# skamann/mcmc-dynamics

Hardware: AMD Instinct MI355X
Metric: star-walker log-L terms/sec (higher is better)
Workload: dtype f64; 1 GPU; C3: 1e6 synthetic stars x 256 walkers, rotation+dispersion + fixed single-Gaussian background mixture (ConstantFit + background.Gaussian), fixed centre; stars_per_gpu=1000000, stars_total=1000000, walkers=256, likelihood=bgfixed, parallelism=1 GPU

## Files before the change

include/mcd.h:

```cpp
#ifndef MCD_H
#define MCD_H

#include <stdint.h>

#ifdef __cplusplus
extern "C" {
#endif

#define MCD_ABI_VERSION 1
#define MCD_UNIQUE_ID_BYTES 128

typedef struct mcd_ctx mcd_ctx;
typedef struct mcd_catalog mcd_catalog;

typedef enum {
    MCD_OK = 0,
    MCD_ERR_INVALID = -1,
    MCD_ERR_HIP = -2,
    MCD_ERR_RCCL = -3,
    MCD_ERR_NO_DEVICE = -4,
    MCD_ERR_NONFINITE = -5,
    MCD_ERR_NOMEM = -6
} mcd_status;

typedef enum {
    MCD_MODEL_CONST = 0,
    MCD_MODEL_CONST_BGFIXED = 1,
    MCD_MODEL_CONST_BGGAUSS = 2,
    MCD_MODEL_PROFILE = 3,
    MCD_MODEL_PROFILE_BGGAUSS = 4,
    MCD_MODEL_PROFILE_BGDENS = 5,
    MCD_MODEL_PROFILE_BGFIXED = 6
} mcd_model;

typedef enum {
    MCD_CENTRE_FIXED = 0,
    MCD_CENTRE_FREE = 1
} mcd_centre;

typedef enum {
    MCD_F64 = 0,
    MCD_F32 = 1,
    MCD_F32_ACC64 = 2
} mcd_precision;

typedef struct {
    int64_t n_stars;
    const double* ra;
    const double* dec;
    const double* v;
    const double* verr;
    const double* lnlike_bg;
    const double* pmember;
    const double* density;
    int32_t model;
    int32_t centre;
    int32_t precision;
    int32_t reserved;
    double ra_center;
    double dec_center;
    int64_t n_bins;
    const int64_t* bin_offsets;
} mcd_catalog_desc;


int mcd_ctx_create(int n_dev, const int* dev_ids, mcd_ctx** out);

int mcd_get_unique_id(void* out_id);
int mcd_ctx_create_rank(int device, int rank, int n_ranks, const void* unique_id, mcd_ctx** out);

int mcd_ctx_set_option(mcd_ctx* ctx, const char* key, int64_t value);
int mcd_ctx_abort(mcd_ctx* ctx, const char* reason);
int mcd_ctx_failed(const mcd_ctx* ctx);

int mcd_ctx_destroy(mcd_ctx* ctx);
int mcd_ctx_n_devices(const mcd_ctx* ctx);
int mcd_ctx_comm_info(const mcd_ctx* ctx, int* comm_size, int* comm_rank, int* rccl_version);


int mcd_catalog_create(mcd_ctx* ctx, const mcd_catalog_desc* desc, mcd_catalog** out);
int mcd_catalog_destroy(mcd_catalog* cat);

int mcd_catalog_param_count(const mcd_catalog* cat);
int64_t mcd_catalog_n_stars(const mcd_catalog* cat);
int64_t mcd_catalog_n_outputs(const mcd_catalog* cat, int64_t n_walkers);


int mcd_loglike_batch(mcd_catalog* cat, int64_t n_walkers, int32_t k, const double* params, double* out);

int mcd_params_upload(mcd_catalog* cat, int64_t n_walkers, int32_t k, const double* params);
int mcd_loglike_enqueue(mcd_catalog* cat);
int mcd_loglike_fetch(mcd_catalog* cat, double* out);
int mcd_sync(mcd_catalog* cat);

int mcd_membership(mcd_catalog* cat, int32_t k, const double* params, double* out);
int mcd_loglike_per_star(mcd_catalog* cat, int32_t k, const double* params, double* out);
int mcd_pointwise_posterior(mcd_catalog* cat, int64_t n_samples, int32_t k, const double* params,
                            double* lppd, double* lnl_var, double* pmem_mean, double* pmem_std);
int mcd_psis_loo(mcd_catalog* cat, int64_t n_samples, int32_t k, const double* params, double r_eff,
                 double* elpd_loo, double* pareto_k, double* lppd, double* n_eff);

int mcd_kde_background(mcd_ctx* ctx, int64_t n_comp, const double* comp, int64_t n, const double* v,
                       const double* verr, double sigma_int, double* out, double* kernel_ms);


typedef struct {
    int64_t n_walkers;
    int32_t n_dim;
    int32_t k;
    const int32_t* col_source;
    const double* col_const;
    const double* col_factor;
    const double* lo;
    const double* hi;
    int32_t fixed_ok;
    int32_t n_bins;
} mcd_stretch_desc;

int mcd_stretch_move(mcd_catalog* cat, const mcd_stretch_desc* desc, int64_t n_steps, double* pos, double* lnp,
                     const int32_t* order, const double* zz, const double* thr, const int32_t* pick, double* chain,
                     double* lnprob_chain, int64_t* accepted);
int mcd_stretch_move_seeded(mcd_catalog* cat, const mcd_stretch_desc* desc, int64_t n_steps, double* pos, double* lnp,
                            uint64_t seed, int64_t step0, double* chain, double* lnprob_chain, int64_t* accepted);
int mcd_chain_numbers(uint64_t seed, int64_t step0, int64_t n_steps, int64_t n_bins, int64_t n_walkers, int32_t n_dim,
                      int32_t* order, double* zz, double* thr, int32_t* pick);

int mcd_stretch_info(const mcd_catalog* cat, int64_t* device_blocks, int64_t* host_blocks, int64_t* discarded_blocks,
                     int32_t* last_discard_status);


const char* mcd_last_error(void);
int mcd_abi_version(void);
double mcd_last_kernel_ms(const mcd_catalog* cat);
double mcd_last_device_ms(const mcd_catalog* cat);
int mcd_set_option(mcd_catalog* cat, const char* key, int64_t value);
int mcd_timing_collect(mcd_catalog* cat, double* total_kernel_ms, int64_t* n_launches);
int64_t mcd_rerun_count(const mcd_catalog* cat);
int mcd_last_prefetch(const mcd_catalog* cat);
int mcd_last_narrow_bounded(const mcd_catalog* cat);
int mcd_last_fast_level(const mcd_catalog* cat);

int mcd_last_f32_domain(const mcd_catalog* cat, double* kappa_v, double* kappa_theta);
int mcd_last_launch_info(const mcd_catalog* cat, int64_t* n_workgroups, int32_t* walker_tile,
                         int64_t* n_chunks, int32_t* record_bytes);

#ifdef __cplusplus
}
#endif
#endif
```

mcmc_dynamics_amd/_native.py:

```python
import atexit
import ctypes
import os
import weakref

import numpy as np

_HERE = os.path.dirname(os.path.abspath(__file__))
LIB_PATH = os.environ.get("MCD_LIB_PATH") or os.path.join(_HERE, "libmcd_hip.so")

MODEL_CONST, MODEL_CONST_BGFIXED, MODEL_CONST_BGGAUSS = 0, 1, 2
MODEL_PROFILE, MODEL_PROFILE_BGGAUSS, MODEL_PROFILE_BGDENS, MODEL_PROFILE_BGFIXED = 3, 4, 5, 6
CENTRE_FIXED, CENTRE_FREE = 0, 1
F64, F32, F32_ACC64 = 0, 1, 2
PRECISIONS = {"f64": F64, "f32": F32, "f32acc64": F32_ACC64}
UNIQUE_ID_BYTES = 128

_c_double_p = ctypes.POINTER(ctypes.c_double)
_c_int64_p = ctypes.POINTER(ctypes.c_int64)

SYMBOLS = {
    "mcd_ctx_create": (ctypes.c_int, [ctypes.c_int, ctypes.POINTER(ctypes.c_int), ctypes.POINTER(ctypes.c_void_p)]),
    "mcd_get_unique_id": (ctypes.c_int, [ctypes.c_void_p]),
    "mcd_ctx_create_rank": (ctypes.c_int, [ctypes.c_int, ctypes.c_int, ctypes.c_int, ctypes.c_void_p,
                                           ctypes.POINTER(ctypes.c_void_p)]),
    "mcd_ctx_destroy": (ctypes.c_int, [ctypes.c_void_p]),
    "mcd_ctx_set_option": (ctypes.c_int, [ctypes.c_void_p, ctypes.c_char_p, ctypes.c_int64]),
    "mcd_ctx_abort": (ctypes.c_int, [ctypes.c_void_p, ctypes.c_char_p]),
    "mcd_ctx_failed": (ctypes.c_int, [ctypes.c_void_p]),
    "mcd_ctx_n_devices": (ctypes.c_int, [ctypes.c_void_p]),
    "mcd_ctx_comm_info": (ctypes.c_int, [ctypes.c_void_p, ctypes.POINTER(ctypes.c_int), ctypes.POINTER(ctypes.c_int),
                                         ctypes.POINTER(ctypes.c_int)]),
    "mcd_catalog_create": (ctypes.c_int, [ctypes.c_void_p, ctypes.c_void_p, ctypes.POINTER(ctypes.c_void_p)]),
    "mcd_catalog_destroy": (ctypes.c_int, [ctypes.c_void_p]),
    "mcd_catalog_param_count": (ctypes.c_int, [ctypes.c_void_p]),
    "mcd_catalog_n_stars": (ctypes.c_int64, [ctypes.c_void_p]),
    "mcd_catalog_n_outputs": (ctypes.c_int64, [ctypes.c_void_p, ctypes.c_int64]),
    "mcd_loglike_batch": (ctypes.c_int, [ctypes.c_void_p, ctypes.c_int64, ctypes.c_int32, _c_double_p, _c_double_p]),
    "mcd_params_upload": (ctypes.c_int, [ctypes.c_void_p, ctypes.c_int64, ctypes.c_int32, _c_double_p]),
    "mcd_loglike_enqueue": (ctypes.c_int, [ctypes.c_void_p]),
    "mcd_loglike_fetch": (ctypes.c_int, [ctypes.c_void_p, _c_double_p]),
    "mcd_sync": (ctypes.c_int, [ctypes.c_void_p]),
    "mcd_membership": (ctypes.c_int, [ctypes.c_void_p, ctypes.c_int32, _c_double_p, _c_double_p]),
    "mcd_loglike_per_star": (ctypes.c_int, [ctypes.c_void_p, ctypes.c_int32, _c_double_p, _c_double_p]),
    "mcd_pointwise_posterior": (ctypes.c_int, [ctypes.c_void_p, ctypes.c_int64, ctypes.c_int32, _c_double_p, _c_double_p,
                                               _c_double_p, _c_double_p, _c_double_p]),
    "mcd_psis_loo": (ctypes.c_int, [ctypes.c_void_p, ctypes.c_int64, ctypes.c_int32, _c_double_p, ctypes.c_double,
                                    _c_double_p, _c_double_p, _c_double_p, _c_double_p]),
    "mcd_kde_background": (ctypes.c_int, [ctypes.c_void_p, ctypes.c_int64, _c_double_p, ctypes.c_int64, _c_double_p,
                                          _c_double_p, ctypes.c_double, _c_double_p, _c_double_p]),
    "mcd_stretch_move": (ctypes.c_int, [ctypes.c_void_p, ctypes.c_void_p, ctypes.c_int64, _c_double_p, _c_double_p,
                                        ctypes.POINTER(ctypes.c_int32), _c_double_p, _c_double_p,
                                        ctypes.POINTER(ctypes.c_int32), _c_double_p, _c_double_p, _c_int64_p]),
    "mcd_stretch_move_seeded": (ctypes.c_int, [ctypes.c_void_p, ctypes.c_void_p, ctypes.c_int64, _c_double_p, _c_double_p,
                                               ctypes.c_uint64, ctypes.c_int64, _c_double_p, _c_double_p, _c_int64_p]),
    "mcd_chain_numbers": (ctypes.c_int, [ctypes.c_uint64, ctypes.c_int64, ctypes.c_int64, ctypes.c_int64, ctypes.c_int64,
                                         ctypes.c_int32, ctypes.POINTER(ctypes.c_int32), _c_double_p, _c_double_p,
                                         ctypes.POINTER(ctypes.c_int32)]),
    "mcd_stretch_info": (ctypes.c_int, [ctypes.c_void_p, _c_int64_p, _c_int64_p, _c_int64_p, ctypes.POINTER(ctypes.c_int32)]),
    "mcd_last_error": (ctypes.c_char_p, []),
    "mcd_abi_version": (ctypes.c_int, []),
    "mcd_last_kernel_ms": (ctypes.c_double, [ctypes.c_void_p]),
    "mcd_last_device_ms": (ctypes.c_double, [ctypes.c_void_p]),
    "mcd_timing_collect": (ctypes.c_int, [ctypes.c_void_p, _c_double_p, _c_int64_p]),
    "mcd_rerun_count": (ctypes.c_int64, [ctypes.c_void_p]),
    "mcd_last_prefetch": (ctypes.c_int, [ctypes.c_void_p]),
    "mcd_last_narrow_bounded": (ctypes.c_int, [ctypes.c_void_p]),
    "mcd_last_fast_level": (ctypes.c_int, [ctypes.c_void_p]),
    "mcd_last_f32_domain": (ctypes.c_int, [ctypes.c_void_p, _c_double_p, _c_double_p]),
    "mcd_set_option": (ctypes.c_int, [ctypes.c_void_p, ctypes.c_char_p, ctypes.c_int64]),
    "mcd_last_launch_info": (ctypes.c_int, [ctypes.c_void_p, _c_int64_p, ctypes.POINTER(ctypes.c_int32), _c_int64_p,
                                            ctypes.POINTER(ctypes.c_int32)]),
}


class NativeError(RuntimeError):
    """Raised when the HIP library is missing, fails to load, or a call returns an error status."""


class CatalogDesc(ctypes.Structure):
    _fields_ = [
        ("n_stars", ctypes.c_int64),
        ("ra", _c_double_p), ("dec", _c_double_p), ("v", _c_double_p), ("verr", _c_double_p),
        ("lnlike_bg", _c_double_p), ("pmember", _c_double_p), ("density", _c_double_p),
        ("model", ctypes.c_int32), ("centre", ctypes.c_int32), ("precision", ctypes.c_int32),
        ("reserved", ctypes.c_int32),
        ("ra_center", ctypes.c_double), ("dec_center", ctypes.c_double),
        ("n_bins", ctypes.c_int64), ("bin_offsets", _c_int64_p),
    ]


class StretchDesc(ctypes.Structure):
    _fields_ = [
        ("n_walkers", ctypes.c_int64), ("n_dim", ctypes.c_int32), ("k", ctypes.c_int32),
        ("col_source", ctypes.POINTER(ctypes.c_int32)), ("col_const", _c_double_p), ("col_factor", _c_double_p),
        ("lo", _c_double_p), ("hi", _c_double_p), ("fixed_ok", ctypes.c_int32), ("n_bins", ctypes.c_int32),
    ]


TEST_SWITCHES = ("MCD_LIB_PATH", "MCD_RCCL_LIBRARY", "MCD_ALLOW_SHARED_DEVICE", "MCD_FORCE_RCCL", "MCD_TARGET_WAVES",
                 "MCD_CHAIN_PART_BYTES", "MCD_CHAIN_PARTS", "MCD_COLLECTIVE_TIMEOUT_MS")

_lib = None
_live_catalogs = weakref.WeakSet()
_live_contexts = weakref.WeakSet()


@atexit.register
def _shutdown():
    for cat in list(_live_catalogs):
        try:
            cat.close()
        except Exception:
            pass
    for ctx in list(_live_contexts):
        try:
            ctx.close()
        except Exception:
            pass


def load_library(path=None):
    global _lib
    if _lib is not None and path is None:
        return _lib
    p = path or LIB_PATH
    if not os.path.exists(p):
        raise NativeError(
            "HIP library not found at {0}: build it with `make -C mcmc_dynamics_amd/csrc` "
            "(or __graft_entry__.build()); there is no CPU fallback.".format(p))
    try:
        lib = ctypes.CDLL(p)
    except OSError as exc:
        raise NativeError("could not load {0}: {1}".format(p, exc))
    for name, (restype, argtypes) in SYMBOLS.items():
        try:
            fn = getattr(lib, name)
        except AttributeError:
            raise NativeError("{0} does not export {1}".format(p, name))
        fn.restype = restype
        fn.argtypes = argtypes
    if path is None:
        _lib = lib
        active = ["{0}={1}".format(k, os.environ[k]) for k in TEST_SWITCHES if os.environ.get(k)]
        if active:
            import logging
            logging.getLogger("mcmc_dynamics_amd").warning(
                "test / tuning switches active (none is needed in production, see INTEGRATION.md): %s", ", ".join(active))
    return lib


def _check(lib, rc, what):
    if rc != 0:
        msg = lib.mcd_last_error()
        raise NativeError("{0} failed (status {1}): {2}".format(what, rc, msg.decode() if msg else ""))


def _f64(a):
    return np.ascontiguousarray(a, dtype=np.float64)


def _ptr(a):
    return a.ctypes.data_as(_c_double_p) if a is not None else None


class Context(object):

    def __init__(self, n_devices=1, device_ids=None, rank=None, n_ranks=None, unique_id=None, device=None):
        self.lib = load_library()
        handle = ctypes.c_void_p()
        if rank is not None:
            uid = ctypes.create_string_buffer(bytes(unique_id), UNIQUE_ID_BYTES) if unique_id is not None else None
            rc = self.lib.mcd_ctx_create_rank(int(device or 0), int(rank), int(n_ranks), uid, ctypes.byref(handle))
            _check(self.lib, rc, "mcd_ctx_create_rank")
            self.rank, self.n_ranks = int(rank), int(n_ranks)
        else:
            ids = None
            if device_ids is not None:
                ids = (ctypes.c_int * len(device_ids))(*[int(d) for d in device_ids])
                n_devices = len(device_ids)
            rc = self.lib.mcd_ctx_create(int(n_devices), ids, ctypes.byref(handle))
            _check(self.lib, rc, "mcd_ctx_create")
            self.rank, self.n_ranks = 0, 1
        self.handle = handle
        self.host_group = None
        self._catalogs = weakref.WeakSet()
        _live_contexts.add(self)

    @staticmethod
    def unique_id():
        lib = load_library()
        buf = ctypes.create_string_buffer(UNIQUE_ID_BYTES)
        _check(lib, lib.mcd_get_unique_id(buf), "mcd_get_unique_id")
        return buf.raw

    @property
    def n_devices(self):
        return self.lib.mcd_ctx_n_devices(self.handle)

    def set_option(self, key, value):
        _check(self.lib, self.lib.mcd_ctx_set_option(self.handle, key.encode(), int(value)), "mcd_ctx_set_option")

    def abort(self, reason=""):
        if getattr(self, "handle", None):
            self.lib.mcd_ctx_abort(self.handle, str(reason).encode()[:400])

    @property
    def failed(self):
        return bool(getattr(self, "handle", None)) and bool(self.lib.mcd_ctx_failed(self.handle))

    def comm_info(self):
        n, r, v = ctypes.c_int(), ctypes.c_int(), ctypes.c_int()
        _check(self.lib, self.lib.mcd_ctx_comm_info(self.handle, ctypes.byref(n), ctypes.byref(r), ctypes.byref(v)),
               "mcd_ctx_comm_info")
        return {"size": n.value, "rank": r.value, "rccl_version": v.value}

    def kde_background(self, comp, v, verr, sigma_int=0.0, return_kernel_ms=False):
        if not getattr(self, "handle", None):
            raise NativeError("context is closed")
        comp, v, verr = _f64(comp).ravel(), _f64(v).ravel(), _f64(verr).ravel()
# ... 86 lines not shown
        self.k = self.lib.mcd_catalog_param_count(handle)
        self._walkers = 0
        _live_catalogs.add(self)
        ctx._catalogs.add(self)

    def _params(self, params):
        p = _f64(params)
        if p.ndim == 1:
            p = p[None, :]
        if self.n_sets > 1:
            if p.ndim != 3 or p.shape[0] != self.n_sets:
                raise ValueError("binned catalogue expects params of shape (n_bins, W, K)")
            w = p.shape[1]
        else:
            if p.ndim == 3 and p.shape[0] == 1:
                p = p[0]
            if p.ndim != 2:
                raise ValueError("params must have shape (W, K)")
            w = p.shape[0]
        if p.shape[-1] != self.k:
            raise ValueError("params have {0} columns, catalogue expects {1}".format(p.shape[-1], self.k))
        return np.ascontiguousarray(p), w

    def _alive(self):
        if not getattr(self, "handle", None):
            raise NativeError("catalogue is closed")

    def loglike(self, params):
        self._alive()
        p, w = self._params(params)
        out = np.empty((self.n_sets, w) if self.n_sets > 1 else (w,), dtype=np.float64)
        rc = self.lib.mcd_loglike_batch(self.handle, w, self.k, _ptr(p), _ptr(out))
        _check(self.lib, rc, "mcd_loglike_batch")
        self._walkers = w
        return out

    def upload_params(self, params):
        p, w = self._params(params)
        _check(self.lib, self.lib.mcd_params_upload(self.handle, w, self.k, _ptr(p)), "mcd_params_upload")
        self._walkers = w

    def enqueue(self):
        _check(self.lib, self.lib.mcd_loglike_enqueue(self.handle), "mcd_loglike_enqueue")

    def sync(self):
        _check(self.lib, self.lib.mcd_sync(self.handle), "mcd_sync")

    def fetch(self):
        w = self._walkers
        out = np.empty((self.n_sets, w) if self.n_sets > 1 else (w,), dtype=np.float64)
        _check(self.lib, self.lib.mcd_loglike_fetch(self.handle, _ptr(out)), "mcd_loglike_fetch")
        return out

    def membership(self, params_row):
        p = _f64(params_row).reshape(-1)
        out = np.empty(self.n_stars, dtype=np.float64)
        _check(self.lib, self.lib.mcd_membership(self.handle, p.size, _ptr(p), _ptr(out)), "mcd_membership")
        return out

    def loglike_per_star(self, params_row):
        p = _f64(params_row).reshape(-1)
        out = np.empty(self.n_stars, dtype=np.float64)
        _check(self.lib, self.lib.mcd_loglike_per_star(self.handle, p.size, _ptr(p), _ptr(out)), "mcd_loglike_per_star")
        return out

    def pointwise_posterior(self, table, membership=False):
        self._alive()
        if self.n_sets > 1:
            raise ValueError("pointwise_posterior is defined for un-binned catalogues only")
        p = _f64(table)
        if p.ndim == 1:
            p = p[None, :]
        if p.ndim != 2 or p.shape[1] != self.k:
            raise ValueError("table must have shape (S, {0})".format(self.k))
        p = np.ascontiguousarray(p)
        names = ("lppd", "lnl_var") + (("pmem_mean", "pmem_std") if membership else ())
        out = {k: np.empty(self.n_stars, dtype=np.float64) for k in names}
        ptrs = [_ptr(out[k]) if k in out else None for k in ("lppd", "lnl_var", "pmem_mean", "pmem_std")]
        rc = self.lib.mcd_pointwise_posterior(self.handle, p.shape[0], self.k, _ptr(p), *ptrs)
        _check(self.lib, rc, "mcd_pointwise_posterior")
        return out

    def psis_loo(self, table, r_eff=1.0):
        self._alive()
        if self.n_sets > 1:
            raise ValueError("psis_loo is defined for un-binned catalogues only")
        p = _f64(table)
        if p.ndim == 1:
            p = p[None, :]
        if p.ndim != 2 or p.shape[1] != self.k:
            raise ValueError("table must have shape (S, {0})".format(self.k))
        p = np.ascontiguousarray(p)
        names = ("elpd_loo", "pareto_k", "lppd", "n_eff")
        out = {k: np.empty(self.n_stars, dtype=np.float64) for k in names}
        rc = self.lib.mcd_psis_loo(self.handle, p.shape[0], self.k, _ptr(p), float(r_eff), *[_ptr(out[k]) for k in names])
        _check(self.lib, rc, "mcd_psis_loo")
        return out

    def _stretch_args(self, name, plan, pos, lnp, n_steps, chain, lnprob_chain, accepted):
        self._alive()
        for a in (pos, lnp):
            if a.dtype != np.float64 or not a.flags.c_contiguous:
                raise ValueError(name + " needs C-contiguous arrays of the documented dtypes")
        if pos.ndim not in (2, 3) or lnp.shape != pos.shape[:-1]:
            raise ValueError(name + ": inconsistent array shapes")
        lead, (w, p) = pos.shape[:-2], pos.shape[-2:]
        cols = [np.ascontiguousarray(plan["col_source"], dtype=np.int32), _f64(plan["col_const"]), _f64(plan["col_factor"]),
                _f64(plan["lo"]), _f64(plan["hi"])]
        if cols[0].size != self.k or cols[1].size != self.k or cols[2].size != self.k or cols[3].size != p or cols[4].size != p:
            raise ValueError("stretch_move: plan does not match the catalogue / the number of free parameters")
        d = StretchDesc()
        d.n_walkers, d.n_dim, d.k, d.n_bins = w, p, self.k, lead[0] if lead else 1
        d.col_source = cols[0].ctypes.data_as(ctypes.POINTER(ctypes.c_int32))
        d.col_const, d.col_factor, d.lo, d.hi = (_ptr(c) for c in cols[1:])
        d.fixed_ok = 1 if plan.get("fixed_ok", True) else 0
        for a, shape in ((chain, (n_steps,) + lead + (w, p)), (lnprob_chain, (n_steps,) + lead + (w,))):
            if a is not None and (a.dtype != np.float64 or not a.flags.c_contiguous or a.shape != shape):
                raise ValueError("stretch_move: chain buffers must be C-contiguous float64 of shape (steps, [B,] W, P) / (steps, [B,] W)")
        if accepted is not None and (accepted.dtype != np.int64 or accepted.shape != lead + (w,) or not accepted.flags.c_contiguous):
            raise ValueError("stretch_move: accepted must be a C-contiguous int64 array of shape ([B,] W)")
        return ((self.handle, ctypes.byref(d), n_steps, _ptr(pos), _ptr(lnp)),
                (_ptr(chain), _ptr(lnprob_chain), accepted.ctypes.data_as(_c_int64_p) if accepted is not None else None), cols)

    def stretch_move(self, plan, pos, lnp, order, zz, thr, pick, chain=None, lnprob_chain=None, accepted=None):
        head, tail, _keep = self._stretch_args("stretch_move", plan, pos, lnp, order.shape[0], chain, lnprob_chain, accepted)
        for a, dt in ((zz, np.float64), (thr, np.float64), (order, np.int32), (pick, np.int32)):
            if a.dtype != dt or not a.flags.c_contiguous:
                raise ValueError("stretch_move needs C-contiguous arrays of the documented dtypes")
        half_shape = (order.shape[0], 2) + pos.shape[:-2] + (pos.shape[-2] // 2,)
        if order.shape != order.shape[:1] + lnp.shape or zz.shape != half_shape or thr.shape != half_shape or \
                pick.shape != half_shape:
            raise ValueError("stretch_move: inconsistent array shapes")
        rc = self.lib.mcd_stretch_move(*head, order.ctypes.data_as(ctypes.POINTER(ctypes.c_int32)), _ptr(zz), _ptr(thr),
                                       pick.ctypes.data_as(ctypes.POINTER(ctypes.c_int32)), *tail)
        _check(self.lib, rc, "mcd_stretch_move")
        self._walkers = pos.shape[-2] // 2

    def stretch_move_seeded(self, plan, pos, lnp, seed, step0, n_steps, chain=None, lnprob_chain=None, accepted=None):
        if n_steps < 0 or step0 < 0:
            raise ValueError("stretch_move_seeded: inconsistent array shapes")
        head, tail, _keep = self._stretch_args("stretch_move_seeded", plan, pos, lnp, n_steps, chain, lnprob_chain, accepted)
        rc = self.lib.mcd_stretch_move_seeded(*head, int(seed) & 0xFFFFFFFFFFFFFFFF, int(step0), *tail)
        _check(self.lib, rc, "mcd_stretch_move_seeded")
        self._walkers = pos.shape[-2] // 2

    @property
    def last_prefetch(self):
        return self.lib.mcd_last_prefetch(self.handle)

    @property
    def last_narrow_bounded(self):
        return self.lib.mcd_last_narrow_bounded(self.handle)

    def stretch_info(self):
        a, b, c, st = ctypes.c_int64(), ctypes.c_int64(), ctypes.c_int64(), ctypes.c_int32()
        _check(self.lib, self.lib.mcd_stretch_info(self.handle, ctypes.byref(a), ctypes.byref(b), ctypes.byref(c), ctypes.byref(st)),
               "mcd_stretch_info")
        return {"device_blocks": a.value, "host_blocks": b.value, "discarded_blocks": c.value, "last_discard_status": st.value}

    def set_option(self, key, value):
        _check(self.lib, self.lib.mcd_set_option(self.handle, key.encode(), int(value)), "mcd_set_option")

    @property
    def last_kernel_ms(self):
        return self.lib.mcd_last_kernel_ms(self.handle)

    @property
    def last_device_ms(self):
        return self.lib.mcd_last_device_ms(self.handle)

    def timing_collect(self):
        total, n = ctypes.c_double(), ctypes.c_int64()
        _check(self.lib, self.lib.mcd_timing_collect(self.handle, ctypes.byref(total), ctypes.byref(n)),
               "mcd_timing_collect")
        return total.value, n.value

    @property
    def rerun_count(self):
        return self.lib.mcd_rerun_count(self.handle)

    @property
    def fast_level(self):
        return self.lib.mcd_last_fast_level(self.handle)

    @property
    def f32_in_domain(self):
        return bool(self.lib.mcd_last_f32_domain(self.handle, None, None))

    @property
    def f32_condition(self):
        kv, kt = ctypes.c_double(), ctypes.c_double()
        self.lib.mcd_last_f32_domain(self.handle, ctypes.byref(kv), ctypes.byref(kt))
        return kv.value, kt.value

    def launch_info(self):
        wg, ch = ctypes.c_int64(), ctypes.c_int64()
        tile, rb = ctypes.c_int32(), ctypes.c_int32()
        _check(self.lib, self.lib.mcd_last_launch_info(self.handle, ctypes.byref(wg), ctypes.byref(tile),
                                                       ctypes.byref(ch), ctypes.byref(rb)), "mcd_last_launch_info")
        return {"workgroups": wg.value, "walker_tile": tile.value, "chunks": ch.value, "record_bytes": rb.value}

    def close(self):
        if getattr(self, "handle", None):
            self.lib.mcd_catalog_destroy(self.handle)
            self.handle = None

    def __del__(self):
        try:
            self.close()
        except Exception:
            pass
```

mcmc_dynamics_amd/csrc/mcd_api_catalog.hip:

```cpp
#include "mcd_host.h"

using namespace mcd::host;

namespace {

int param_count(int model, bool free_centre) {
    int k = (mcd::is_profile(model) ? 6 : 4) + (free_centre ? 2 : 0);
    const int bg = mcd::bg_kind(model);
    if (bg == mcd::BG_GAUSS) k += 3;
    if (bg == mcd::BG_FIXED_DENSITY) k += 1;
    return k;
}

void free_workset(WorkSet& w) {
    if (w.d_chunks) (void)hipFree(w.d_chunks);
    if (w.d_offsets) (void)hipFree(w.d_offsets);
    if (w.d_chunk_general) (void)hipFree(w.d_chunk_general);
    if (w.d_params) (void)hipFree(w.d_params);
    if (w.d_wpar) (void)hipFree(w.d_wpar);
    if (w.d_partials) (void)hipFree(w.d_partials);
    if (w.d_out) (void)hipFree(w.d_out);
    if (w.d_out2) (void)hipFree(w.d_out2);
    if (w.d_partials2) (void)hipFree(w.d_partials2);
    if (w.ev_staged) (void)hipEventDestroy(w.ev_staged);
    for (int b = 0; b < 2; ++b) {
        if (w.ev_reduced[b]) (void)hipEventDestroy(w.ev_reduced[b]);
        if (w.ev_comm[b]) (void)hipEventDestroy(w.ev_comm[b]);
    }
    if (w.h_params) (void)hipHostFree(w.h_params);
    if (w.h_out) (void)hipHostFree(w.h_out);
    w = WorkSet();
}

double model_cost(int model, bool free_centre) {
    static const double kCost[mcd::kNumModels] = {8.5, 24.0, 45.0, 25.0, 60.0, 40.0, 42.0};
    return (kCost[model] + (free_centre ? 7.0 : 0.0)) / 8.5;
}
int balance_auto_m(const mcd_catalog* cat, int64_t n, int64_t n_walkers) {
    const int64_t n_wtiles = (n_walkers + 63) / 64;
    const double tiles = n_wtiles <= 4 ? (double)n_wtiles : 4.0 * (double)((n_wtiles + 3) / 4);
    const double work = (double)n * tiles / 4.0 * model_cost(cat->model, cat->free_centre);
    const double limit = mcd::bg_kind(cat->model) == mcd::BG_NONE ? 9.0e5 : 1.3e6;
    if (cat->n_psets != 1 || work > limit) return 0;
    return work < 6.0e4 ? 2 : (work <= 3.4e5 ? 4 : 8);
}

bool wants_prefetch(const mcd_catalog* cat, const Shard& sh) {
    if (cat->prefetch >= 0) return cat->prefetch != 0;
    const size_t bytes = (size_t)sh.n * (size_t)mcd::record_bytes(cat->model, cat->free_centre, cat->precision);
    if (mcd::bg_kind(cat->model) == mcd::BG_NONE) return cat->n_psets == 1 && bytes >= ((size_t)128 << 20);
    return bytes >= ((size_t)8 << 20);
}

struct Option {
    const char* key;
    int64_t min, max;
    const char* message;
    bool sync, replan;
    void (*set)(mcd_catalog* c, int64_t v);
    bool (*accepts)(int64_t v) = nullptr;
};
constexpr int64_t kMin = std::numeric_limits<int64_t>::min(), kMax = std::numeric_limits<int64_t>::max();
#define MCD_SET(statement) [](mcd_catalog* c, int64_t v) { statement; }
const Option kOptions[] = {
    {"fast_path", 0, 2, "fast_path: 0 (plain), 1 (guarded, default) or 2 (guarded, no narrow variant)", false, false, MCD_SET(c->allow_fast = (int)v)},
    {"zero_copy", kMin, kMax, nullptr, false, false, MCD_SET(c->zero_copy = v != 0)},
    {"device_chain", 0, 2, "device_chain: 0 (host-driven blocks), 1 (default) or 2 (as 1 with the general step kernel, testing aid)", false, false,
     MCD_SET(c->device_chain = (int)v; c->chain_backoff = 0; c->chain_consecutive = 0; c->chain_hint = -1)},
    {"fused_reduce", kMin, kMax, nullptr, false, false, MCD_SET(c->fused_reduce = v != 0)},
    {"defer_guard", kMin, kMax, nullptr, false, false, MCD_SET(c->defer_guard = v != 0)},
    {"f32_domain", kMin, kMax, nullptr, false, false, MCD_SET(c->f32_domain = v != 0)},
    {"loo_scratch_mb", 1, kMax, "loo_scratch_mb must be >= 1", false, false, MCD_SET(c->loo_scratch_mb = v)},
    {"posterior_pass", 1, kMax, "posterior_pass must be >= 1", false, false, MCD_SET(c->posterior_pass = v)},
    {"two_lanes", kMin, kMax, nullptr, true, false, MCD_SET(c->two_lanes = v != 0)},
    {"narrow_bounded", 0, 1, "narrow_bounded: 1 (where the guard admits it, default) or 0 (never)", false, false, MCD_SET(c->narrow_bounded = (int)v)},
    {"prefetch", -1, 1, "prefetch: -1 (by record volume, default), 0 (off) or 1 (on)", false, false, MCD_SET(c->prefetch = (int)v)},
    {"spin_us", 0, kMax, "spin_us must be >= 0", false, false, MCD_SET(c->spin_us = v)},
    {"tail_split", kMin, kMax, nullptr, true, true, MCD_SET(c->tail_split = (int)v)},
    {"target_waves", 1, kMax, "target_waves must be positive", true, true, MCD_SET(c->target_waves = v)},
    {"chunk_len", 0, kMax, "chunk_len must be >= 0", true, true, MCD_SET(c->chunk_len = v)},
    {"balance", -1, 8, "balance: -1 (auto), 0 (off) or 1 .. 8 workgroups per CU", true, true, MCD_SET(c->balance = (int)v)},
    {"combine", 0, 16, "combine: 0 (never), 1 (largest workgroup the plan allows), 8 or 16 (waves per workgroup at most)", true, true,
     MCD_SET(c->combine = (int)v), [](int64_t v) { return v <= 1 || v == 8 || v == 16; }},
};
#undef MCD_SET
}

MCD_HOST_BEGIN

LaunchShape main_launch_shape(mcd_catalog* cat, const Shard& sh, const WorkSet& w, int level, bool coll, double* out_buf,
                              int64_t n_out) {
    LaunchShape shape{cat->model, cat->free_centre, cat->precision, level, w.uniform_len, sh.n};
    shape.uniform_extra = w.uniform_extra;
    shape.waves = w.waves;
    shape.chunk_general = w.d_chunk_general;
    shape.prefetch = wants_prefetch(cat, sh);
    cat->last_prefetch = shape.prefetch && shape.fast != 0;
    shape.rerun_flag = coll ? nullptr : out_buf + n_out;
    return shape;
}

const double* fast_pset_const(const mcd_catalog* cat, const Shard& sh, int level) {
    const int bgk = mcd::bg_kind(cat->model);
    return (level && (bgk == mcd::BG_FIXED || bgk == mcd::BG_FIXED_DENSITY)) ? sh.d_pset_const : nullptr;
}

int build_workset(mcd_catalog* cat, Shard& sh, int64_t n_walkers, WorkSet** out) {
    auto it = sh.work.find(n_walkers);
    if (it != sh.work.end()) { *out = &it->second; return MCD_OK; }
    if (sh.work.size() >= 8) {
        for (auto& kv : sh.work) free_workset(kv.second);
        sh.work.clear();
        cat->cur_walkers = 0;
    }
    const DeviceSlot& slot = cat->ctx->slots[sh.slot];
    MCD_HIP(hipSetDevice(slot.device));

    mcd::ChunkPlan plan;
    for (int m = cat->balance < 0 ? balance_auto_m(cat, sh.n, n_walkers) : cat->balance;; m /= 2) {
        plan = mcd::plan_chunks(cat->bin_offsets, sh.star_begin, sh.n, n_walkers, cat->target_waves, cat->tail_split,
                                cat->stats.narrow_exceptions, cat->chunk_len, m);
        if (m == 0 || plan.balanced_m > 0) break;
    }
    const std::vector<mcd::Chunk>& chunks = plan.chunks;
    const std::vector<int64_t>& offs = plan.offsets;
    const std::vector<uint8_t>& general = plan.general;

    WorkSet w;
    w.n_walkers = n_walkers;
    w.n_chunks = (int64_t)chunks.size();
    w.max_chunks_per_pset = plan.max_chunks_per_pset;
    w.uniform_len = plan.uniform_len;
    w.uniform_extra = plan.uniform_extra;
    {
        const int64_t n_wtiles = (n_walkers + 63) / 64;
        const bool shape_ok = plan.balanced_m > 0 && plan.balanced_m % 2 == 0 && (n_wtiles == 1 || n_wtiles == 2 || n_wtiles == 4) &&
                              cat->precision == MCD_F64;
        w.waves = 4;
        if (cat->combine != 0 && shape_ok) {
            const bool can16 = mcd::bg_kind(cat->model) != mcd::BG_GAUSS;
            w.waves = 8;
            if (cat->combine == 16 && plan.balanced_m % 4 == 0 && can16) w.waves = 16;
            if (cat->combine == 1 && plan.balanced_m == 4 && can16) w.waves = 16;
        }
    }
    const int64_t padded_walkers = (n_walkers + 63) / 64 * 64;
    const int64_t n_out = cat->n_psets * n_walkers;
    const size_t term_bytes = cat->precision == MCD_F64 ? 8 : 4;
    auto allocate = [&]() -> hipError_t {
        hipError_t e;
        if (!general.empty()) {
            if ((e = hipMalloc(&w.d_chunk_general, general.size())) != hipSuccess) return e;
            if ((e = hipMemcpy(w.d_chunk_general, general.data(), general.size(), hipMemcpyHostToDevice)) != hipSuccess) return e;
        }
        if ((e = hipMalloc(&w.d_chunks, std::max<size_t>(1, chunks.size()) * sizeof(mcd::Chunk))) != hipSuccess) return e;
        if ((e = hipMalloc(&w.d_offsets, offs.size() * sizeof(int64_t))) != hipSuccess) return e;
        if ((e = hipMalloc(&w.d_params, (size_t)n_out * cat->k * sizeof(double))) != hipSuccess) return e;
        if ((e = hipMalloc(&w.d_wpar, (size_t)n_out * mcd::KD * term_bytes)) != hipSuccess) return e;
        if ((e = hipMalloc(&w.d_partials, std::max<size_t>(1, (size_t)padded_walkers * w.n_chunks) * sizeof(double))) != hipSuccess) return e;
        if ((e = hipMalloc(&w.d_out, (size_t)(n_out + 1) * sizeof(double))) != hipSuccess) return e;
        if ((e = hipMemset(w.d_out, 0, (size_t)(n_out + 1) * sizeof(double))) != hipSuccess) return e;
        if ((e = hipMalloc(&w.d_out2, (size_t)(n_out + 1) * sizeof(double))) != hipSuccess) return e;
        if ((e = hipMemset(w.d_out2, 0, (size_t)(n_out + 1) * sizeof(double))) != hipSuccess) return e;
        if ((e = hipEventCreateWithFlags(&w.ev_staged, hipEventDisableTiming)) != hipSuccess) return e;
        for (int b = 0; b < 2; ++b) {
            if ((e = hipEventCreateWithFlags(&w.ev_reduced[b], hipEventDisableTiming)) != hipSuccess) return e;
            if ((e = hipEventCreateWithFlags(&w.ev_comm[b], hipEventDisableTiming)) != hipSuccess) return e;
        }
        if ((e = hipHostMalloc(&w.h_params, (size_t)n_out * cat->k * sizeof(double), hipHostMallocMapped)) != hipSuccess) return e;
        if ((e = hipHostMalloc(&w.h_out, (size_t)(n_out + 1) * sizeof(double), hipHostMallocMapped)) != hipSuccess) return e;
        std::memset(w.h_out, 0, (size_t)(n_out + 1) * sizeof(double));
        if ((e = hipHostGetDevicePointer((void**)&w.m_params, w.h_params, 0)) != hipSuccess) return e;
        if ((e = hipHostGetDevicePointer((void**)&w.m_out, w.h_out, 0)) != hipSuccess) return e;
        if (!chunks.empty() &&
            (e = hipMemcpy(w.d_chunks, chunks.data(), chunks.size() * sizeof(mcd::Chunk), hipMemcpyHostToDevice)) != hipSuccess)
            return e;
        return hipMemcpy(w.d_offsets, offs.data(), offs.size() * sizeof(int64_t), hipMemcpyHostToDevice);
    };
    const hipError_t err = allocate();
    if (err != hipSuccess) {
        free_workset(w);
        return fail(MCD_ERR_HIP, std::string("work buffers for this walker count: ") + hipGetErrorString(err));
    }
    auto ins = sh.work.emplace(n_walkers, w);
    *out = &ins.first->second;
    return MCD_OK;
}

MCD_HOST_END

extern "C" {

static int catalog_create_impl(mcd_ctx* ctx, const mcd_catalog_desc* d, std::unique_ptr<mcd_catalog>& cat);

int mcd_catalog_create(mcd_ctx* ctx, const mcd_catalog_desc* d, mcd_catalog** out) {
    try {
    if (!ctx || !d || !out) return fail(MCD_ERR_INVALID, "mcd_catalog_create: null argument");
    std::unique_ptr<mcd_catalog> cat;
    const int rc = catalog_create_impl(ctx, d, cat);
    if (rc != MCD_OK) {
        if (cat) {
            const std::string msg = g_last_error;
            mcd_catalog_destroy(cat.release());
            g_last_error = msg;
        }
        return rc;
    }
    *out = cat.release();
    return MCD_OK;
    } catch (...) { return on_exception("mcd_catalog_create"); }
}

static int catalog_create_impl(mcd_ctx* ctx, const mcd_catalog_desc* d, std::unique_ptr<mcd_catalog>& cat) {
    if (int urc = ctx_usable(ctx)) return urc;
    if (d->n_stars < 0) return fail(MCD_ERR_INVALID, "negative n_stars");
    if (d->model < 0 || d->model >= mcd::kNumModels) return fail(MCD_ERR_INVALID, "unknown model");
    const int bgk = mcd::bg_kind(d->model);
    if (d->centre != MCD_CENTRE_FIXED && d->centre != MCD_CENTRE_FREE) return fail(MCD_ERR_INVALID, "unknown centre mode");
    if (d->precision < MCD_F64 || d->precision > MCD_F32_ACC64) return fail(MCD_ERR_INVALID, "unknown precision");
    if (d->n_stars > 0 && (!d->ra || !d->dec || !d->v || !d->verr)) return fail(MCD_ERR_INVALID, "missing ra/dec/v/verr column");
    if (bgk == mcd::BG_FIXED && d->n_stars > 0 && (!d->lnlike_bg || !d->pmember))
        return fail(MCD_ERR_INVALID, "background model needs lnlike_bg and pmember columns");
    if (bgk == mcd::BG_GAUSS && d->n_stars > 0 && !d->density)
        return fail(MCD_ERR_INVALID, "Gaussian-background model needs the density column");
    if (bgk == mcd::BG_FIXED_DENSITY && d->n_stars > 0 && (!d->lnlike_bg || !d->density))
        return fail(MCD_ERR_INVALID, "constant-background model needs lnlike_bg and density columns");

    cat.reset(new (std::nothrow) mcd_catalog());
    if (!cat) return fail(MCD_ERR_INVALID, "out of memory");
    cat->ctx = ctx;
    cat->model = d->model;
    cat->free_centre = d->centre == MCD_CENTRE_FREE;
    cat->precision = d->precision;
    cat->k = param_count(d->model, cat->free_centre);
    cat->n_stars = d->n_stars;
    if (const char* tw = std::getenv("MCD_TARGET_WAVES")) {
        long v = std::atol(tw);
        if (v > 0) cat->target_waves = v;
    }
    if (d->n_bins > 1) {
        if (!d->bin_offsets) return fail(MCD_ERR_INVALID, "bin_offsets required when n_bins > 1");
        cat->n_psets = d->n_bins;
        cat->bin_offsets.assign(d->bin_offsets, d->bin_offsets + d->n_bins + 1);
        if (cat->bin_offsets.front() != 0 || cat->bin_offsets.back() != d->n_stars)
            return fail(MCD_ERR_INVALID, "bin_offsets must start at 0 and end at n_stars");
        for (int64_t b = 0; b < d->n_bins; ++b)
            if (cat->bin_offsets[b + 1] < cat->bin_offsets[b]) return fail(MCD_ERR_INVALID, "bin_offsets must be non-decreasing");
    } else {
        cat->n_psets = 1;
        cat->bin_offsets = {0, d->n_stars};
    }

    cat->stats = mcd::compute_stats(d->n_stars, d->v, d->verr, d->lnlike_bg, d->pmember, d->density, bgk,
                                    cat->precision != MCD_F64 || mcd::is_profile(cat->model) ? d->ra : nullptr, d->dec,
                                    !cat->free_centre, d->ra_center, d->dec_center);

    const int n_dev = (int)ctx->slots.size();
    cat->shards.resize(n_dev);
    const int rec_bytes = mcd::record_bytes(cat->model, cat->free_centre, cat->precision);
    for (int i = 0; i < n_dev; ++i) {
        Shard& sh = cat->shards[i];
        sh.slot = i;
        const mcd::ShardRange range = mcd::shard_range(d->n_stars, i, n_dev);
        sh.star_begin = range.begin;
        sh.n = range.n;
        const DeviceSlot& slot = ctx->slots[i];
        MCD_HIP(hipSetDevice(slot.device));
        MCD_HIP(hipEventCreate(&sh.ev_begin));
        MCD_HIP(hipEventCreate(&sh.ev_k0));
        MCD_HIP(hipEventCreate(&sh.ev_k1));
        MCD_HIP(hipEventCreate(&sh.ev_end));
        MCD_HIP(hipMalloc(&sh.records, (size_t)sh.n * rec_bytes + 2048));
        MCD_HIP(hipMemsetAsync(sh.records, 0, (size_t)sh.n * rec_bytes + 2048, slot.stream));
        if (bgk == mcd::BG_FIXED || bgk == mcd::BG_FIXED_DENSITY) {
            const std::vector<double> sums = mcd::pset_background_sums(d->lnlike_bg, cat->bin_offsets, sh.star_begin, sh.n);
            MCD_HIP(hipMalloc(&sh.d_pset_const, sums.size() * sizeof(double)));
            MCD_HIP(hipMemcpy(sh.d_pset_const, sums.data(), sums.size() * sizeof(double), hipMemcpyHostToDevice));
        }
        if (sh.n == 0) continue;
        const double* host_cols[7] = {d->ra, d->dec, d->v, d->verr, d->lnlike_bg, d->pmember, d->density};
        struct Scratch {
            double* p[7] = {nullptr, nullptr, nullptr, nullptr, nullptr, nullptr, nullptr};
            ~Scratch() { for (double* q : p) if (q) (void)hipFree(q); }
        } dev;
        for (int c = 0; c < 7; ++c) {
            if (!host_cols[c]) continue;
            MCD_HIP(hipMalloc(&dev.p[c], (size_t)sh.n * sizeof(double)));
            MCD_HIP(hipMemcpyAsync(dev.p[c], host_cols[c] + sh.star_begin, (size_t)sh.n * sizeof(double),
                                   hipMemcpyHostToDevice, slot.stream));
        }
        mcd::RawColumns raw{dev.p[0], dev.p[1], dev.p[2], dev.p[3], dev.p[4], dev.p[5], dev.p[6]};
        MCD_HIP(mcd::launch_prepare_records(slot.stream, raw, sh.n, cat->model, cat->free_centre, cat->precision,
                                            d->ra_center, d->dec_center, sh.records));
        MCD_HIP(hipStreamSynchronize(slot.stream));
    }
    return MCD_OK;
}

int mcd_catalog_destroy(mcd_catalog* cat) {
    if (!cat) return MCD_OK;
    if (cat->ctx && cat->ctx->failed.load()) { delete cat; return MCD_OK; }
    for (Shard& sh : cat->shards) {
        (void)hipSetDevice(cat->ctx->slots[sh.slot].device);
        (void)hipStreamSynchronize(cat->ctx->slots[sh.slot].stream);
        (void)hipStreamSynchronize(cat->ctx->slots[sh.slot].comm_stream);
        (void)hipStreamSynchronize(cat->ctx->slots[sh.slot].stream2);
        for (auto& kv : sh.work) free_workset(kv.second);
        if (sh.records) (void)hipFree(sh.records);
        if (sh.d_pset_const) (void)hipFree(sh.d_pset_const);
        if (sh.ev_begin) (void)hipEventDestroy(sh.ev_begin);
        if (sh.ev_k0) (void)hipEventDestroy(sh.ev_k0);
        if (sh.ev_k1) (void)hipEventDestroy(sh.ev_k1);
        if (sh.ev_end) (void)hipEventDestroy(sh.ev_end);
        for (auto& pr : sh.ring) { (void)hipEventDestroy(pr.first); (void)hipEventDestroy(pr.second); }
    }
    for (hipEvent_t e : cat->chain_events) (void)hipEventDestroy(e);
    if (cat->chain.d) (void)hipFree(cat->chain.d);
    if (cat->chain.h) (void)hipHostFree(cat->chain.h);
    delete cat;
    return MCD_OK;
}

int mcd_catalog_param_count(const mcd_catalog* cat) { return cat ? cat->k : MCD_ERR_INVALID; }
int64_t mcd_catalog_n_stars(const mcd_catalog* cat) { return cat ? cat->n_stars : MCD_ERR_INVALID; }
int64_t mcd_catalog_n_outputs(const mcd_catalog* cat, int64_t n_walkers) {
    return cat ? cat->n_psets * n_walkers : MCD_ERR_INVALID;
}

int mcd_set_option(mcd_catalog* cat, const char* key, int64_t value) {
    try {
    if (!cat || !key) return fail(MCD_ERR_INVALID, "mcd_set_option: null argument");
    if (!std::strcmp(key, "timing")) {
        int rc = sync_all(cat);
        if (rc != MCD_OK) return rc;
        cat->timing = value != 0;
        cat->timing_all = value == 2;
        for (Shard& sh : cat->shards) sh.ring_used = 0;
        return MCD_OK;
    }
    if (!std::strcmp(key, "timing_discard")) {
        int rc = sync_all(cat);
        if (rc != MCD_OK) return rc;
        for (Shard& sh : cat->shards) sh.ring_used = 0;
        cat->timing_launches = 0;
        return MCD_OK;
    }
    if (!std::strcmp(key, "timing_stride")) {
        if (value < 1) return fail(MCD_ERR_INVALID, "timing_stride must be >= 1");
        int rc = sync_all(cat);
        if (rc != MCD_OK) return rc;
        cat->timing_stride = value;
        cat->timing_launches = 0;
        return MCD_OK;
    }
    if (!std::strcmp(key, "timing_reserve")) {
        if (value < 0 || value > ((int64_t)1 << 16)) return fail(MCD_ERR_INVALID, "timing_reserve: 0 .. 65536 launches");
        for (Shard& sh : cat->shards) {
            MCD_HIP(hipSetDevice(cat->ctx->slots[sh.slot].device));
            while ((int64_t)sh.ring.size() < value) {
                hipEvent_t a, b;
                MCD_HIP(hipEventCreate(&a));
                if (hipEventCreate(&b) != hipSuccess) { (void)hipEventDestroy(a); return fail(MCD_ERR_HIP, "hipEventCreate"); }
                sh.ring.emplace_back(a, b);
            }
        }
        return MCD_OK;
    }
    for (const Option& o : kOptions) {
        if (std::strcmp(key, o.key)) continue;
        if (value < o.min || value > o.max || (o.accepts && !o.accepts(value))) return fail(MCD_ERR_INVALID, o.message);
        if (o.sync)
            if (int rc = sync_all(cat)) return rc;
        o.set(cat, value);
        if (o.replan) {
            for (Shard& sh : cat->shards) {
                (void)hipSetDevice(cat->ctx->slots[sh.slot].device);
                for (auto& kv : sh.work) free_workset(kv.second);
                sh.work.clear();
            }
            cat->cur_walkers = 0;
        }
        return MCD_OK;
    }
    return fail(MCD_ERR_INVALID, std::string("unknown option: ") + key);
    } catch (...) { return on_exception("mcd_set_option"); }
}

int mcd_timing_collect(mcd_catalog* cat, double* total_kernel_ms, int64_t* n_launches) {
    try {
    if (!cat) return fail(MCD_ERR_INVALID, "null catalogue");
    int rc = sync_all(cat);
    if (rc != MCD_OK) return rc;
    Shard& sh = cat->shards[0];
    double total = 0.0;
    for (size_t i = 0; i < sh.ring_used; ++i) {
        float ms = 0.f;
        MCD_HIP(hipEventElapsedTime(&ms, sh.ring[i].first, sh.ring[i].second));
        total += ms;
    }
    if (total_kernel_ms) *total_kernel_ms = total;
    if (n_launches) *n_launches = (int64_t)sh.ring_used;
    for (Shard& s2 : cat->shards) s2.ring_used = 0;
    cat->timing_launches = 0;
    return MCD_OK;
    } catch (...) { return on_exception("mcd_timing_collect"); }
}

int64_t mcd_rerun_count(const mcd_catalog* cat) { return cat ? cat->n_reruns : MCD_ERR_INVALID; }

int mcd_stretch_info(const mcd_catalog* cat, int64_t* device_blocks, int64_t* host_blocks, int64_t* discarded_blocks,
                     int32_t* last_discard_status) {
    if (!cat) return fail(MCD_ERR_INVALID, "null catalogue");
    if (device_blocks) *device_blocks = cat->chain_device_blocks;
    if (host_blocks) *host_blocks = cat->chain_host_blocks;
    if (discarded_blocks) *discarded_blocks = cat->chain_discarded;
    if (last_discard_status) *last_discard_status = cat->chain_last_status;
    return MCD_OK;
}

int mcd_last_prefetch(const mcd_catalog* cat) { return cat ? cat->last_prefetch : -1; }

int mcd_last_narrow_bounded(const mcd_catalog* cat) { return cat ? cat->last_narrow_bounded : -1; }

int mcd_last_f32_domain(const mcd_catalog* cat, double* kappa_v, double* kappa_theta) {
    if (!cat) return -1;
    if (kappa_v) *kappa_v = cat->last_f32.kappa_v;
    if (kappa_theta) *kappa_theta = cat->last_f32.kappa_theta;
    if (cat->precision == MCD_F64) return 1;
    return cat->last_f32.inside ? 1 : 0;
}

int mcd_last_fast_level(const mcd_catalog* cat) {
    if (!cat || cat->cur_walkers <= 0 || cat->shards.empty()) return -1;
    const auto it = cat->shards.front().work.find(cat->cur_walkers);
    return it == cat->shards.front().work.end() ? -1 : it->second.fast;
}

double mcd_last_kernel_ms(const mcd_catalog* cat) { return cat ? cat->last_kernel_ms : -1.0; }
double mcd_last_device_ms(const mcd_catalog* cat) { return cat ? cat->last_device_ms : -1.0; }

int mcd_last_launch_info(const mcd_catalog* cat, int64_t* n_workgroups, int32_t* walker_tile, int64_t* n_chunks,
                         int32_t* record_bytes) {
    if (!cat) return fail(MCD_ERR_INVALID, "null catalogue");
    if (n_workgroups) *n_workgroups = cat->last_grid;
    if (walker_tile) *walker_tile = 64;
    if (n_chunks) *n_chunks = cat->last_chunks;
    if (record_bytes) *record_bytes = mcd::record_bytes(cat->model, cat->free_centre, cat->precision);
    return MCD_OK;
}

}
```

mcmc_dynamics_amd/csrc/mcd_api_chain.hip:

```cpp
#include "mcd_host.h"
#include "mcd_rng.h"
#include "mcd_stretch.h"

using namespace mcd::host;

namespace {

void big_copy(void* dst, const void* src, size_t bytes) {
    constexpr size_t kSerial = (size_t)4 << 20;
    if (bytes < kSerial) { std::memcpy(dst, src, bytes); return; }
    constexpr int kMaxThreads = 16;
    static const int kThreads = [] {
        const char* e = std::getenv("MCD_COPY_THREADS");
        const int n = e ? std::atoi(e) : 4;
        return n < 1 ? 1 : (n > kMaxThreads ? kMaxThreads : n);
    }();
    std::thread workers[kMaxThreads - 1];
    const size_t part = (bytes / kThreads + 63) / 64 * 64;
    int started = 0;
    for (int t = 1; t < kThreads; ++t) {
        const size_t at = std::min(bytes, part * t), len = std::min(bytes, part * (t + 1)) - at;
        try {
            workers[t - 1] = std::thread([=] { if (len) std::memcpy((char*)dst + at, (const char*)src + at, len); });
            ++started;
// ... 10 lines not shown
int stretch_block_device(mcd_catalog* cat, const mcd_stretch_desc* d, int64_t n_steps, double* pos, double* lnp,
                         const int32_t* order, const double* zz, const double* thr, const int32_t* pick, double* chain,
                         double* lnprob_chain, int64_t* accepted, bool* done, const uint64_t* seed = nullptr,
                         int64_t step0 = 0) {
    *done = false;
    mcd_ctx* ctx = cat->ctx;
    if (int urc = ctx_usable(ctx)) return urc;
    const int64_t B = cat->n_psets;
    if (!cat->device_chain || cat->shards.size() != 1 || cat->precision != MCD_F64 || n_steps < 1 || cat->timing || !d->fixed_ok)
        return MCD_OK;
    if (B > 1 && cat->device_chain != 1) return MCD_OK;
    if (cat->chain_backoff > 0) { --cat->chain_backoff; return MCD_OK; }
    const int64_t W = d->n_walkers, half = W / 2;
    const int P = d->n_dim, K = d->k;
    bool small_ensemble = false;
    {
        mcd::StretchDevice probe;
        probe.n_bins = B; probe.n_walkers = W; probe.n_dim = P; probe.k = K;
        probe.force_general = cat->device_chain == 2;
        if (!mcd::stretch_step_handles(probe)) return MCD_OK;
        small_ensemble = mcd::stretch_step_fuses(probe);
    }
    Shard& sh = cat->shards[0];
    const DeviceSlot& slot = ctx->slots[sh.slot];
    MCD_HIP(hipSetDevice(slot.device));
    WorkSet* wp = nullptr;
    int rc = build_workset(cat, sh, half, &wp);
    if (rc != MCD_OK) return rc;
    WorkSet& w = *wp;
    MCD_WAIT(cat->ctx, slot.stream, cat->spin_us, "mcd_stretch_move (previous evaluation)");
    MCD_WAIT(cat->ctx, slot.stream2, cat->spin_us, "mcd_stretch_move (previous evaluation, second lane)");
    MCD_WAIT(cat->ctx, slot.comm_stream, cat->spin_us, "mcd_stretch_move (previous collective)");
    w.comm_pending[0] = w.comm_pending[1] = false;
    w.staged = false;

    size_t off = 0;
    auto take = [&](size_t bytes) { const size_t at = off; off += (bytes + 63) / 64 * 64; return at; };
    const size_t BW = (size_t)B * W, Bh = (size_t)B * half;
    const size_t o_pos = take(BW * P * 8), o_lnp = take(BW * 8), o_acc = take(BW * 8);
    const size_t o_meta = take(mcd::META_WORDS * 4), o_status = take(8);
    const size_t n_launches = (size_t)2 * n_steps;
    const bool defer = cat->defer_guard != 0 && B == 1 && small_ensemble && n_launches * half * K * 8 <= ((size_t)64 << 20);
    const size_t o_levels = take(defer ? n_launches * 4 : 0);
    const size_t state_end = off;
    const size_t o_src = take((size_t)K * 4), o_const = take((size_t)K * 8), o_fac = take((size_t)K * 8);
    const size_t o_lo = take((size_t)P * 8), o_hi = take((size_t)P * 8);
    const bool seeded = seed != nullptr;
    const bool gen_device = seeded && mcd::chain_numbers_on_device(W);
    const size_t n_in = (size_t)n_steps;
    const size_t o_order = take(n_in * BW * 4), o_zz = take(n_in * BW * 8);
    const size_t o_thr = take(n_in * BW * 8), o_pick = take(n_in * BW * 4);
    const size_t input_end = off;
    const size_t o_prop = take(Bh * P * 8), o_ok = take(Bh), o_nok = take((size_t)2 * B * 4), o_ranges = take((size_t)2 * B * 10 * 8);
    const size_t o_nok_log = take(defer ? n_launches * 4 : 0), o_table_log = take(defer ? n_launches * half * K * 8 : 0);
    const size_t o_chain = take(chain ? (size_t)n_steps * BW * P * 8 : 0);
    const size_t o_lnpc = take(lnprob_chain ? (size_t)n_steps * BW * 8 : 0);
    const size_t total = off;
    ChainArena& a = cat->chain;
    if (a.bytes < total) {
        if (a.d) (void)hipFree(a.d);
        if (a.h) (void)hipHostFree(a.h);
        a = ChainArena();
        const size_t want = total + total / 2;
        const bool must_agree = ctx->n_ranks > 1 || ctx->force_collective;
        if (hipMalloc((void**)&a.d, want) != hipSuccess) {
            (void)hipGetLastError();
            a = ChainArena();
            if (must_agree) return fail(MCD_ERR_NOMEM, "mcd_stretch_move: no device memory for the resident block of this rank (use shorter blocks)");
            return MCD_OK;
        }
        if (hipHostMalloc((void**)&a.h, want, hipHostMallocDefault) != hipSuccess) {
            (void)hipGetLastError();
            (void)hipFree(a.d);
            a = ChainArena();
            if (must_agree) return fail(MCD_ERR_NOMEM, "mcd_stretch_move: no pinned host memory for the resident block of this rank (use shorter blocks)");
            return MCD_OK;
        }
        a.bytes = want;
    }
    std::memcpy(a.h + o_pos, pos, BW * P * 8);
    std::memcpy(a.h + o_lnp, lnp, BW * 8);
    if (accepted) std::memcpy(a.h + o_acc, accepted, BW * 8);
    else std::memset(a.h + o_acc, 0, BW * 8);
    std::memset(a.h + o_meta, 0, mcd::META_WORDS * 4);
    std::memset(a.h + o_status, 0, 8);
    std::memcpy(a.h + o_src, d->col_source, (size_t)K * 4);
    std::memcpy(a.h + o_const, d->col_const, (size_t)K * 8);
    std::memcpy(a.h + o_fac, d->col_factor, (size_t)K * 8);
    std::memcpy(a.h + o_lo, d->lo, (size_t)P * 8);
    std::memcpy(a.h + o_hi, d->hi, (size_t)P * 8);
    const size_t moved = (size_t)n_steps * BW * ((gen_device ? 0 : 24) + (chain ? (size_t)P * 8 : 0) + (lnprob_chain ? 8 : 0));
    size_t part_threshold = (size_t)16 << 20;
    if (const char* e = std::getenv("MCD_CHAIN_PART_BYTES")) part_threshold = (size_t)std::strtoull(e, nullptr, 10);
    int64_t max_parts = 16;
    if (const char* e = std::getenv("MCD_CHAIN_PARTS")) max_parts = std::max<long long>(1, std::atoll(e));
    const int64_t n_parts = moved >= part_threshold ? std::min<int64_t>(max_parts, n_steps) : 1;
    auto part_begin = [&](int64_t k) { return n_steps * k / n_parts; };
    auto copy_in = [&](int64_t i0, int64_t i1) {
        if (gen_device) return;
        const size_t at = (size_t)i0 * BW, n = (size_t)(i1 - i0) * BW;
        if (seeded) {
            std::vector<uint64_t> sorter;
            for (int64_t i = i0; i < i1; ++i)
                mcd::chain_numbers_of_step(*seed, step0 + i, B, W, P, (int32_t*)(a.h + o_order) + (size_t)i * BW,
                                           (double*)(a.h + o_zz) + (size_t)i * BW, (double*)(a.h + o_thr) + (size_t)i * BW,
                                           (int32_t*)(a.h + o_pick) + (size_t)i * BW, sorter);
            return;
        }
        big_copy(a.h + o_order + at * 4, order + at, n * 4);
        big_copy(a.h + o_zz + at * 8, zz + at, n * 8);
        big_copy(a.h + o_thr + at * 8, thr + at, n * 8);
        big_copy(a.h + o_pick + at * 4, pick + at, n * 4);
    };
    if (n_parts == 1) copy_in(0, n_steps);

    int level = cat->chain_hint;
    if (level < 0) {
        std::vector<double> table(BW * K);
        for (size_t j = 0; j < BW; ++j)
            for (int c = 0; c < K; ++c) {
                const int src = d->col_source[c];
                table[j * K + c] = src < 0 ? d->col_const[c]
                                           : (d->col_factor[c] == 1.0 ? pos[j * P + src] : pos[j * P + src] * d->col_factor[c]);
            }
        level = fast_level(cat, table.data(), (int64_t)BW);
    }

    mcd::StretchDevice sd;
    sd.n_bins = B;
    sd.n_walkers = W; sd.n_dim = P; sd.k = K; sd.fixed_ok = d->fixed_ok;
    sd.model = cat->model; sd.free_centre = cat->free_centre ? 1 : 0; sd.allow_fast = cat->allow_fast;
    sd.expected_level = level;
    sd.force_general = cat->device_chain == 2;
    sd.stats = cat->stats;
    sd.col_source = (const int32_t*)(a.d + o_src); sd.col_const = (const double*)(a.d + o_const);
    sd.col_factor = (const double*)(a.d + o_fac); sd.lo = (const double*)(a.d + o_lo); sd.hi = (const double*)(a.d + o_hi);
    sd.pos = (double*)(a.d + o_pos); sd.lnp = (double*)(a.d + o_lnp); sd.accepted = (long long*)(a.d + o_acc);
    sd.order = (const int32_t*)(a.d + o_order); sd.zz = (const double*)(a.d + o_zz); sd.thr = (const double*)(a.d + o_thr);
    sd.pick = (const int32_t*)(a.d + o_pick);
    sd.chain = chain ? (double*)(a.d + o_chain) : nullptr;
    sd.lnprob_chain = lnprob_chain ? (double*)(a.d + o_lnpc) : nullptr;
    sd.proposal = (double*)(a.d + o_prop); sd.ok = (uint8_t*)(a.d + o_ok); sd.meta = (int32_t*)(a.d + o_meta);
    sd.n_ok = (int32_t*)(a.d + o_nok); sd.ranges = (double*)(a.d + o_ranges);
    sd.table = w.d_params; sd.wpar = (double*)w.d_wpar;
    if (defer) {
        sd.defer_guard = 1;
        sd.table_log = (double*)(a.d + o_table_log); sd.n_ok_log = (int32_t*)(a.d + o_nok_log); sd.level_log = (int32_t*)(a.d + o_levels);
    }

    const bool coll = ctx->n_ranks > 1 || ctx->force_collective;
    double* const out_buf = w.d_out;
    mcd::LaunchShape shape = main_launch_shape(cat, sh, w, level, coll, out_buf, (int64_t)Bh);
    cat->last_narrow_bounded = 0;
    const double* pset_const = fast_pset_const(cat, sh, level);
    const int64_t n_slots = mcd::partial_slots(shape, w.n_chunks, half);
    const int64_t max_slots = B == 1 ? n_slots : w.max_chunks_per_pset;
    const bool fused = cat->fused_reduce != 0 && !coll && max_slots <= mcd::kFusedReduceSlots && mcd::stretch_step_fuses(sd);
    sd.fused = fused ? 1 : 0;
    sd.partials = w.d_partials;
    sd.n_slots = n_slots;
    sd.slot_offsets = B == 1 ? nullptr : w.d_offsets;
    sd.pset_const = pset_const;
    cat->chain_last_fused = fused;
    double prev_tag = 0.0;
    int64_t acc_step = -1;
    int acc_h = 0;
#ifdef MCD_CHAIN_STAMPS
    static unsigned long long* d_stamps = nullptr;
    if (!d_stamps) MCD_HIP(hipMalloc((void**)&d_stamps, 8 * 8 * 4096));
    MCD_HIP(hipMemsetAsync(d_stamps, 0, 8 * 8 * 4096, slot.stream));
    sd.stamps = d_stamps;
#endif
    auto enqueue_steps = [&](int64_t i0, int64_t i1, hipEvent_t mark) -> int {
        for (int64_t i = i0; i < i1; ++i)
            for (int h = 0; h < 2; ++h) {
#ifdef MCD_CHAIN_STAMPS
                sd.launch_index = i * 2 + h;
#endif
                MCD_HIP(mcd::launch_stretch_step(slot.stream, sd, acc_step, acc_h, i, h, out_buf, prev_tag));
                if (mark && i == i0 && h == 0) MCD_HIP(hipEventRecord(mark, slot.stream));
                prev_tag = coll ? 0.0 : (double)(++cat->launch_seq);
                shape.launch_tag = prev_tag;
                MCD_HIP(mcd::launch_loglike(slot.stream, shape, sh.records, w.d_chunks, w.n_chunks, w.d_wpar, w.d_partials, half));
                if (!fused)
                    MCD_HIP(mcd::launch_reduce(slot.stream, w.d_partials, w.d_offsets, B, n_slots, max_slots, half, pset_const,
                                               out_buf));
                if (coll) {
                    if (!ctx->multi_process) MCD_NCCL(g_rccl.GroupStart());
                    MCD_NCCL(g_rccl.AllReduce(out_buf, out_buf, Bh, ncclDouble, ncclSum, slot.comm, slot.stream));
                    if (!ctx->multi_process) MCD_NCCL(g_rccl.GroupEnd());
                }
                acc_step = i;
                acc_h = h;
            }
        return MCD_OK;
    };
    auto finish = [&]() -> int {
        MCD_HIP(mcd::launch_stretch_step(slot.stream, sd, acc_step, acc_h, -1, 0, out_buf, prev_tag));
        if (defer) MCD_HIP(mcd::launch_stretch_judge(slot.stream, sd, (int64_t)n_launches));
        if (coll) {
            double* status = (double*)(a.d + o_status);
            MCD_HIP(mcd::launch_stretch_status(slot.stream, sd.meta, status));
            if (!ctx->multi_process) MCD_NCCL(g_rccl.GroupStart());
            MCD_NCCL(g_rccl.AllReduce(status, status, 1, ncclDouble, ncclSum, slot.comm, slot.stream));
            if (!ctx->multi_process) MCD_NCCL(g_rccl.GroupEnd());
        }
        return MCD_OK;
    };
    struct MidBlockGuard {
        mcd_ctx* ctx; bool armed; bool ok;
        ~MidBlockGuard() {
            if (armed && !ok && !ctx->failed.load()) {
                const std::string cause = g_last_error;
                (void)ctx_fail(ctx, "mcd_stretch_move: this rank failed in the middle of a resident block (" + cause + ")");
            }
        }
    } mid_block{ctx, coll, false};
    bool rows_delivered = false;
    auto generate = [&](hipStream_t s, int64_t i0, int64_t i1) {
        return mcd::launch_chain_numbers(s, *seed, step0, i0, i1, B, W, P, (int32_t*)(a.d + o_order), (double*)(a.d + o_zz),
                                         (double*)(a.d + o_thr), (int32_t*)(a.d + o_pick));
    };
    if (n_parts == 1) {
        MCD_HIP(hipMemcpyAsync(a.d, a.h, gen_device ? o_order : input_end, hipMemcpyHostToDevice, slot.stream));
        if (gen_device) MCD_HIP(generate(slot.stream, 0, n_steps));
        rc = enqueue_steps(0, n_steps, nullptr);
        if (rc != MCD_OK) return rc;
        rc = finish();
        if (rc != MCD_OK) return rc;
        MCD_HIP(hipMemcpyAsync(a.h, a.d, state_end, hipMemcpyDeviceToHost, slot.stream));
        if (total > o_chain)
            MCD_HIP(hipMemcpyAsync(a.h + o_chain, a.d + o_chain, total - o_chain, hipMemcpyDeviceToHost, slot.stream));
        MCD_WAIT(cat->ctx, slot.stream, cat->spin_us, "mcd_stretch_move (resident block)");
    } else {
        while ((int64_t)cat->chain_events.size() < 3 * n_parts) {
            hipEvent_t e;
            MCD_HIP(hipEventCreateWithFlags(&e, hipEventDisableTiming));
            cat->chain_events.push_back(e);
        }
        hipEvent_t* ev_in = cat->chain_events.data();
        hipEvent_t* ev_rows = ev_in + n_parts;
        hipEvent_t* ev_out = ev_rows + n_parts;
        auto rows_to_host = [&](int64_t k) -> int {
            const size_t at = (size_t)part_begin(k) * BW, n = (size_t)(part_begin(k + 1) - part_begin(k)) * BW;
            MCD_HIP(hipStreamWaitEvent(slot.comm_stream, ev_rows[k], 0));
            if (chain) MCD_HIP(hipMemcpyAsync(a.h + o_chain + at * P * 8, a.d + o_chain + at * P * 8, n * P * 8, hipMemcpyDeviceToHost, slot.comm_stream));
            if (lnprob_chain) MCD_HIP(hipMemcpyAsync(a.h + o_lnpc + at * 8, a.d + o_lnpc + at * 8, n * 8, hipMemcpyDeviceToHost, slot.comm_stream));
            MCD_HIP(hipEventRecord(ev_out[k], slot.comm_stream));
            return MCD_OK;
        };
        auto rows_to_caller = [&](int64_t k) -> int {
            const size_t at = (size_t)part_begin(k) * BW, n = (size_t)(part_begin(k + 1) - part_begin(k)) * BW;
            MCD_WAIT(cat->ctx, slot.comm_stream, cat->spin_us, "mcd_stretch_move (chain rows of a part)");
            if (chain) big_copy(chain + at * P, a.h + o_chain + at * P * 8, n * P * 8);
            if (lnprob_chain) big_copy(lnprob_chain + at, a.h + o_lnpc + at * 8, n * 8);
            return MCD_OK;
        };
        MCD_HIP(hipMemcpyAsync(a.d, a.h, o_order, hipMemcpyHostToDevice, slot.stream));
        for (int64_t k = 0; k < n_parts; ++k) {
            const int64_t i0 = part_begin(k), i1 = part_begin(k + 1);
            const size_t at = (size_t)i0 * BW, n = (size_t)(i1 - i0) * BW;
            if (gen_device) {
                MCD_HIP(generate(slot.comm_stream, i0, i1));
                MCD_HIP(hipEventRecord(ev_in[k], slot.comm_stream));
                MCD_HIP(hipStreamWaitEvent(slot.stream, ev_in[k], 0));
            } else {
                copy_in(i0, i1);
                MCD_HIP(hipMemcpyAsync(a.d + o_order + at * 4, a.h + o_order + at * 4, n * 4, hipMemcpyHostToDevice, slot.comm_stream));
                MCD_HIP(hipMemcpyAsync(a.d + o_zz + at * 8, a.h + o_zz + at * 8, n * 8, hipMemcpyHostToDevice, slot.comm_stream));
                MCD_HIP(hipMemcpyAsync(a.d + o_thr + at * 8, a.h + o_thr + at * 8, n * 8, hipMemcpyHostToDevice, slot.comm_stream));
                MCD_HIP(hipMemcpyAsync(a.d + o_pick + at * 4, a.h + o_pick + at * 4, n * 4, hipMemcpyHostToDevice, slot.comm_stream));
                MCD_HIP(hipEventRecord(ev_in[k], slot.comm_stream));
                MCD_HIP(hipStreamWaitEvent(slot.stream, ev_in[k], 0));
            }
            rc = enqueue_steps(i0, i1, k > 0 ? ev_rows[k - 1] : nullptr);
            if (rc != MCD_OK) return rc;
            if (k > 0) {
                rc = rows_to_host(k - 1);
                if (rc != MCD_OK) return rc;
                rc = rows_to_caller(k - 1);
                if (rc != MCD_OK) return rc;
            }
        }
        rc = finish();
        if (rc != MCD_OK) return rc;
        MCD_HIP(hipEventRecord(ev_rows[n_parts - 1], slot.stream));
        MCD_HIP(hipMemcpyAsync(a.h, a.d, state_end, hipMemcpyDeviceToHost, slot.stream));
        rc = rows_to_host(n_parts - 1);
        if (rc != MCD_OK) return rc;
        rc = rows_to_caller(n_parts - 1);
        if (rc != MCD_OK) return rc;
        MCD_WAIT(cat->ctx, slot.stream, cat->spin_us, "mcd_stretch_move (resident block, last part)");
        MCD_WAIT(cat->ctx, slot.comm_stream, cat->spin_us, "mcd_stretch_move (resident block, chain rows)");
        rows_delivered = true;
    }
#ifdef MCD_CHAIN_STAMPS
    {
        const int64_t n = std::min<int64_t>(n_steps * 2, 4096);
        std::vector<unsigned long long> st((size_t)n * 8);
        MCD_HIP(hipMemcpy(st.data(), d_stamps, st.size() * 8, hipMemcpyDeviceToHost));
        double sum[8] = {0}, period = 0;
        int64_t cnt = 0;
        for (int64_t i = 2; i + 1 < n; ++i) {
            for (int k = 1; k < 8; ++k) sum[k] += (double)(st[i * 8 + k] - st[i * 8 + k - 1]);
            period += (double)(st[(i + 1) * 8] - st[i * 8]);
            ++cnt;
        }
        if (cnt > 0) {
            fprintf(stderr, "[chain stamps] period %.2f us; phases (us):", period / cnt / 100.0);
            for (int k = 1; k < 8; ++k) fprintf(stderr, " %d:%.2f", k, sum[k] / cnt / 100.0);
            fprintf(stderr, "\n");
        }
    }
#endif

    mid_block.ok = true;
    w.fast = level;
    cat->cur_walkers = half;
    cat->last_chunks = w.n_chunks;
    {
        const int64_t slots = mcd::partial_slots(shape, w.n_chunks, half);
        cat->last_grid = slots != w.n_chunks ? slots : mcd::main_grid(w.n_chunks, half);
    }
    const int32_t* meta = (const int32_t*)(a.h + o_meta);
    const bool discard = meta[mcd::META_STATUS] != 0 || (coll && *(const double*)(a.h + o_status) != 0.0);
    if (discard) {
        ++cat->chain_discarded;
        cat->chain_last_status = meta[mcd::META_STATUS];
        cat->chain_hint = (meta[mcd::META_STATUS] & mcd::CHAIN_LEVEL) ? meta[mcd::META_LEVEL] : -1;
        if (defer && (meta[mcd::META_STATUS] & mcd::CHAIN_LEVEL)) {
            const int32_t* levels = (const int32_t*)(a.h + o_levels);
            cat->chain_hint = -1;
            for (size_t l = 0; l < n_launches; ++l)
                if (levels[l] >= 0 && levels[l] != level) { cat->chain_hint = levels[l]; break; }
        }
        cat->chain_consecutive = std::min(cat->chain_consecutive + 1, 7);
// ... 114 lines not shown
```

mcmc_dynamics_amd/csrc/mcd_api_eval.hip:

```cpp
#include "mcd_host.h"

using namespace mcd::host;

MCD_HOST_BEGIN

int fast_level(const mcd_catalog* cat, const double* params, int64_t n_rows) {
    if (!cat->allow_fast) return 0;
    const int level = mcd::fast_level(cat->stats, cat->model, cat->free_centre, cat->precision != MCD_F64, cat->k, params, n_rows);
    return cat->allow_fast == 2 && level > 1 ? 1 : level;
}

int sync_all(mcd_catalog* cat) {
    if (!cat) return fail(MCD_ERR_INVALID, "null catalogue");
    if (int rc = ctx_usable(cat->ctx)) return rc;
    for (Shard& sh : cat->shards) {
        const DeviceSlot& slot = cat->ctx->slots[sh.slot];
        MCD_HIP(hipSetDevice(slot.device));
        MCD_WAIT(cat->ctx, slot.stream, cat->spin_us, "mcd_sync / mcd_loglike_fetch (compute stream)");
        MCD_WAIT(cat->ctx, slot.stream2, cat->spin_us, "mcd_sync / mcd_loglike_fetch (second compute lane)");
        MCD_WAIT(cat->ctx, slot.comm_stream, cat->spin_us, "mcd_sync / mcd_loglike_fetch (communication stream)");
    }
    if (cat->timing && cat->timing_pending) {
        Shard& sh = cat->shards[0];
        float k_ms = 0.f, d_ms = 0.f;
        if (cat->timing_all) {
            if (sh.ring_used > 0)
                MCD_HIP(hipEventElapsedTime(&k_ms, sh.ring[sh.ring_used - 1].first, sh.ring[sh.ring_used - 1].second));
        } else {
            MCD_HIP(hipEventElapsedTime(&k_ms, sh.ev_k0, sh.ev_k1));
        }
        if (!cat->timing_all) MCD_HIP(hipEventElapsedTime(&d_ms, sh.ev_begin, sh.ev_end));
        cat->last_kernel_ms = k_ms;
        cat->last_device_ms = cat->timing_all ? -1.0 : d_ms;
        cat->timing_pending = false;
    }
    return MCD_OK;
}

MCD_HOST_END

namespace {

WorkSet* find_work(Shard& sh, int64_t W) {
    const auto it = sh.work.find(W);
    return it == sh.work.end() ? nullptr : &it->second;
}

bool all_staged(mcd_catalog* cat) {
    if (cat->cur_walkers <= 0) return false;
    for (Shard& sh : cat->shards) {
        const WorkSet* w = find_work(sh, cat->cur_walkers);
        if (!w || !w->staged) return false;
    }
    return true;
}

int stage_params_impl(mcd_catalog* cat, int64_t n_walkers, int32_t k, const double* params, bool zero_copy) {
    if (!cat || !params) return fail(MCD_ERR_INVALID, "null catalogue or params");
    if (int rc = ctx_usable(cat->ctx)) return rc;
    if (n_walkers <= 0) return fail(MCD_ERR_INVALID, "n_walkers must be positive");
    if (k != cat->k) {
        char buf[128];
        snprintf(buf, sizeof buf, "parameter table has %d columns, catalogue expects %d", (int)k, cat->k);
        return fail(MCD_ERR_INVALID, buf);
    }
    const int64_t n_rows = cat->n_psets * n_walkers;
    if (cat->precision != MCD_F64) {
        cat->last_f32 = mcd::f32_domain(cat->stats, cat->model, cat->free_centre, cat->k, params, n_rows);
        if (!cat->last_f32.inside && cat->f32_domain)
            return fail(MCD_ERR_INVALID, std::string("outside the float32 accuracy domain (use an MCD_F64 catalogue, or option "
                                                     "f32_domain = 0 to evaluate regardless): ") + cat->last_f32.reason);
    }
    const int fast = fast_level(cat, params, n_rows);
    const int narrow_rescale = fast == 2 && cat->precision == MCD_F64
                                   ? mcd::bounded_rescale(cat->stats, cat->model, cat->free_centre, cat->k, params, n_rows) : 0;
    for (Shard& sh : cat->shards) {
        WorkSet* w = nullptr;
        int rc = build_workset(cat, sh, n_walkers, &w);
        if (rc != MCD_OK) return rc;
        const DeviceSlot& slot = cat->ctx->slots[sh.slot];
        MCD_HIP(hipSetDevice(slot.device));
        MCD_WAIT(cat->ctx, slot.stream, cat->spin_us, "mcd_params_upload (previous evaluation)");
        if (w->lane1_used) {
            MCD_WAIT(cat->ctx, slot.stream2, cat->spin_us, "mcd_params_upload (previous evaluation, second lane)");
            w->lane1_used = false;
        }
        std::memcpy(w->h_params, params, (size_t)n_rows * k * sizeof(double));
        w->mapped = zero_copy;
        const double* src = w->m_params;
        if (!zero_copy) {
            MCD_HIP(hipMemcpyAsync(w->d_params, w->h_params, (size_t)n_rows * k * sizeof(double), hipMemcpyHostToDevice,
                                   slot.stream));
            src = w->d_params;
        }
        MCD_HIP(mcd::launch_prepare_walkers(slot.stream, src, n_rows, k, cat->model, cat->free_centre,
                                            cat->precision, w->d_wpar));
        MCD_HIP(hipEventRecord(w->ev_staged, slot.stream));
        w->lane1_knows_staging = false;
        w->fast = fast;
        w->narrow_rescale = narrow_rescale;
        w->staged = true;
    }
    cat->cur_walkers = n_walkers;
    return MCD_OK;
}

int stage_params(mcd_catalog* cat, int64_t n_walkers, int32_t k, const double* params, bool zero_copy) {
    const int rc = stage_params_impl(cat, n_walkers, k, params, zero_copy);
    if (rc != MCD_OK && cat) cat->cur_walkers = 0;
    return rc;
}

int enqueue(mcd_catalog* cat, bool pipelined) {
    if (!cat) return fail(MCD_ERR_INVALID, "null catalogue");
    if (int rc = ctx_usable(cat->ctx)) return rc;
    if (cat->cur_walkers <= 0) return fail(MCD_ERR_INVALID, "no parameters staged (call mcd_params_upload first)");
    if (!all_staged(cat)) return fail(MCD_ERR_INVALID, "no parameters staged for this walker count (the last upload failed?)");
    const int64_t W = cat->cur_walkers;
    const int64_t n_out = cat->n_psets * W;
    mcd_ctx* ctx = cat->ctx;
    for (Shard& sh : cat->shards) {
        WorkSet& w = (*find_work(sh, W));
        const DeviceSlot& slot = ctx->slots[sh.slot];
        MCD_HIP(hipSetDevice(slot.device));
        const bool coll = ctx->n_ranks > 1 || ctx->slots.size() > 1 || ctx->force_collective;
        double* out_buf = w.mapped ? w.m_out : w.d_out;
        const bool two_lanes = pipelined && cat->two_lanes && !(cat->timing && !cat->timing_all);
        hipStream_t lane_stream = slot.stream;
        double* lane_partials = w.d_partials;
        if (coll || two_lanes) {
            w.buf ^= 1;
            out_buf = w.buf ? w.d_out2 : w.d_out;
            if (two_lanes && w.buf) {
                if (!w.d_partials2) {
                    const int64_t padded_walkers = (W + 63) / 64 * 64;
                    MCD_HIP(hipMalloc(&w.d_partials2, std::max<size_t>(1, (size_t)padded_walkers * w.n_chunks) * sizeof(double)));
                }
                if (!w.lane1_knows_staging) {
                    MCD_HIP(hipStreamWaitEvent(slot.stream2, w.ev_staged, 0));
                    w.lane1_knows_staging = true;
                }
                lane_stream = slot.stream2;
                lane_partials = w.d_partials2;
                w.lane1_used = true;
            }
        } else {
            w.buf = 0;
        }
        mcd::LaunchShape shape = main_launch_shape(cat, sh, w, w.fast, coll, out_buf, n_out);
        shape.narrow_rescale = cat->narrow_bounded ? w.narrow_rescale : 0;
        cat->last_narrow_bounded = mcd::narrow_bounded_launch(shape) ? shape.narrow_rescale : 0;
        w.launch_tag = coll ? 0.0 : (double)(++cat->launch_seq);
        shape.launch_tag = w.launch_tag;
        hipEvent_t k0 = sh.ev_k0, k1 = sh.ev_k1;
        const bool sampled = !cat->timing_all || (cat->timing_launches % cat->timing_stride) == 0;
        if (cat->timing_all && sampled) {
            if (sh.ring_used >= (size_t)1 << 16) sh.ring_used = 0;
            if (sh.ring_used == sh.ring.size()) {
                hipEvent_t a, b;
                MCD_HIP(hipEventCreate(&a));
                MCD_HIP(hipEventCreate(&b));
                sh.ring.emplace_back(a, b);
            }
            k0 = sh.ring[sh.ring_used].first;
            k1 = sh.ring[sh.ring_used].second;
            ++sh.ring_used;
        }
        if (cat->timing && !cat->timing_all) MCD_HIP(hipEventRecord(sh.ev_begin, slot.stream));
        if (cat->timing && sampled) MCD_HIP(hipEventRecord(k0, lane_stream));
        MCD_HIP(mcd::launch_loglike(lane_stream, shape, sh.records, w.d_chunks, w.n_chunks, w.d_wpar, lane_partials, W));
        if (cat->timing && sampled) MCD_HIP(hipEventRecord(k1, lane_stream));
        const double* pset_const = fast_pset_const(cat, sh, w.fast);
        if (coll && w.comm_pending[w.buf]) {
            MCD_HIP(hipStreamWaitEvent(lane_stream, w.ev_comm[w.buf], 0));
            w.comm_pending[w.buf] = false;
        }
        {
            const int64_t n_slots = mcd::partial_slots(shape, w.n_chunks, W);
            MCD_HIP(mcd::launch_reduce(lane_stream, lane_partials, w.d_offsets, cat->n_psets, n_slots,
                                       cat->n_psets == 1 ? n_slots : w.max_chunks_per_pset, W, pset_const, out_buf));
        }
        if (coll && pipelined) MCD_HIP(hipEventRecord(w.ev_reduced[w.buf], lane_stream));
    }
    const bool collective = ctx->n_ranks > 1 || ctx->slots.size() > 1 || ctx->force_collective;
    if (collective) {
        if (!ctx->multi_process) MCD_NCCL(g_rccl.GroupStart());
        for (Shard& sh : cat->shards) {
            WorkSet& w = (*find_work(sh, W));
            const DeviceSlot& slot = ctx->slots[sh.slot];
            MCD_HIP(hipSetDevice(slot.device));
            double* buf = w.buf ? w.d_out2 : w.d_out;
            if (pipelined) {
                MCD_HIP(hipStreamWaitEvent(slot.comm_stream, w.ev_reduced[w.buf], 0));
                MCD_NCCL(g_rccl.AllReduce(buf, buf, (size_t)n_out, ncclDouble, ncclSum, slot.comm, slot.comm_stream));
            } else {
                if (w.comm_pending[w.buf ^ 1]) {
                    MCD_HIP(hipStreamWaitEvent(slot.stream, w.ev_comm[w.buf ^ 1], 0));
                    w.comm_pending[w.buf ^ 1] = false;
                }
                MCD_NCCL(g_rccl.AllReduce(buf, buf, (size_t)n_out, ncclDouble, ncclSum, slot.comm, slot.stream));
            }
        }
        if (!ctx->multi_process) MCD_NCCL(g_rccl.GroupEnd());
        if (pipelined) {
            for (Shard& sh : cat->shards) {
                WorkSet& w = (*find_work(sh, W));
                const DeviceSlot& slot = ctx->slots[sh.slot];
                MCD_HIP(hipSetDevice(slot.device));
                MCD_HIP(hipEventRecord(w.ev_comm[w.buf], slot.comm_stream));
                w.comm_pending[w.buf] = true;
            }
        }
    }
    if (cat->timing_all) ++cat->timing_launches;
    if (cat->timing) {
        if (!cat->timing_all) {
            for (Shard& sh : cat->shards) {
                const DeviceSlot& slot = ctx->slots[sh.slot];
                MCD_HIP(hipSetDevice(slot.device));
                MCD_HIP(hipEventRecord(sh.ev_end, slot.stream));
            }
        }
        cat->timing_pending = true;
    }
    {
        WorkSet& w0 = (*find_work(cat->shards[0], W));
        cat->last_chunks = w0.n_chunks;
        mcd::LaunchShape sh0{cat->model, cat->free_centre, cat->precision, w0.fast};
        sh0.waves = w0.waves;
        const int64_t slots = mcd::partial_slots(sh0, w0.n_chunks, W);
        cat->last_grid = slots != w0.n_chunks ? slots : mcd::main_grid(w0.n_chunks, W);
    }
    return MCD_OK;
}

int fetch_once(mcd_catalog* cat, bool* rerun) {
    const int64_t W = cat->cur_walkers;
    const int64_t n_out = cat->n_psets * W;
    *rerun = false;
    const bool coll = cat->ctx->n_ranks > 1 || cat->ctx->slots.size() > 1 || cat->ctx->force_collective;
    bool any_fast = false;
    for (Shard& sh : cat->shards) {
        WorkSet& w = (*find_work(sh, W));
        any_fast = any_fast || w.fast != 0;
        const DeviceSlot& slot = cat->ctx->slots[sh.slot];
        MCD_HIP(hipSetDevice(slot.device));
        if (!w.mapped && &sh == &cat->shards[0]) {
            const double* res = w.buf ? w.d_out2 : w.d_out;
            if (w.comm_pending[w.buf]) MCD_HIP(hipStreamWaitEvent(slot.stream, w.ev_comm[w.buf], 0));
            hipStream_t copy_stream = (!coll && w.buf && w.lane1_used) ? slot.stream2 : slot.stream;
            MCD_HIP(hipMemcpyAsync(w.h_out, res, (size_t)(n_out + 1) * sizeof(double), hipMemcpyDeviceToHost, copy_stream));
        }
    }
    int rc = sync_all(cat);
    if (rc != MCD_OK) return rc;
    const WorkSet& w0 = (*find_work(cat->shards[0], W));
    if (coll) {
        for (int64_t i = 0; i < n_out && !*rerun; ++i) *rerun = w0.h_out[i] != w0.h_out[i];
    } else if (any_fast) {
        *rerun = w0.h_out[n_out] == w0.launch_tag;
    }
    return MCD_OK;
}

int fetch(mcd_catalog* cat, double* out) {
    if (!cat || !out) return fail(MCD_ERR_INVALID, "null catalogue or output");
    if (cat->cur_walkers <= 0 || !all_staged(cat)) return fail(MCD_ERR_INVALID, "nothing evaluated yet");
    const int64_t W = cat->cur_walkers;
    const int64_t n_out = cat->n_psets * W;
    bool rerun = false;
    int rc = fetch_once(cat, &rerun);
    if (rc != MCD_OK) return rc;
    if (rerun) {
        ++cat->n_reruns;
        for (Shard& sh : cat->shards) (*find_work(sh, W)).fast = 0;
        rc = enqueue(cat, false);
        if (rc != MCD_OK) return rc;
        rc = fetch_once(cat, &rerun);
        if (rc != MCD_OK) return rc;
    }
    std::memcpy(out, (*find_work(cat->shards[0], W)).h_out, (size_t)n_out * sizeof(double));
    return MCD_OK;
}

int per_star(mcd_catalog* cat, int32_t k, const double* params, int mode, double* out) {
    if (!cat || !params || !out) return fail(MCD_ERR_INVALID, "per-star output: null argument");
    if (mcd::bg_kind(cat->model) == mcd::BG_NONE) return fail(MCD_ERR_INVALID, "per-star outputs need a background model");
    if (cat->n_psets != 1) return fail(MCD_ERR_INVALID, "per-star outputs are defined for un-binned catalogues");
    if (k != cat->k) return fail(MCD_ERR_INVALID, "parameter row has the wrong number of columns");
    const size_t term_bytes = cat->precision == MCD_F64 ? 8 : 4;
    for (Shard& sh : cat->shards) {
        if (sh.n == 0) continue;
        const DeviceSlot& slot = cat->ctx->slots[sh.slot];
        MCD_HIP(hipSetDevice(slot.device));
        double* d_p = nullptr; void* d_w = nullptr; double* d_o = nullptr;
        MCD_HIP(hipMalloc(&d_p, k * sizeof(double)));
        MCD_HIP(hipMalloc(&d_w, mcd::KD * term_bytes));
        MCD_HIP(hipMalloc(&d_o, (size_t)sh.n * sizeof(double)));
        MCD_HIP(hipMemcpyAsync(d_p, params, k * sizeof(double), hipMemcpyHostToDevice, slot.stream));
        MCD_HIP(mcd::launch_prepare_walkers(slot.stream, d_p, 1, k, cat->model, cat->free_centre, cat->precision, d_w));
        mcd::LaunchShape shape{cat->model, cat->free_centre, cat->precision, 0};
        MCD_HIP(mcd::launch_per_star(slot.stream, shape, sh.records, sh.n, d_w, mode, d_o));
        MCD_HIP(hipMemcpyAsync(out + sh.star_begin, d_o, (size_t)sh.n * sizeof(double), hipMemcpyDeviceToHost, slot.stream));
        MCD_HIP(hipStreamSynchronize(slot.stream));
        MCD_HIP(hipFree(d_p)); MCD_HIP(hipFree(d_w)); MCD_HIP(hipFree(d_o));
    }
    return MCD_OK;
}

}

extern "C" {

int mcd_params_upload(mcd_catalog* cat, int64_t n_walkers, int32_t k, const double* params) {
    try { return stage_params(cat, n_walkers, k, params, false); } catch (...) { return on_exception("mcd_params_upload"); }
}

int mcd_loglike_enqueue(mcd_catalog* cat) {
    try { return enqueue(cat, true); } catch (...) { return on_exception("mcd_loglike_enqueue"); }
}
int mcd_loglike_fetch(mcd_catalog* cat, double* out) {
    try { return fetch(cat, out); } catch (...) { return on_exception("mcd_loglike_fetch"); }
}
// ... 30 lines not shown
```

mcmc_dynamics_amd/csrc/mcd_chunks.h:

```cpp
#pragma once

#include <algorithm>
#include <cmath>
#include <cstdint>
#include <vector>

namespace mcd {

struct Chunk {
    int64_t begin;
    int32_t count;
    int32_t pset;
};

struct ShardRange { int64_t begin, n; };
inline ShardRange shard_range(int64_t n_stars, int i, int n_shards) {
    const int64_t b = n_stars * i / n_shards;
    return ShardRange{b, n_stars * (i + 1) / n_shards - b};
}

constexpr int64_t kMaxChunkLen = (int64_t)1 << 20;

struct ChunkPlan {
    std::vector<Chunk> chunks;
    std::vector<int64_t> offsets;
    std::vector<uint8_t> general;
    int64_t max_chunks_per_pset = 0;
    int64_t len = 0;
    int uniform_len = 0;
    int uniform_extra = 0;
    int balanced_m = 0;
};

inline Chunk uniform_chunk(int64_t c, int64_t len, int64_t extra, int64_t n, int64_t n_chunks) {
    Chunk ch;
    ch.begin = c * len + 8 * std::min(c, extra);
    ch.count = (int32_t)(c == n_chunks - 1 ? n - ch.begin : len + (c < extra ? 8 : 0));
    ch.pset = 0;
    return ch;
}

constexpr int64_t kNumCUs = 256;

inline int64_t balanced_chunk_count(int64_t n_wtiles, int64_t m) {
    if (n_wtiles <= 0 || m <= 0) return 0;
    if (n_wtiles == 3) return (4 * kNumCUs * m + 2) / 3;
    if (n_wtiles <= 4) return kNumCUs * m * (4 / n_wtiles);
    const int64_t mb = (n_wtiles + 3) / 4;
    return std::max<int64_t>(8, kNumCUs * m / mb / 8 * 8);
}

inline ChunkPlan plan_chunks(const std::vector<int64_t>& bin_offsets, int64_t star_begin, int64_t n, int64_t n_walkers,
                             int64_t target_waves, int tail_split, const std::vector<int64_t>& narrow_exceptions,
                             int64_t chunk_len = 0, int balance = 0) {
    ChunkPlan plan;
    const int64_t n_psets = (int64_t)bin_offsets.size() - 1;
    const int64_t n_wtiles = (n_walkers + 63) / 64;
    if (balance > 0 && n_psets == 1 && chunk_len == 0 && n > 0 && bin_offsets[0] <= star_begin &&
        bin_offsets[1] >= star_begin + n) {
        const int64_t m = std::min<int64_t>(balance, 8);
        const int64_t G = balanced_chunk_count(n_wtiles, m);
        const int64_t q = G > 0 ? n / G / 8 * 8 : 0;
        if (q >= 16 && q + 8 < kMaxChunkLen) {
            const int64_t extra = (n - G * q) / 8;
            plan.len = q;
            plan.uniform_len = (int)q;
            plan.uniform_extra = (int)extra;
            plan.balanced_m = (int)m;
            plan.chunks.reserve((size_t)G);
            for (int64_t c = 0; c < G; ++c) plan.chunks.push_back(uniform_chunk(c, q, extra, n, G));
            plan.offsets = {0, G};
            plan.max_chunks_per_pset = G;
        }
    }
    if (!plan.chunks.empty()) {
    } else {
    plan = ChunkPlan();
    int64_t len;
    if (n_wtiles > 4) len = (5 * n * n_wtiles + 6 * target_waves - 1) / std::max<int64_t>(1, 6 * target_waves);
    else if (n_wtiles == 4) len = (n * n_wtiles + target_waves - 1) / std::max<int64_t>(1, target_waves);
    else len = (5 * n * n_wtiles / 4 + (target_waves * 3 / 5 - 136) - 1) / std::max<int64_t>(1, target_waves * 3 / 5 - 136);
    if (n_psets > 1) len = std::max<int64_t>(1, len * 4 / 5);
    if (chunk_len > 0) {
        len = std::max<int64_t>(64, (chunk_len + 31) / 32 * 32);
    } else {
        const int64_t k = std::max<int64_t>(1, len / 64);
        len = 32 * (2 * k + 1);
    }
    len = std::min(len, kMaxChunkLen - 32);
    plan.len = len;
    plan.offsets.assign(n_psets + 1, 0);
    for (int64_t p = 0; p < n_psets; ++p) {
        plan.offsets[p] = (int64_t)plan.chunks.size();
        const int64_t b0 = std::max(bin_offsets[p], star_begin);
        const int64_t b1 = std::min(bin_offsets[p + 1], star_begin + n);
        const int64_t total = b1 - b0;
        const int mode = (total >= 16 * len && len >= 128 && p == n_psets - 1) ? tail_split : 0;
        const int64_t resident_chunks = std::max<int64_t>(1, 8192 / n_wtiles);
        for (int64_t s = b0; s < b1;) {
            const int64_t done = s - b0, rem = b1 - s;
            int64_t step = len;
            if (mode == 1) step = done * 100 < total * 85 ? len : (done * 100 < total * 95 ? len / 2 : len / 4);
            else if (mode == 2) step = done * 100 < total * 70 ? len : (done * 100 < total * 85 ? len / 2 : (done * 100 < total * 95 ? len / 4 : len / 8));
            else if (mode == 3) step = std::min(len, std::max<int64_t>(64, rem / (2 * resident_chunks) / 8 * 8));
            else if (mode == 4) step = std::min(len, std::max<int64_t>(128, rem / resident_chunks / 8 * 8));
            step = std::max<int64_t>(8, step / 8 * 8);
            Chunk c;
            c.begin = s - star_begin;
            c.count = (int32_t)std::min(step, rem);
            c.pset = (int32_t)p;
            plan.chunks.push_back(c);
            s += step;
        }
        plan.max_chunks_per_pset = std::max<int64_t>(plan.max_chunks_per_pset, (int64_t)plan.chunks.size() - plan.offsets[p]);
    }
    plan.offsets[n_psets] = (int64_t)plan.chunks.size();
    if (n_psets == 1 && !plan.chunks.empty() && len < (int64_t)1 << 30) {
        bool uniform = true;
        for (size_t i = 0; i < plan.chunks.size() && uniform; ++i) {
            const Chunk u = uniform_chunk((int64_t)i, len, 0, n, (int64_t)plan.chunks.size());
            uniform = plan.chunks[i].begin == u.begin && plan.chunks[i].count == u.count;
        }
        if (uniform) plan.uniform_len = (int)len;
    }
    }
    if (!narrow_exceptions.empty()) {
        plan.general.assign(plan.chunks.size(), 0);
        bool any = false;
        for (size_t i = 0; i < plan.chunks.size(); ++i) {
            const int64_t lo = star_begin + plan.chunks[i].begin, hi = lo + plan.chunks[i].count;
            const auto it = std::lower_bound(narrow_exceptions.begin(), narrow_exceptions.end(), lo);
            if (it != narrow_exceptions.end() && *it < hi) { plan.general[i] = 1; any = true; }
        }
        if (!any) plan.general.clear();
    }
    return plan;
}

inline std::vector<double> pset_background_sums(const double* lnlike_bg, const std::vector<int64_t>& bin_offsets,
                                                int64_t star_begin, int64_t n) {
    const int64_t n_psets = (int64_t)bin_offsets.size() - 1;
    std::vector<double> sums(n_psets, 0.0);
    for (int64_t p = 0; p < n_psets; ++p) {
        const int64_t b0 = std::max(bin_offsets[p], star_begin);
        const int64_t b1 = std::min(bin_offsets[p + 1], star_begin + n);
        double sum = 0.0, comp = 0.0;
        for (int64_t i = b0; i < b1; ++i) {
            const double x = lnlike_bg[i], t = sum + x;
            comp += (std::fabs(sum) >= std::fabs(x)) ? (sum - t) + x : (x - t) + sum;
            sum = t;
        }
        sums[p] = sum + comp;
    }
    return sums;
}

inline int64_t main_grid(int64_t n_chunks, int64_t n_walkers) {
    const int64_t n_wtiles = (n_walkers + 63) / 64;
    if (n_wtiles <= 4) return (n_chunks * n_wtiles + 3) / 4;
    return (n_chunks + 7) / 8 * 8 * ((n_wtiles + 3) / 4);
}

}
```

mcmc_dynamics_amd/csrc/mcd_host.h:

```cpp
#pragma once

#include <hip/hip_runtime.h>
#include <rccl/rccl.h>

#include <algorithm>
#include <atomic>
#include <chrono>
#include <cmath>
#include <cstdio>
#include <cstdlib>
#include <cstring>
#include <limits>
#include <map>
#include <memory>
#include <mutex>
#include <string>
#include <thread>
#include <vector>

#include "../../include/mcd.h"
#include "mcd_internal.h"
#include "mcd_guard.h"
#include "mcd_math.h"

struct mcd_ctx;
struct mcd_catalog;

#define MCD_HOST_BEGIN namespace mcd { namespace host __attribute__((visibility("hidden"))) {
#define MCD_HOST_END }}
MCD_HOST_BEGIN

extern thread_local std::string g_last_error;
int fail(int code, const std::string& msg);
int on_exception(const char* where) noexcept;

#define MCD_HIP(call)                                                                                   \
    do {                                                                                                \
        hipError_t e_ = (call);                                                                         \
        if (e_ != hipSuccess)                                                                           \
            return ::mcd::host::fail(MCD_ERR_HIP, std::string(#call) + ": " + hipGetErrorString(e_));   \
    } while (0)

struct Rccl {
    void* handle = nullptr;
    decltype(&ncclGetUniqueId) GetUniqueId = nullptr;
    decltype(&ncclCommInitRank) CommInitRank = nullptr;
    decltype(&ncclCommInitAll) CommInitAll = nullptr;
    decltype(&ncclCommDestroy) CommDestroy = nullptr;
    decltype(&ncclAllReduce) AllReduce = nullptr;
    decltype(&ncclGroupStart) GroupStart = nullptr;
    decltype(&ncclGroupEnd) GroupEnd = nullptr;
    decltype(&ncclGetErrorString) GetErrorString = nullptr;
    decltype(&ncclCommCount) CommCount = nullptr;
    decltype(&ncclCommUserRank) CommUserRank = nullptr;
    decltype(&ncclGetVersion) GetVersion = nullptr;
};
extern Rccl g_rccl;
int load_rccl();

#define MCD_NCCL(call)                                                                                  \
    do {                                                                                                \
        ncclResult_t r_ = (call);                                                                       \
        if (r_ != ncclSuccess)                                                                          \
            return ::mcd::host::fail(MCD_ERR_RCCL,                                                      \
                                   std::string(#call) + ": " + ::mcd::host::g_rccl.GetErrorString(r_)); \
    } while (0)

struct DeviceSlot {
    int device = 0;
    hipStream_t stream = nullptr;
    hipStream_t stream2 = nullptr;
    hipStream_t comm_stream = nullptr;
    ncclComm_t comm = nullptr;
};

struct WorkSet {
    int64_t n_walkers = 0;
    int64_t n_chunks = 0;
    int64_t max_chunks_per_pset = 0;
    int uniform_len = 0;
    int uniform_extra = 0;
    int waves = 4;
    mcd::Chunk* d_chunks = nullptr;
    int64_t* d_offsets = nullptr;
    uint8_t* d_chunk_general = nullptr;
    double* d_params = nullptr;
    void* d_wpar = nullptr;
    double* d_partials = nullptr;
    double* d_out = nullptr;
    double* d_out2 = nullptr;
    int buf = 0;
    double* d_partials2 = nullptr;
    hipEvent_t ev_staged = nullptr;
    bool lane1_knows_staging = false;
    bool lane1_used = false;
    hipEvent_t ev_reduced[2] = {nullptr, nullptr};
    hipEvent_t ev_comm[2] = {nullptr, nullptr};
    bool comm_pending[2] = {false, false};
    double* h_params = nullptr;
    double* h_out = nullptr;
    double* m_params = nullptr;
    double* m_out = nullptr;
    bool mapped = false;
    double launch_tag = 0.0;
    int fast = 0;
    int narrow_rescale = 0;
    bool staged = false;
};

struct ChainArena {
    char* d = nullptr;
    char* h = nullptr;
    size_t bytes = 0;
};

struct Shard {
    int slot = 0;
    int64_t star_begin = 0;
    int64_t n = 0;
    void* records = nullptr;
    double* d_pset_const = nullptr;
    std::map<int64_t, WorkSet> work;
    hipEvent_t ev_begin = nullptr, ev_k0 = nullptr, ev_k1 = nullptr, ev_end = nullptr;
    std::vector<std::pair<hipEvent_t, hipEvent_t>> ring;
    size_t ring_used = 0;
};

struct DeviceScratch {
    std::vector<void*> blocks;
    hipEvent_t e0 = nullptr, e1 = nullptr;
    DeviceScratch() = default;
    DeviceScratch(const DeviceScratch&) = delete;
    template <class T>
    hipError_t malloc(T** p, size_t bytes) {
        blocks.push_back(nullptr);
        const hipError_t e = hipMalloc(&blocks.back(), bytes);
        *p = static_cast<T*>(blocks.back());
        return e;
    }
    hipError_t create_events() {
        const hipError_t e = hipEventCreate(&e0);
        return e != hipSuccess ? e : hipEventCreate(&e1);
    }
    ~DeviceScratch() {
        for (void* p : blocks) (void)hipFree(p);
        if (e0) (void)hipEventDestroy(e0);
        if (e1) (void)hipEventDestroy(e1);
    }
};

int ctx_fail(mcd_ctx* ctx, const std::string& what);
int ctx_usable(mcd_ctx* ctx);
int wait_ctx_stream(mcd_ctx* ctx, hipStream_t s, int64_t spin_us, const char* stage);
int build_workset(mcd_catalog* cat, Shard& sh, int64_t n_walkers, WorkSet** out);
LaunchShape main_launch_shape(mcd_catalog* cat, const Shard& sh, const WorkSet& w, int level, bool coll, double* out_buf,
                              int64_t n_out);
const double* fast_pset_const(const mcd_catalog* cat, const Shard& sh, int level);
int fast_level(const mcd_catalog* cat, const double* params, int64_t n_rows);
int sync_all(mcd_catalog* cat);

MCD_HOST_END

struct mcd_ctx {
    std::vector<mcd::host::DeviceSlot> slots;
    int rank = 0;
    int n_ranks = 1;
    bool multi_process = false;
    bool force_collective = false;
    int64_t collective_timeout_ms = 120000;
    std::atomic<int> abort_flag{0};
    std::atomic<int> failed{0};
    std::mutex note_mutex;
    std::string abort_reason;
    std::string failure;
    bool has_comm() const { return n_ranks > 1 || slots.size() > 1 || force_collective; }
};

struct mcd_catalog {
    mcd_ctx* ctx = nullptr;
    int model = 0;
    bool free_centre = false;
    int precision = 0;
    int k = 4;
    int64_t n_stars = 0;
    int64_t n_psets = 1;
    std::vector<int64_t> bin_offsets;
    std::vector<mcd::host::Shard> shards;
    mcd::CatalogStats stats;
    bool timing = false;
    bool timing_all = false;
    int allow_fast = 1;
    bool zero_copy = true;
    int64_t timing_stride = 1;
    int64_t timing_launches = 0;
    int64_t spin_us = 20000;
    int tail_split = 1;
    int64_t target_waves = 10240;
    int64_t chunk_len = 0;
    int prefetch = -1;
    int narrow_bounded = 1;
    int balance = -1;
    int two_lanes = 1;
    int f32_domain = 1;
    mcd::F32Domain last_f32;
    int64_t posterior_pass = 65536;
    int64_t loo_scratch_mb = 2048;
    int combine = 1;
    int64_t cur_walkers = 0;
    double last_kernel_ms = -1.0, last_device_ms = -1.0;
    bool timing_pending = false;
    int64_t last_grid = 0, last_chunks = 0;
    uint64_t launch_seq = 0;
    int64_t n_reruns = 0;
    int device_chain = 1;
    int fused_reduce = 1;
    int defer_guard = 1;
    bool chain_last_fused = false;
    mcd::host::ChainArena chain;
    int chain_hint = -1;
    int64_t chain_backoff = 0;
    int chain_consecutive = 0;
    int64_t chain_device_blocks = 0, chain_host_blocks = 0, chain_discarded = 0;
    int chain_last_status = 0;
    std::vector<hipEvent_t> chain_events;
    int last_prefetch = -1;
    int last_narrow_bounded = -1;
};

#define MCD_WAIT(ctx, stream, spin, stage)                                                              \
    do {                                                                                                \
        const int w_rc_ = ::mcd::host::wait_ctx_stream((ctx), (stream), (spin), (stage));               \
        if (w_rc_ != MCD_OK) return w_rc_;                                                              \
    } while (0)
```

mcmc_dynamics_amd/csrc/mcd_internal.h:

```cpp
#pragma once

#include <hip/hip_runtime.h>
#include <cstdint>

#include "mcd_chunks.h"
#include "mcd_guard.h"

namespace mcd {

struct LaunchShape {
    int model;
    bool free_centre;
    int precision;
    int fast;
    int uniform_len = 0;
    int64_t n_records = 0;
    int uniform_extra = 0;
    int waves = 4;
    const uint8_t* chunk_general = nullptr;
    bool prefetch = false;
    int narrow_rescale = 0;
    double* rerun_flag = nullptr;
    double launch_tag = 0.0;
};

struct RawColumns {
    const double* ra;
    const double* dec;
    const double* v;
    const double* verr;
    const double* lnbg;
    const double* pmember;
    const double* density;
};

hipError_t launch_prepare_records(hipStream_t s, const RawColumns& raw, int64_t n, int model, bool free_centre,
                                  int precision, double ra_c_deg, double dec_c_deg, void* records);

hipError_t launch_prepare_walkers(hipStream_t s, const double* params, int64_t n_rows, int k, int model,
                                  bool free_centre, int precision, void* wpar);

inline bool narrow_bounded_launch(const LaunchShape& sh) {
    return sh.fast == 2 && sh.model == MODEL_BGFIXED && !sh.free_centre && sh.precision == 0 && sh.prefetch &&
           (sh.narrow_rescale == 16 || sh.narrow_rescale == 32);
}

hipError_t launch_loglike(hipStream_t s, const LaunchShape& shape, const void* records, const Chunk* chunks,
                          int64_t n_chunks, const void* wpar, double* partials, int64_t n_walkers);

hipError_t launch_reduce(hipStream_t s, const double* partials, const int64_t* pset_slot_offsets,
                         int64_t n_psets, int64_t n_slots, int64_t max_slots_per_pset, int64_t n_walkers,
                         const double* pset_const, double* out);
int64_t partial_slots(const LaunchShape& shape, int64_t n_chunks, int64_t n_walkers);
constexpr int64_t kFusedReduceSlots = 256;

hipError_t launch_per_star(hipStream_t s, const LaunchShape& shape, const void* records, int64_t n,
                           const void* wpar_row, int mode, double* out);

int record_bytes(int model, bool free_centre, int precision);

enum ChainMeta : int { META_N_OK = 0, META_STATUS = 1, META_LEVEL = 2, META_WORDS = 4 };
enum ChainStatus : int {
    CHAIN_NAN = 1,
    CHAIN_RERUN = 2,
    CHAIN_LEVEL = 4,
    CHAIN_NO_PROPOSAL = 8
};
struct StretchDevice {
    int64_t n_bins = 1;
    int64_t n_walkers = 0;
    int32_t n_dim = 0, k = 0;
    int32_t fixed_ok = 1;
    int32_t model = 0, free_centre = 0;
    int32_t allow_fast = 1;
    int32_t expected_level = 0;
#ifdef MCD_CHAIN_STAMPS
    unsigned long long* stamps = nullptr;
    long long launch_index = 0;
#endif
    int32_t force_general = 0;
    int32_t fused = 0;
    const double* partials = nullptr;
    int64_t n_slots = 0;
    const int64_t* slot_offsets = nullptr;
    const double* pset_const = nullptr;
    StatsScalars stats;
    const int32_t* col_source = nullptr;
    const double* col_const = nullptr;
    const double* col_factor = nullptr;
    const double* lo = nullptr;
    const double* hi = nullptr;
    double* pos = nullptr;
    double* lnp = nullptr;
    long long* accepted = nullptr;
    const int32_t* order = nullptr;
    const double* zz = nullptr;
    const double* thr = nullptr;
    const int32_t* pick = nullptr;
    double* chain = nullptr;
    double* lnprob_chain = nullptr;
    double* proposal = nullptr;
    uint8_t* ok = nullptr;
    int32_t* meta = nullptr;
    int32_t* n_ok = nullptr;
    double* ranges = nullptr;
    double* table = nullptr;
    int32_t defer_guard = 0;
    double* table_log = nullptr;
    int32_t* n_ok_log = nullptr;
    int32_t* level_log = nullptr;
    double* wpar = nullptr;
};

hipError_t launch_stretch_step(hipStream_t s, const StretchDevice& d, int64_t acc_step, int acc_h, int64_t prop_step,
                               int prop_h, const double* ll, double rerun_tag);
hipError_t launch_stretch_status(hipStream_t s, const int32_t* meta, double* out);
hipError_t launch_stretch_judge(hipStream_t s, const StretchDevice& d, int64_t n_launches);
bool chain_numbers_on_device(int64_t n_walkers);
hipError_t launch_chain_numbers(hipStream_t s, uint64_t seed, int64_t step0, int64_t i0, int64_t i1, int64_t n_bins,
                                int64_t n_walkers, int n_dim, int32_t* order, double* zz, double* thr, int32_t* pick);
bool stretch_step_handles(const StretchDevice& d);
bool stretch_step_fuses(const StretchDevice& d);

int kde_slices(int64_t n, int64_t m, int* slice_len);
hipError_t launch_kde(hipStream_t s, const double* comp, int64_t m, const double* v, const double* verr, int64_t n,
                      double sigma_int, int slice_len, int n_slices, double* part_dmin, double* part_sum,
                      double* out);

}
```

mcmc_dynamics_amd/csrc/mcd_kernels.hip:

```cpp
#include "mcd_internal.h"
#include "mcd_math.h"
#include "mcd_prep.h"
#include "mcd_reduce.h"

namespace mcd {

namespace {

constexpr int kWave = 64;
constexpr int kBlock = 256;
constexpr int kWavesPerBlock = kBlock / kWave;

constexpr double kR0Arcmin = 3437.7467707849392526;

template <class T>
__global__ __launch_bounds__(kBlock) void prepare_records_kernel(RawColumns raw, int64_t n, int model,
                                                                  int free_centre, double ra_c, double dec_c,
                                                                  T* __restrict__ rec) {
    int64_t i = (int64_t)blockIdx.x * kBlock + threadIdx.x;
    if (i >= n) return;
    const int nd = record_doubles(model, free_centre != 0);
    T* r = rec + i * nd;
    const double verr = raw.verr[i];
    r[0] = (T)raw.v[i];
    r[1] = (T)(verr * verr);
    const double ra = raw.ra[i], dec = raw.dec[i];
    const int k = geometry_doubles(model, free_centre != 0);
    if (free_centre) {
        double sa, ca, sd, cd;
        sincos(ra * kDeg2Rad, &sa, &ca);
        sincos(dec * kDeg2Rad, &sd, &cd);
        r[2] = (T)(cd * sa); r[3] = (T)(cd * ca); r[4] = (T)sd; r[5] = (T)0;
    } else {
        const double dra = (ra - ra_c) * kDeg2Rad;
        const double dec_r = dec * kDeg2Rad, dec_cr = dec_c * kDeg2Rad;
        const double dx = -kR0Arcmin * cos(dec_r) * sin(dra);
        const double dy = kR0Arcmin * (sin(dec_r) * cos(dec_cr) - cos(dec_r) * sin(dec_cr) * cos(dra));
        if (is_profile(model)) {
            const double xs = 60.0 * dx, ys = 60.0 * dy;
            r[2] = (T)xs; r[3] = (T)ys; r[4] = (T)(xs * xs + ys * ys); r[5] = (T)0;
        } else {
            const double rr = hypot(dx, dy);
            double s, c;
            if (rr > 0.0) { s = dy / rr; c = dx / rr; }
            else { s = 0.0; c = signbit(dx) ? -1.0 : 1.0; }
            r[2] = (T)s; r[3] = (T)c;
        }
    }
    const int bg = bg_kind(model);
    if (bg == BG_FIXED) {
        const double b = raw.lnbg[i], pm = raw.pmember[i];
        r[k] = (T)b; r[k + 1] = (T)pm; r[k + 2] = (T)(1.0 - pm); r[k + 3] = (T)fmax(log(pm) - (b + kHalfLn2Pi), -2000.0);
    } else if (bg == BG_GAUSS) {
        r[k] = (T)raw.density[i]; r[k + 1] = (T)0;
    } else if (bg == BG_FIXED_DENSITY) {
        const double b = raw.lnbg[i];
        r[k] = (T)b; r[k + 1] = (T)fmax(log(raw.density[i]) - (b + kHalfLn2Pi), -2000.0); r[k + 2] = (T)raw.density[i];
        r[k + 3] = (T)0;
    }
}

template <class T>
__global__ __launch_bounds__(kBlock) void prepare_walkers_kernel(const double* __restrict__ params, int64_t n_rows,
                                                                  int k, int model, int free_centre,
                                                                  T* __restrict__ wpar) {
    int64_t i = (int64_t)blockIdx.x * kBlock + threadIdx.x;
    if (i >= n_rows) return;
    walker_constants<T>(params + i * k, model, free_centre != 0, wpar + i * KD);
}

#ifdef MCD_MAIN_STAMPS
constexpr int kStampBlocks = 1 << 16;
__device__ unsigned long long g_main_stamps[kStampBlocks][4];
#endif

__device__ const double kExpTabDevice[kExpTabSize] = {MCD_EXP_TABLE_VALUES};
__device__ const double kExpTabSqrt2Device[kExpTabSize] = {MCD_EXP_TABLE_SQRT2_VALUES};

template <int MODEL, bool FREE, class T, class A, int FAST, bool PF, int WAVES, bool BOUNDED = false>
__global__ __launch_bounds__(WAVES * kWave, WAVES > 4 ? 4 : 1) void loglike_kernel(const T* __restrict__ recs,
                                                                 const Chunk* __restrict__ chunks,
                                                                 const T* __restrict__ wpar,
                                                                 double* __restrict__ partials, int64_t n_tasks,
                                                                 int n_wtiles, int64_t n_walkers, int64_t n_chunks,
                                                                 int uniform_len, int uniform_extra, int64_t n_records,
                                                                 double* __restrict__ rerun_flag, double launch_tag,
                                                                 const uint8_t* __restrict__ chunk_general,
                                                                 int64_t n_slots, int narrow_iters) {
    constexpr int ND = record_doubles(MODEL, FREE);
    constexpr int kThreads = WAVES * kWave;
    constexpr bool kCombine = WAVES > kWavesPerBlock;
#ifdef MCD_MAIN_STAMPS
    const unsigned long long stamp_entry = __builtin_amdgcn_s_memrealtime();
#endif
    constexpr bool kUsesExpTab = FAST && bg_kind(MODEL) != BG_NONE && sizeof(T) == 8;
    __shared__ double exptab_lds[kUsesExpTab ? kExpTabSize : 1];
    constexpr bool kTabBiased = kUsesExpTab && FAST == 2 && MODEL == MODEL_BGFIXED;
    __shared__ double combine_lds[kCombine ? WAVES : 1][kCombine ? kWave : 1];
    if constexpr (kUsesExpTab) {
        static_assert(kExpTabSize % kThreads == 0, "whole table entries per thread");
        const double* __restrict__ src = exp_table_is_sqrt2_scaled(MODEL) ? kExpTabSqrt2Device : kExpTabDevice;
#pragma unroll
        for (int i = 0; i < kExpTabSize / kThreads; ++i) {
            const int j = i * kThreads + threadIdx.x;
            exptab_lds[j] = kTabBiased ? exp_tab_bias(src[j], j) : src[j];
        }
        __syncthreads();
    }
    const int wave = __builtin_amdgcn_readfirstlane((int)(threadIdx.x >> 6));
    const int lane = threadIdx.x & (kWave - 1);
    int64_t chunk_id;
    int wtile;
    bool live = true;
    if (kCombine || n_wtiles <= kWavesPerBlock) {
        const int64_t task = (int64_t)blockIdx.x * WAVES + wave;
        if (task >= n_tasks) {
            if constexpr (!kCombine) return;
            live = false;
        }
        chunk_id = task / n_wtiles;
        wtile = (int)(task - chunk_id * n_wtiles);
        if (!live) { chunk_id = 0; wtile = wave % n_wtiles; }
    } else {
        const int m = (n_wtiles + kWavesPerBlock - 1) / kWavesPerBlock;
        const int64_t group = blockIdx.x / (8 * m);
        const int j = (int)(blockIdx.x - group * (8 * m));
        chunk_id = group * 8 + (j & 7);
        wtile = (j >> 3) * kWavesPerBlock + wave;
        if (chunk_id >= n_chunks || wtile >= n_wtiles) return;
    }
    Chunk ch;
    if (uniform_len > 0) {
        const int64_t shifted = chunk_id < (int64_t)uniform_extra ? chunk_id : (int64_t)uniform_extra;
        ch.begin = chunk_id * uniform_len + 8 * shifted;
        const int64_t left = n_records - ch.begin;
        ch.count = chunk_id == n_chunks - 1 ? (int32_t)left : uniform_len + (chunk_id < (int64_t)uniform_extra ? 8 : 0);
        ch.pset = 0;
    } else {
        ch = chunks[chunk_id];
    }
    const int64_t w_raw = (int64_t)wtile * kWave + lane;
    const bool active = w_raw < n_walkers;
    const int64_t w_idx = active ? w_raw : n_walkers - 1;

    double result = 0.0;
    if (live) {
        const T* __restrict__ wp = wpar + ((int64_t)ch.pset * n_walkers + w_idx) * KD;
        WalkerConsts<T> w;
        w.load(wp);

        const RecPtr<T> chunk_recs = (RecPtr<T>)(recs + ch.begin * ND);
        bool denormal;
        if constexpr (FAST == 2) {
            const bool general = bg_kind(MODEL) != BG_NONE && chunk_general != nullptr && chunk_general[chunk_id] != 0;
            if (general) result = chunk_loglike<MODEL, FREE, T, A, 1, PF, kTabBiased>(chunk_recs, ch.count, w, denormal, exptab_lds);
            else result = chunk_loglike<MODEL, FREE, T, A, 2, PF, kTabBiased, BOUNDED>(chunk_recs, ch.count, w, denormal,
                                                                                         exptab_lds, narrow_iters);
        } else {
            result = chunk_loglike<MODEL, FREE, T, A, FAST, PF>(chunk_recs, ch.count, w, denormal, exptab_lds);
        }
        if (FAST && denormal && active) {
            if (rerun_flag) *rerun_flag = launch_tag;
            else result = __builtin_nan("");
        }
    }
    if constexpr (kCombine) {
        combine_lds[wave][lane] = result;
        __syncthreads();
        if (wave < n_wtiles) {
            double sum = combine_lds[wave][lane];
            for (int c = n_wtiles; c < WAVES; c += n_wtiles) sum += combine_lds[c + wave][lane];
            partials[((w_raw >> 3) * n_slots + blockIdx.x) * kPartialGroup + (w_raw & (kPartialGroup - 1))] = sum;
        }
    } else {
        partials[((w_raw >> 3) * n_slots + chunk_id) * kPartialGroup + (w_raw & (kPartialGroup - 1))] = result;
    }
#ifdef MCD_MAIN_STAMPS
    if (threadIdx.x == 0 && blockIdx.x < kStampBlocks) {
        g_main_stamps[blockIdx.x][0] = stamp_entry;
        g_main_stamps[blockIdx.x][1] = __builtin_amdgcn_s_memrealtime();
        g_main_stamps[blockIdx.x][2] = ((unsigned long long)__builtin_amdgcn_s_getreg((31 << 11) | 20) << 32) |
                                       (unsigned)__builtin_amdgcn_s_getreg((31 << 11) | 4);
        g_main_stamps[blockIdx.x][3] = (unsigned long long)ch.count;
    }
#endif
}

template <int SUB, int U, bool ONE_ROUND>
__global__ __launch_bounds__(kPartialGroup * SUB) void reduce_group_kernel(const double* __restrict__ partials,
                                                                            const int64_t* __restrict__ offs,
                                                                            int64_t n_slots, int64_t n_walkers,
                                                                            int64_t n_groups,
                                                                            const double* __restrict__ pset_const,
                                                                            double* __restrict__ out, int64_t single0) {
    constexpr int kThreads = kPartialGroup * SUB;
    constexpr int kWaves = kThreads / kWave;
    __shared__ double lds[kWaves > 1 ? kWaves : 1][kPartialGroup];
    const int64_t pset = blockIdx.x / n_groups, g = blockIdx.x - pset * n_groups;
    const int q = threadIdx.x & 3, s = threadIdx.x >> 2;
    const int64_t c0 = single0 >= 0 ? 0 : offs[pset], c1 = single0 >= 0 ? single0 : offs[pset + 1];
    const double add = pset_const ? pset_const[pset] : 0.0;
    const double2* __restrict__ col = reinterpret_cast<const double2*>(partials + g * n_slots * kPartialGroup) + q;
    double ax, ay;
    reduce_sublane_sum<SUB, U, ONE_ROUND>(col, c0, c1, s, ax, ay);
    reduce_wave_combine(ax, ay);
    const int lane = threadIdx.x & (kWave - 1);
    if constexpr (kWaves > 1) {
        if (lane < 4) { lds[threadIdx.x >> 6][2 * q] = ax; lds[threadIdx.x >> 6][2 * q + 1] = ay; }
        __syncthreads();
        if (threadIdx.x < kPartialGroup) {
            double acc = lds[0][threadIdx.x];
#pragma unroll
            for (int w = 1; w < kWaves; ++w) acc += lds[w][threadIdx.x];
            const int64_t w = g * kPartialGroup + threadIdx.x;
            if (w < n_walkers) out[pset * n_walkers + w] = acc + add;
        }
    } else {
        if (lane < 4) {
            const int64_t w = g * kPartialGroup + 2 * q;
            if (w < n_walkers) out[pset * n_walkers + w] = ax + add;
            if (w + 1 < n_walkers) out[pset * n_walkers + w + 1] = ay + add;
        }
    }
}

template <int MODEL, bool FREE, class T>
__global__ __launch_bounds__(kBlock) void per_star_kernel(const T* __restrict__ recs, int64_t n,
                                                           const T* __restrict__ wp, int mode,
                                                           double* __restrict__ out) {
    constexpr int ND = record_doubles(MODEL, FREE);
    const int64_t i = (int64_t)blockIdx.x * kBlock + threadIdx.x;
    if (i >= n) return;
    WalkerConsts<T> w;
    w.load(wp);
    T lc, lb, m;
    star_components<MODEL, FREE, T>((RecPtr<T>)(recs + i * ND), w, lc, lb, m);
    if (mode == 1) { out[i] = (double)mixture_lnl(lc, lb, m); return; }
    const T shift = is_profile(MODEL) ? max_(lc, lb) : T(0);
    const T ec = m * exp_(lc - shift), eb = (T(1) - m) * exp_(lb - shift);
    out[i] = (double)(ec / (ec + eb));
}

template <int MODEL, bool FREE, class T, class A, int FAST>
hipError_t launch_one(hipStream_t s, const LaunchShape& sh, const void* records, const Chunk* chunks, int64_t n_chunks,
                      const void* wpar, double* partials, int64_t n_walkers) {
    const int n_wtiles = (int)((n_walkers + kWave - 1) / kWave);
    const int64_t n_tasks = n_chunks * n_wtiles;
    constexpr bool kCanCombine = FAST != 0 && sizeof(T) == 8 && sizeof(A) == 8;
    const bool combine = kCanCombine && sh.waves > kWavesPerBlock;
    const int64_t grid = combine ? (n_tasks + sh.waves - 1) / sh.waves
                                 : main_grid(n_chunks, n_walkers);
    if (grid <= 0) return hipSuccess;
    const int64_t n_slots = combine ? grid : n_chunks;
    constexpr bool kCanBound = FAST == 2 && MODEL == MODEL_BGFIXED && !FREE && sizeof(T) == 8 && sizeof(A) == 8;
    const bool bounded = kCanBound && sh.prefetch && narrow_bounded_launch(sh);
    const int narrow_iters = bounded ? sh.narrow_rescale / 8 : 1;
#define MCD_LAUNCH_MAIN(PF_, WAVES_, BOUNDED_)                                                                               \
    hipLaunchKernelGGL((loglike_kernel<MODEL, FREE, T, A, FAST, PF_, WAVES_, BOUNDED_>), dim3((unsigned)grid),               \
                       dim3(WAVES_ * kWave), 0, s, (const T*)records, chunks, (const T*)wpar, partials, n_tasks, n_wtiles,   \
                       n_walkers, n_chunks, sh.uniform_len, sh.uniform_extra, sh.n_records, sh.rerun_flag, sh.launch_tag,    \
                       sh.chunk_general, n_slots, narrow_iters)
    if constexpr (kCanCombine) {
        if (combine && sh.waves == 8) {
            if (bounded) MCD_LAUNCH_MAIN(true, 8, kCanBound);
            else if (sh.prefetch) MCD_LAUNCH_MAIN(true, 8, false);
            else MCD_LAUNCH_MAIN(false, 8, false);
            return hipGetLastError();
        }
        if constexpr (bg_kind(MODEL) != BG_GAUSS) {
            if (combine && sh.waves == 16) {
                if (bounded) MCD_LAUNCH_MAIN(true, 16, kCanBound);
                else if (sh.prefetch) MCD_LAUNCH_MAIN(true, 16, false);
                else MCD_LAUNCH_MAIN(false, 16, false);
                return hipGetLastError();
            }
        }
        if (combine) return hipErrorInvalidValue;
    }
    if (bounded) MCD_LAUNCH_MAIN(true, kWavesPerBlock, kCanBound);
    else if (FAST != 0 && sh.prefetch) MCD_LAUNCH_MAIN((FAST != 0), kWavesPerBlock, false);
    else MCD_LAUNCH_MAIN(false, kWavesPerBlock, false);
#undef MCD_LAUNCH_MAIN
    return hipGetLastError();
}

template <int MODEL, bool FREE>
hipError_t launch_precision(hipStream_t s, const LaunchShape& sh, const void* records, const Chunk* chunks,
                            int64_t n_chunks, const void* wpar, double* partials, int64_t n_walkers) {
    switch (sh.precision) {
        case 0:
            if constexpr (bg_kind(MODEL) != BG_NONE || (MODEL == MODEL_PROFILE && !FREE)) {
                if (sh.fast == 2)
                    return launch_one<MODEL, FREE, double, double, 2>(s, sh, records, chunks, n_chunks, wpar, partials, n_walkers);
            }
            if (sh.fast) return launch_one<MODEL, FREE, double, double, 1>(s, sh, records, chunks, n_chunks, wpar, partials, n_walkers);
            return launch_one<MODEL, FREE, double, double, 0>(s, sh, records, chunks, n_chunks, wpar, partials, n_walkers);
        case 1:
            if (sh.fast) return launch_one<MODEL, FREE, float, float, 1>(s, sh, records, chunks, n_chunks, wpar, partials, n_walkers);
            return launch_one<MODEL, FREE, float, float, 0>(s, sh, records, chunks, n_chunks, wpar, partials, n_walkers);
        case 2:
            if (sh.fast) return launch_one<MODEL, FREE, float, double, 1>(s, sh, records, chunks, n_chunks, wpar, partials, n_walkers);
            return launch_one<MODEL, FREE, float, double, 0>(s, sh, records, chunks, n_chunks, wpar, partials, n_walkers);
    }
    return hipErrorInvalidValue;
}

}

#ifdef MCD_MAIN_STAMPS
extern "C" int mcd_debug_main_stamps(unsigned long long* out, long long n_blocks) {
    if (n_blocks > kStampBlocks) n_blocks = kStampBlocks;
    return (int)hipMemcpyFromSymbol(out, HIP_SYMBOL(g_main_stamps), (size_t)n_blocks * 4 * sizeof(unsigned long long));
}
#endif

int record_bytes(int model, bool free_centre, int precision) {
    return record_doubles(model, free_centre) * (precision == 0 ? 8 : 4);
}

hipError_t launch_prepare_records(hipStream_t s, const RawColumns& raw, int64_t n, int model, bool free_centre,
                                  int precision, double ra_c_deg, double dec_c_deg, void* records) {
    if (n <= 0) return hipSuccess;
    const unsigned grid = (unsigned)((n + kBlock - 1) / kBlock);
    if (precision == 0)
        hipLaunchKernelGGL(prepare_records_kernel<double>, dim3(grid), dim3(kBlock), 0, s, raw, n, model,
                           (int)free_centre, ra_c_deg, dec_c_deg, (double*)records);
    else
        hipLaunchKernelGGL(prepare_records_kernel<float>, dim3(grid), dim3(kBlock), 0, s, raw, n, model,
                           (int)free_centre, ra_c_deg, dec_c_deg, (float*)records);
    return hipGetLastError();
}

hipError_t launch_prepare_walkers(hipStream_t s, const double* params, int64_t n_rows, int k, int model,
                                  bool free_centre, int precision, void* wpar) {
    if (n_rows <= 0) return hipSuccess;
    const unsigned grid = (unsigned)((n_rows + kBlock - 1) / kBlock);
    if (precision == 0)
        hipLaunchKernelGGL(prepare_walkers_kernel<double>, dim3(grid), dim3(kBlock), 0, s, params, n_rows, k, model,
                           (int)free_centre, (double*)wpar);
    else
        hipLaunchKernelGGL(prepare_walkers_kernel<float>, dim3(grid), dim3(kBlock), 0, s, params, n_rows, k, model,
                           (int)free_centre, (float*)wpar);
    return hipGetLastError();
}

hipError_t launch_loglike(hipStream_t s, const LaunchShape& sh, const void* records, const Chunk* chunks,
                          int64_t n_chunks, const void* wpar, double* partials, int64_t n_walkers) {
#define MCD_DISPATCH(M)                                                                                          \
    case M:                                                                                                      \
        return sh.free_centre ? launch_precision<M, true>(s, sh, records, chunks, n_chunks, wpar, partials, n_walkers) \
                              : launch_precision<M, false>(s, sh, records, chunks, n_chunks, wpar, partials, n_walkers);
    switch (sh.model) {
        MCD_DISPATCH(MODEL_CONST)
        MCD_DISPATCH(MODEL_BGFIXED)
        MCD_DISPATCH(MODEL_BGGAUSS)
        MCD_DISPATCH(MODEL_PROFILE)
        MCD_DISPATCH(MODEL_PROFILE_BGGAUSS)
        MCD_DISPATCH(MODEL_PROFILE_BGDENS)
        MCD_DISPATCH(MODEL_PROFILE_BGFIXED)
    }
#undef MCD_DISPATCH
    return hipErrorInvalidValue;
}

int64_t partial_slots(const LaunchShape& sh, int64_t n_chunks, int64_t n_walkers) {
    if (sh.waves <= kWavesPerBlock || sh.fast == 0 || sh.precision != 0) return n_chunks;
    const int64_t n_wtiles = (n_walkers + kWave - 1) / kWave;
    return (n_chunks * n_wtiles + sh.waves - 1) / sh.waves;
}

hipError_t launch_reduce(hipStream_t s, const double* partials, const int64_t* offs, int64_t n_psets,
                         int64_t n_slots, int64_t max_slots_per_pset, int64_t n_walkers, const double* pset_const,
                         double* out) {
    if (n_psets * n_walkers <= 0) return hipSuccess;
    const int64_t n_groups = (n_walkers + kPartialGroup - 1) / kPartialGroup;
    const dim3 grid((unsigned)(n_psets * n_groups));
    const int64_t single0 = n_psets == 1 ? n_slots : -1;
#define MCD_LAUNCH_REDUCE(SUB_, U_, ONE_)                                                                                   \
    hipLaunchKernelGGL((reduce_group_kernel<SUB_, U_, ONE_>), grid, dim3(kPartialGroup * SUB_), 0, s, partials, offs,       \
                       n_slots, n_walkers, n_groups, pset_const, out, single0)
    static_assert(kFusedReduceSlots == 2 * 8 * 16, "one round of the one-wave shape");
    if (max_slots_per_pset <= kFusedReduceSlots) MCD_LAUNCH_REDUCE(8, 16, true);
    else if (max_slots_per_pset <= 1024) MCD_LAUNCH_REDUCE(32, 16, true);
    else if (max_slots_per_pset <= 4096) MCD_LAUNCH_REDUCE(128, 16, true);
    else MCD_LAUNCH_REDUCE(128, 16, false);
#undef MCD_LAUNCH_REDUCE
    return hipGetLastError();
}

namespace {
template <int MODEL>
hipError_t per_star_model(hipStream_t s, const LaunchShape& sh, const void* records, int64_t n, const void* wpar_row,
                          int mode, double* out) {
    const unsigned grid = (unsigned)((n + kBlock - 1) / kBlock);
    if (sh.precision == 0) {
        if (sh.free_centre)
            hipLaunchKernelGGL((per_star_kernel<MODEL, true, double>), dim3(grid), dim3(kBlock), 0, s,
                               (const double*)records, n, (const double*)wpar_row, mode, out);
        else
            hipLaunchKernelGGL((per_star_kernel<MODEL, false, double>), dim3(grid), dim3(kBlock), 0, s,
                               (const double*)records, n, (const double*)wpar_row, mode, out);
    } else {
        if (sh.free_centre)
            hipLaunchKernelGGL((per_star_kernel<MODEL, true, float>), dim3(grid), dim3(kBlock), 0, s,
                               (const float*)records, n, (const float*)wpar_row, mode, out);
        else
            hipLaunchKernelGGL((per_star_kernel<MODEL, false, float>), dim3(grid), dim3(kBlock), 0, s,
                               (const float*)records, n, (const float*)wpar_row, mode, out);
    }
    return hipGetLastError();
}
}

hipError_t launch_per_star(hipStream_t s, const LaunchShape& sh, const void* records, int64_t n,
// ... 14 lines not shown
```

mcmc_dynamics_amd/csrc/mcd_math.h:

```cpp
#pragma once

#include <cmath>
#include <cstdint>
#include <cstring>

#include "mcd_exp_table.h"

#if defined(__HIPCC__)
#define MCD_HD __host__ __device__ __forceinline__
#else
#define MCD_HD inline
#endif
#if defined(__HIP_DEVICE_COMPILE__)
#define MCD_CONST_AS __attribute__((address_space(4)))
#else
#define MCD_CONST_AS
#endif
namespace mcd { template <class T> using RecPtr = const T MCD_CONST_AS*; }

#if defined(__HIP_DEVICE_COMPILE__)
#define MCD_KEEP_BRANCH() asm volatile("")
#else
#define MCD_KEEP_BRANCH() ((void)0)
#endif

namespace mcd {

constexpr double kLn2 = 0.693147180559945309417232121458;
constexpr double kLn2Pi = 1.837877066409345483560659472811;
constexpr double kHalfLn2Pi = 0.918938533204672741780329736406;

enum WalkerSlot : int {
    W_VSYS = 0, W_S2 = 1, W_VX = 2, W_VY = 3,
    W_SAC = 4, W_CAC = 5, W_SDC = 6, W_CDC = 7,
    W_VB = 8, W_SB2 = 9, W_FB = 10,
    W_A2 = 11, W_S2A = 12, W_RP2 = 13, W_2RP = 14,
    KD = 16
};

enum Model : int {
    MODEL_CONST = 0, MODEL_BGFIXED = 1, MODEL_BGGAUSS = 2,
    MODEL_PROFILE = 3, MODEL_PROFILE_BGGAUSS = 4, MODEL_PROFILE_BGDENS = 5,
    MODEL_PROFILE_BGFIXED = 6
};
constexpr int kNumModels = 7;
enum Background : int { BG_NONE = 0, BG_FIXED = 1, BG_GAUSS = 2, BG_FIXED_DENSITY = 3 };

MCD_HD constexpr bool is_profile(int model) { return model >= MODEL_PROFILE; }
MCD_HD constexpr int bg_kind(int model) {
    return (model == MODEL_CONST || model == MODEL_PROFILE) ? BG_NONE
           : (model == MODEL_BGFIXED || model == MODEL_PROFILE_BGFIXED) ? BG_FIXED
           : (model == MODEL_PROFILE_BGDENS) ? BG_FIXED_DENSITY : BG_GAUSS;
}

MCD_HD constexpr int geometry_doubles(int model, bool free_centre) {
    return (free_centre || is_profile(model)) ? 6 : 4;
}
MCD_HD constexpr int record_doubles(int model, bool free_centre) {
    return geometry_doubles(model, free_centre) +
           (bg_kind(model) == BG_NONE ? 0 : (bg_kind(model) == BG_GAUSS ? 2 : 4));
}

constexpr double kArcsecPerRad = 206264.80624709635516;

template <class T>
MCD_HD T fma_(T a, T b, T c) {
#if defined(__HIP_DEVICE_COMPILE__)
    return __builtin_fma(a, b, c);
#else
    return std::fma(a, b, c);
#endif
}
MCD_HD float fma_(float a, float b, float c) {
#if defined(__HIP_DEVICE_COMPILE__)
    return __builtin_fmaf(a, b, c);
#else
    return std::fmaf(a, b, c);
#endif
}

MCD_HD double rsqrt_nr(double n);
MCD_HD double rcp_nr(double x);

template <class T>
MCD_HD void free_centre_xy(T A, T B, T sd, T sac, T cac, T sdc, T cdc, T& x, T& y) {
    x = fma_(B, sac, -(A * cac));
    const T t = fma_(B, cac, A * sac);
    y = fma_(sd, cdc, -(sdc * t));
}

template <bool FASTMATH, class T>
MCD_HD T free_centre_residual(T A, T B, T sd, T sac, T cac, T sdc, T cdc, T vx, T vy, T v_minus_vsys) {
    T x, y;
    free_centre_xy(A, B, sd, sac, cac, sdc, cdc, x, y);
    const T r2 = fma_(x, x, y * y);
    T inv;
    if constexpr (FASTMATH && sizeof(T) == 8) {
        inv = (T)rsqrt_nr((double)r2);
    } else {
#if defined(__HIP_DEVICE_COMPILE__)
        inv = T(1) / sqrt(r2);
#else
        inv = T(1) / std::sqrt(r2);
#endif
    }
    const T cross = fma_(vx, y, -(vy * x));
    const T general = fma_(-cross, inv, v_minus_vsys);
    const T on_centre = fma_(vy, std::signbit(x) ? T(-1) : T(1), v_minus_vsys);
    return r2 > T(0) ? general : on_centre;
}

MCD_HD double fma_sgpr_addend(double a, double b, double c) {
#if defined(__HIP_DEVICE_COMPILE__)
    double r;
    asm("v_fma_f64 %0, %1, %2, %3" : "=v"(r) : "v"(a), "v"(b), "s"(c));
    return r;
#else
    return std::fma(a, b, c);
#endif
}

MCD_HD double fnma_sgpr_addend(double a, double b, double c) {
#if defined(__HIP_DEVICE_COMPILE__)
    double r;
    asm("v_fma_f64 %0, -%1, %2, %3" : "=v"(r) : "v"(a), "v"(b), "s"(c));
    return r;
#else
    return std::fma(-a, b, c);
#endif
}

MCD_HD double fmax_raw(double x, double lo) {
#if defined(__HIP_DEVICE_COMPILE__)
    double r;
    asm("v_max_f64 %0, %1, %2" : "=v"(r) : "v"(x), "s"(lo));
    return r;
#else
    return std::fmax(x, lo);
#endif
}

MCD_HD double log_unit(double m) {
#ifdef MCD_LIBM_LOG_UNIT
    const bool always_libm = true;
#else
    const bool always_libm = false;
#endif
    if (always_libm || !(m >= 0.5 && m < 1.0)) {
#if defined(__HIP_DEVICE_COMPILE__)
        return log(m);
#else
        return std::log(m);
#endif
    }
    const bool low = m < 0.70710678118654752440;
    const double mm = low ? m + m : m;
    const double f = (mm - 1.0) / (mm + 1.0), s = f * f;
// ... 190 lines not shown
    return log(x);
#else
    return std::log(x);
#endif
}
template <class T> MCD_HD T exp_(T x) {
#if defined(__HIP_DEVICE_COMPILE__)
    return exp(x);
#else
    return std::exp(x);
#endif
}
template <class T> MCD_HD T max_(T a, T b) { return a > b ? a : b; }

template <class T>
MCD_HD T gauss_lnl(T d, T n) {
    return T(-0.5) * (log_(n) + T(kLn2Pi) + d * d / n);
}

template <class T>
MCD_HD T mixture_lnl(T m, T b, T p) {
    T mx = max_(m, b);
    return mx + log_(p * exp_(m - mx) + (T(1) - p) * exp_(b - mx));
}


MCD_HD double rsqrt_nr(double n) {
#if defined(__HIP_DEVICE_COMPILE__)
    double y = __builtin_amdgcn_rsq(n);
#else
    double y = 1.0 / std::sqrt(n);
#endif
    const double e = fma_(-(n * y), y, 1.0);
    const double t = fma_(0.375, e, 0.5);
    return fma_(y, t * e, y);
}

MCD_HD double rcp_nr(double x) {
#if defined(__HIP_DEVICE_COMPILE__)
    double y = __builtin_amdgcn_rcp(x);
#else
    double y = 1.0 / x;
#endif
    const double e = fma_(-x, y, 1.0);
    return fma_(y, fma_(e, e, e), y);
}

MCD_HD double rsqrt2_newton(double m) {
#if defined(MCD_AB_NEWTON3)
    return 2.0 * rsqrt_nr(m);
#endif
#if defined(__HIP_DEVICE_COMPILE__)
    const double y = __builtin_amdgcn_rsq(m);
#else
    const double y = 1.0 / std::sqrt(m);
#endif
    const double s = fma_(-m, y * y, 3.0);
    return y * s;
}

MCD_HD double add_hi_word(double x, int32_t v) {
    uint32_t w[2];
    std::memcpy(w, &x, sizeof w);
    w[1] += (uint32_t)v;
    std::memcpy(&x, w, sizeof x);
    return x;
}

constexpr int kExpTabHiShift = 20 - kExpTabBits;
MCD_HD double exp_tab_bias(double t, int j) { return add_hi_word(t, -(j << kExpTabHiShift)); }

template <bool TWO_STEP>
MCD_HD double exp_tab_reduce(double u, int& k) {
    constexpr double kMagic = 6755399441055744.0;
    const double shifted = fma_(u, kExpTabInvStep, kMagic);
    const double kf = shifted - kMagic;
    uint64_t bits;
    std::memcpy(&bits, &shifted, sizeof bits);
    k = (int)(uint32_t)bits;
    if constexpr (TWO_STEP) {
        const double r = fma_(-kf, kExpTabStepHi, u);
        return fma_(-kf, kExpTabStepLo, r);
    } else {
        return fma_(-kf, kExpTabStepHi + kExpTabStepLo, u);
    }
}

template <bool TWO_STEP = true, bool BIASED = false>
MCD_HD double exp_tab(double u, int& e_out, const double* __restrict__ tab) {
    if constexpr (BIASED) {
        int k;
        const double r = exp_tab_reduce<TWO_STEP>(u, k);
        double p;
        if constexpr (kExpPolyDegree == 4) p = fma_(fma_(r, kExpPolyC4, kExpPolyC3), r, kExpPolyC2);
        else p = fma_(r, kExpPolyC3, kExpPolyC2);
        p = fma_(p, r, 1.0);
        p = fma_(p, r, 1.0);
        e_out = k >> kExpTabBits;
        const int j = k & (kExpTabSize - 1);
        return add_hi_word(tab[j], j << kExpTabHiShift) * p;
    }
    constexpr double kMagic = 6755399441055744.0;
    const double shifted = fma_(u, kExpTabInvStep, kMagic);
    const double kf = shifted - kMagic;
    uint64_t bits;
    std::memcpy(&bits, &shifted, sizeof bits);
    const int k = (int)(uint32_t)bits;
    double r;
    if constexpr (TWO_STEP) {
        r = fma_(-kf, kExpTabStepHi, u);
        r = fma_(-kf, kExpTabStepLo, r);
    } else {
        r = fma_(-kf, kExpTabStepHi + kExpTabStepLo, u);
    }
    double p;
    if constexpr (kExpPolyDegree == 4) p = fma_(fma_(r, kExpPolyC4, kExpPolyC3), r, kExpPolyC2);
    else p = fma_(r, kExpPolyC3, kExpPolyC2);
    p = fma_(p, r, 1.0);
    p = fma_(p, r, 1.0);
    e_out = k >> kExpTabBits;
    return tab[k & (kExpTabSize - 1)] * p;
}

constexpr int kExpTabKMin = -1021 * kExpTabSize;
MCD_HD double vgpr_constant(double x) {
#if defined(__HIP_DEVICE_COMPILE__)
    asm("" : "+v"(x));
#endif
    return x;
}
template <bool TWO_STEP = false, bool CLAMP = true>
MCD_HD double exp_tab_scaled(double u, const double* __restrict__ tab) {
    int k;
    const double r = exp_tab_reduce<TWO_STEP>(u, k);
    double p;
    if constexpr (kExpPolyDegree == 4) p = fma_(fma_(r, kExpPolyC4, kExpPolyC3), r, kExpPolyC2);
    else p = fma_(r, kExpPolyC3, kExpPolyC2);
    p = fma_(p, r, 1.0);
    p = fma_(p, r, 1.0);
    if constexpr (CLAMP) k = k > kExpTabKMin ? k : kExpTabKMin;
    const double t = tab[k & (kExpTabSize - 1)];
    const int32_t kh = (int32_t)((uint32_t)k << kExpTabHiShift);
#if defined(__HIP_DEVICE_COMPILE__)
    if constexpr (!CLAMP) {
        typedef uint32_t word2 __attribute__((ext_vector_type(2)));
        word2 w = __builtin_bit_cast(word2, t);
        w.y += (uint32_t)kh;
        return __builtin_bit_cast(double, w) * p;
    }
#endif
    return add_hi_word(t, kh) * p;
}

MCD_HD bool is_zero_bits(double x) {
    uint64_t b;
    __builtin_memcpy(&b, &x, sizeof b);
    return (b << 1) == 0;
}

MCD_HD double ldexp_(double x, int k) {
#if defined(__HIP_DEVICE_COMPILE__)
    return __builtin_ldexp(x, k);
#else
    return std::ldexp(x, k);
#endif
}
MCD_HD double fmin_(double a, double b) {
#if defined(__HIP_DEVICE_COMPILE__)
    return __builtin_fmin(a, b);
#else
    return std::fmin(a, b);
#endif
}
MCD_HD double fabs_(double a) {
#if defined(__HIP_DEVICE_COMPILE__)
    return __builtin_fabs(a);
#else
    return std::fabs(a);
#endif
}
MCD_HD double fmax_(double a, double b) {
#if defined(__HIP_DEVICE_COMPILE__)
    return __builtin_fmax(a, b);
#else
    return std::fmax(a, b);
#endif
}

struct BgFixedAcc {
    LogProduct l;
    LogProduct lden;
    int emin;
    MCD_HD void init() { l.init(); lden.init(); emin = LogProduct::kTrackInit; }
    MCD_HD bool denormal() const { return emin < LogProduct::kTrackFloor; }
    template <bool NARROW = false>
    MCD_HD void add_density(double d, double n, double rho, double f, double nbp, const double* __restrict__ exptab) {
        add<false, false, NARROW>(d, n, f, nbp, exptab);
        lden.mul(rho + f);
    }
    template <bool UNIFORM_OMP = true, bool HALVED = false, bool NARROW = false, bool TAB_BIASED = false, bool CLAMP = true>
    MCD_HD void add(double d, double n, double omp, double nbp, const double* __restrict__ exptab) {
        const double g = (NARROW && HALVED) ? rsqrt2_newton(n) : rsqrt_nr(n);
        const double dg = d * g;
        const double u0 = HALVED ? fnma_sgpr_addend(dg, dg, nbp) : fma_sgpr_addend(-0.5 * dg, dg, nbp);
        const double u = NARROW ? u0 : fmax_raw(u0, -1100.0);
        if constexpr (NARROW && TAB_BIASED) {
            const double es = exp_tab_scaled<false, CLAMP>(u, exptab);
            const double y = UNIFORM_OMP ? fma_sgpr_addend(g, es, omp) : fma_(g, es, omp);
            l.mul(y);
            return;
        }
        int k;
        const double er = exp_tab<!NARROW, TAB_BIASED>(u, k, exptab);
        if constexpr (NARROW) {
            const double y = UNIFORM_OMP ? fma_sgpr_addend(g, ldexp_(er, k), omp) : fma_(g, ldexp_(er, k), omp);
            l.mul(y);
            return;
        }
        const int kc = k > 1000 ? 1000 : k;
        const double y = UNIFORM_OMP ? fma_sgpr_addend(g, ldexp_(er, kc), omp) : fma_(g, ldexp_(er, kc), omp);
        l.mul_any_track(y, emin);
        l.e32 += k - kc;
    }
    MCD_HD void rescale() { l.rescale(); }
    MCD_HD void rescale_density() { l.rescale(); lden.rescale(); }
    MCD_HD void rescale_narrow() { l.rescale_narrow(); }
    MCD_HD void rescale_density_narrow() { l.rescale_narrow(); lden.rescale_narrow(); }
    MCD_HD double finish() { return l.value(); }
    MCD_HD double finish_density() { return l.value() - lden.value(); }
};

struct BgGaussAcc {
    double sum_min;
    LogProduct ly;
    LogProduct lden;
    int emin;
    MCD_HD void init() { sum_min = 0.0; ly.init(); lden.init(); emin = LogProduct::kTrackInit; }
    MCD_HD bool denormal() const { return emin < LogProduct::kTrackFloor; }
    template <bool HALVED = false, bool NARROW = false>
    MCD_HD void add(double d, double n, double db, double nb, double rho, double f, const double* __restrict__ exptab) {
        const double g = (NARROW && HALVED) ? rsqrt2_newton(n) : rsqrt_nr(n);
        const double gb = (NARROW && HALVED) ? rsqrt2_newton(nb) : rsqrt_nr(nb);
        const double dg = d * g, dbg = db * gb;
        const double w = dg * dg, wb = dbg * dbg;
        const double t = wb - w;
        const bool cluster_big = t >= 0.0;
        const double u0 = HALVED ? -fabs_(t) : -0.5 * fabs_(t);
        int k;
        const double er = exp_tab<!NARROW>(NARROW ? u0 : fmax_(u0, -1100.0), k, exptab);
        const double e = ldexp_(er, k);
        const double a = rho * g, b = f * gb;
        const double y = cluster_big ? fma_(b, e, a) : fma_(a, e, b);
        if constexpr (NARROW) ly.mul(y);
        else ly.mul_any_track(y, emin);
        lden.mul(rho + f);
        sum_min += fmin_(w, wb);
    }
    MCD_HD void rescale() { ly.rescale(); lden.rescale(); }
    MCD_HD void rescale_narrow() { ly.rescale_narrow(); lden.rescale_narrow(); }
    template <bool HALVED = false>
    MCD_HD double finish(int64_t count) {
        const double per_star = HALVED ? kHalfLn2Pi - 0.5 * kLn2 : kHalfLn2Pi;
        return fma_(-(double)count, per_star, HALVED ? -sum_min : -0.5 * sum_min) + (ly.value() - lden.value());
    }
};

MCD_HD float rsqf_(float x) {
#if defined(__HIP_DEVICE_COMPILE__)
    return __builtin_amdgcn_rsqf(x);
#else
    return 1.0f / std::sqrt(x);
#endif
}
MCD_HD float expf_(float x) {
#if defined(__HIP_DEVICE_COMPILE__)
    return __builtin_amdgcn_exp2f(x * 1.44269504088896340736f);
#else
    return std::exp(x);
#endif
}
template <class A>
struct LogProductF {
    A p;
    int e;
    MCD_HD void init() { p = 1; e = 0; }
    MCD_HD void mul(float x) { p *= (A)x; }
    MCD_HD void rescale() {
        int ex;
        if constexpr (sizeof(A) == 8) {
#if defined(__HIP_DEVICE_COMPILE__)
            p = __builtin_frexp(p, &ex);
#else
            p = std::frexp(p, &ex);
#endif
        } else {
#if defined(__HIP_DEVICE_COMPILE__)
            p = __builtin_frexpf(p, &ex);
#else
            p = std::frexp(p, &ex);
#endif
        }
        e += ex;
    }
    MCD_HD double value() {
        rescale();
        return fma_((double)e, kLn2, log_unit((double)p));
    }
};
template <class A>
struct BgFixedAccF {
    LogProductF<A> l, lden;
    MCD_HD void init() { l.init(); lden.init(); }
    MCD_HD void add(float d, float n, float w0, float nbp) {
        const float g = rsqf_(n);
        const float dg = d * g;
        l.mul(fma_(g, expf_(fma_(-0.5f * dg, dg, nbp)), w0));
    }
    MCD_HD void add_density(float d, float n, float rho, float f, float nbp) {
        add(d, n, f, nbp);
        lden.mul(rho + f);
    }
    MCD_HD void rescale() { l.rescale(); }
    MCD_HD void rescale_density() { l.rescale(); lden.rescale(); }
    MCD_HD double finish() { return l.value(); }
    MCD_HD double finish_density() { return l.value() - lden.value(); }
    MCD_HD A value_for_anchor() const { return l.p; }
};
template <class A>
struct BgGaussAccF {
    A sum_min;
    LogProductF<A> ly, lden;
    MCD_HD void init() { sum_min = 0; ly.init(); lden.init(); }
    MCD_HD void add(float d, float n, float db, float nb, float rho, float f) {
        const float g = rsqf_(n), gb = rsqf_(nb);
        const float dg = d * g, dbg = db * gb;
        const float w = dg * dg, wb = dbg * dbg;
        const float t = wb - w;
        const float e = expf_(-0.5f * (t < 0.0f ? -t : t));
        const float a = rho * g, b = f * gb;
        ly.mul(t >= 0.0f ? fma_(b, e, a) : fma_(a, e, b));
        lden.mul(rho + f);
        sum_min += (A)(w < wb ? w : wb);
    }
    MCD_HD void rescale() { ly.rescale(); lden.rescale(); }
    MCD_HD double finish(int64_t count) {
        return fma_(-(double)count, kHalfLn2Pi, -0.5 * (double)sum_min) + (ly.value() - lden.value());
    }
    MCD_HD A value_for_anchor() const { return ly.p; }
};

struct KdeLane {
    double v, h, d2min, sum;
    MCD_HD void init(double v_, double verr, double sigma_int2) {
        v = v_;
        h = 0.5 / fma_(verr, verr, sigma_int2);
    }
    MCD_HD void nearest(double c, double& dmin) const { dmin = fmin_(dmin, fabs_(c - v)); }
    MCD_HD void begin_sum(double dmin) { d2min = dmin * dmin; sum = 0.0; }
    MCD_HD void add(double c, const double* __restrict__ exptab) {
        const double d = c - v;
        const double u = fmax_(fma_(-d, d, d2min) * h, -800.0);
        int k;
        const double er = exp_tab<false>(u, k, exptab);
        sum += ldexp_(er, k);
    }
};

#ifndef MCD_PREFETCH_DISTANCE
#define MCD_PREFETCH_DISTANCE 1
#endif
template <int BYTES, bool ON>
struct RecordPrefetch {
    static constexpr int kLines = (BYTES + 63) / 64 > 8 ? 8 : (BYTES + 63) / 64;
    uint32_t t;
    template <class P>
    MCD_HD void issue(P next) {
#if defined(__HIP_DEVICE_COMPILE__) && !defined(MCD_NO_PREFETCH)
        if constexpr (ON) {
            const unsigned lane = __builtin_amdgcn_mbcnt_hi(~0u, __builtin_amdgcn_mbcnt_lo(~0u, 0u));
            typedef const uint32_t __attribute__((address_space(1)))* global_word_ptr;
            t = 0;
            if (lane < (unsigned)kLines) t = *(global_word_ptr)((uint64_t)next + lane * 64u);
            return;
        }
#endif
        (void)next;
        t = 0;
    }
    MCD_HD void retire(double anchor) {
#if defined(__HIP_DEVICE_COMPILE__) && !defined(MCD_NO_PREFETCH)
        if constexpr (ON) asm volatile("" :: "v"(t), "v"(anchor));
#endif
        (void)anchor;
    }
};

template <class T> struct WalkerConsts {
    T vsys, s2, vx, vy, sac, cac, sdc, cdc, vb, sb2, fb, a2, s2a, rp2, rp_2;
    template <class P>
    MCD_HD void load(const P* __restrict__ p) {
        vsys = p[W_VSYS]; s2 = p[W_S2]; vx = p[W_VX]; vy = p[W_VY];
        sac = p[W_SAC]; cac = p[W_CAC]; sdc = p[W_SDC]; cdc = p[W_CDC];
        vb = p[W_VB]; sb2 = p[W_SB2]; fb = p[W_FB];
        a2 = p[W_A2]; s2a = p[W_S2A]; rp2 = p[W_RP2]; rp_2 = p[W_2RP];
    }
};

template <class T> MCD_HD T sqrt_(T x) {
#if defined(__HIP_DEVICE_COMPILE__)
    return sqrt(x);
#else
    return std::sqrt(x);
#endif
}

template <int MODEL, class T, bool FREE, bool FASTMATH = false, bool NEWTON1 = false>
MCD_HD void star_d_n(RecPtr<T> r, const WalkerConsts<T>& w, T& d, T& n) {
    if constexpr (!is_profile(MODEL)) {
        if (FREE) d = free_centre_residual<FASTMATH>(r[2], r[3], r[4], w.sac, w.cac, w.sdc, w.cdc, w.vx, w.vy, r[0] - w.vsys);
        else d = fma_(-w.vx, r[2], fma_(w.vy, r[3], r[0] - w.vsys));
        n = r[1] + w.s2;
    } else {
        T dx, dy, r2;
        if (FREE) {
            T x, y;
            free_centre_xy(r[2], r[3], r[4], w.sac, w.cac, w.sdc, w.cdc, x, y);
            dx = T(kArcsecPerRad) * x;
            dy = T(kArcsecPerRad) * y;
            r2 = fma_(dx, dx, dy * dy);
        } else { dx = r[2]; dy = r[3]; r2 = r[4]; }
        T t, inv;
        if constexpr (FASTMATH && NEWTON1 && sizeof(T) == 8) {
            const T cross = fma_(w.vx, dy, -(w.vy * dx));
            inv = (T)rcp_nr((double)(w.rp2 + r2));
            d = fma_(-(w.rp_2 * inv), cross, r[0] - w.vsys);
            n = fma_(T(0.5) * w.s2a, (T)rsqrt2_newton((double)(w.a2 + r2)), r[1]);
            return;
        } else if constexpr (FASTMATH && sizeof(T) == 8) {
            t = (T)rsqrt_nr((double)(w.a2 + r2));
            inv = (T)rcp_nr((double)(w.rp2 + r2));
        } else {
            t = T(1) / sqrt_(w.a2 + r2);
            inv = T(1) / (w.rp2 + r2);
        }
        const T cross = fma_(w.vx, dy, -(w.vy * dx));
        d = fma_(-(w.rp_2 * inv), cross, r[0] - w.vsys);
        n = fma_(w.s2a, t, r[1]);
    }
}

MCD_HD constexpr bool exp_table_is_sqrt2_scaled(int model) { return model == MODEL_BGFIXED; }

template <int MODEL, bool FREE, class T, class A, int FAST, bool PF = false, bool TAB_BIASED = false, bool BOUNDED = false>
MCD_HD double chunk_loglike(RecPtr<T> r, int count, const WalkerConsts<T>& w, bool& denormal,
                            const double* __restrict__ exptab, int rescale_iters = 1) {
    constexpr int ND = record_doubles(MODEL, FREE);
    denormal = false;
    constexpr int XB = geometry_doubles(MODEL, FREE);
    constexpr int BG = bg_kind(MODEL);
    double result;

    if constexpr (BG != BG_NONE && FAST && sizeof(T) == 4) {
        auto run4 = [&](auto& acc, auto&& one, auto&& rescale) {
            const int n4 = count >> 2;
            for (int g = 0; g < n4; ++g, r += 4 * ND) {
                RecordPrefetch<4 * ND * 4, PF> pf;
                pf.issue(r + MCD_PREFETCH_DISTANCE * 4 * ND);
#pragma unroll
                for (int j = 0; j < 4; ++j) one(r + j * ND);
                rescale();
                pf.retire((double)acc.value_for_anchor());
            }
            for (int j = n4 * 4; j < count; ++j, r += ND) { one(r); rescale(); }
        };
        if constexpr (BG == BG_GAUSS) {
            BgGaussAccF<A> acc;
            acc.init();
            run4(acc, [&](RecPtr<T> rr) {
                T d, n;
                star_d_n<MODEL, T, FREE, true>(rr, w, d, n);
                acc.add(d, n, rr[0] - w.vb, rr[1] + w.sb2, rr[XB], w.fb);
            }, [&]() { acc.rescale(); });
            result = acc.finish(count);
        } else if constexpr (BG == BG_FIXED) {
            BgFixedAccF<A> acc;
            acc.init();
            run4(acc, [&](RecPtr<T> rr) {
                T d, n;
                star_d_n<MODEL, T, FREE, true>(rr, w, d, n);
                acc.add(d, n, rr[XB + 2], rr[XB + 3]);
            }, [&]() { acc.rescale(); });
            result = acc.finish();
        } else {
            BgFixedAccF<A> acc;
            acc.init();
            run4(acc, [&](RecPtr<T> rr) {
                T d, n;
                star_d_n<MODEL, T, FREE, true>(rr, w, d, n);
                acc.add_density(d, n, rr[XB + 2], w.fb, rr[XB + 1]);
            }, [&]() { acc.rescale_density(); });
            result = acc.finish_density();
        }
    } else if constexpr (BG == BG_NONE && FAST && sizeof(T) == 4) {
        ConstAccF<A> acc;
        acc.init();
        constexpr bool TREE16 = MODEL == MODEL_CONST && !FREE;
        const int n16 = TREE16 ? count >> 4 : 0;
        for (int g = 0; g < n16; ++g, r += 16 * ND) {
            RecordPrefetch<16 * ND * 4, PF> pf;
            pf.issue(r + MCD_PREFETCH_DISTANCE * 16 * ND);
            float qq[16], nn[16];
#pragma unroll
            for (int j = 0; j < 16; ++j) {
                float d;
                star_d_n<MODEL, float, FREE, true>(r + j * ND, w, d, nn[j]);
                qq[j] = d * d;
            }
#pragma unroll
            for (int t = 0; t < 4; ++t) acc.add4(qq + 4 * t, nn + 4 * t);
            pf.retire((double)acc.p);
        }
        const int done = n16 << 4;
        const int n4 = (count - done) >> 2;
        for (int g = 0; g < n4; ++g, r += 4 * ND) {
            float qq[4], nn[4];
#pragma unroll
            for (int j = 0; j < 4; ++j) {
                float d;
                star_d_n<MODEL, float, FREE, true>(r + j * ND, w, d, nn[j]);
                qq[j] = d * d;
            }
            acc.add4(qq, nn);
        }
        for (int j = done + n4 * 4; j < count; ++j, r += ND) {
            float d, n;
            star_d_n<MODEL, float, FREE, true>(r, w, d, n);
            acc.add1(d * d, n);
        }
        result = acc.finish(count);
    } else if constexpr (BG == BG_NONE && FAST == 2 && MODEL == MODEL_PROFILE && !FREE) {
        ProfileNarrowAcc acc;
        acc.init();
        const double hs2a = 0.5 * w.s2a;
        auto one = [&](RecPtr<double> rr, double& q1, double& n1, double& m1) {
            m1 = w.rp2 + rr[4];
            const double t2 = rsqrt2_newton(w.a2 + rr[4]);
            const double n = fma_(hs2a, t2, rr[1]);
            const double cross = fma_(w.vx, rr[3], -(w.vy * rr[2]));
            const double nd = fma_(rr[0] - w.vsys, m1, -(w.rp_2 * cross));
            q1 = nd * nd;
            n1 = (m1 * m1) * n;
        };
        const int n8 = count >> 3;
        for (int g = 0; g < n8; ++g, r += 8 * ND) {
            RecordPrefetch<8 * ND * 8, PF> pf;
            pf.issue(r + MCD_PREFETCH_DISTANCE * 8 * ND);
            double qq[8], nn[8], mm[8];
#pragma unroll
            for (int j = 0; j < 8; ++j) one(r + j * ND, qq[j], nn[j], mm[j]);
            const double m_prod = ((mm[0] * mm[1]) * (mm[2] * mm[3])) * ((mm[4] * mm[5]) * (mm[6] * mm[7]));
            acc.add8(qq, nn, m_prod);
            pf.retire(acc.q);
        }
        for (int j = count & ~7; j < count; ++j, r += ND) {
            double q1, n1, m1;
            one(r, q1, n1, m1);
            acc.add1(q1, n1, m1);
        }
        result = acc.finish(count);
    } else if constexpr (BG == BG_NONE && FAST) {
        ConstAcc acc;
        acc.init();
        constexpr bool TREE16 = MODEL == MODEL_CONST && !FREE;
        const int n16 = TREE16 ? count >> 4 : 0;
        for (int g = 0; g < n16; ++g, r += 16 * ND) {
            RecordPrefetch<16 * ND * 8, PF> pf;
            pf.issue(r + MCD_PREFETCH_DISTANCE * 16 * ND);
            double qq[16], nn[16];
#pragma unroll
            for (int j = 0; j < 16; ++j) {
                double d;
                star_d_n<MODEL, double, FREE, true>(r + j * ND, w, d, nn[j]);
                qq[j] = d * d;
            }
            acc.add16(qq, nn);
            pf.retire(acc.q);
        }
        const int n8 = TREE16 ? (count >> 3) & 1 : count >> 3;
        for (int g = 0; g < n8; ++g, r += 8 * ND) {
            RecordPrefetch<8 * ND * 8, PF> pf;
            pf.issue(r + MCD_PREFETCH_DISTANCE * 8 * ND);
            double qq[8], nn[8];
#pragma unroll
            for (int j = 0; j < 8; ++j) {
                double d;
                star_d_n<MODEL, double, FREE, true>(r + j * ND, w, d, nn[j]);
                qq[j] = d * d;
            }
            acc.add8(qq, nn);
            pf.retire(acc.q);
        }
        for (int j = count & ~7; j < count; ++j, r += ND) {
            double d, n;
            star_d_n<MODEL, double, FREE, true>(r, w, d, n);
            acc.add1(d * d, n);
        }
        result = acc.finish(count);
    } else if constexpr (BG == BG_NONE) {
        A sum_log = 0, sum_q = 0;
#pragma unroll 4
        for (int j = 0; j < count; ++j, r += ND) {
            T d, n;
            star_d_n<MODEL, T, FREE>(r, w, d, n);
            sum_log += (A)log_(n);
            sum_q += (A)(d * d / n);
        }
        result = -0.5 * ((double)count * kLn2Pi + (double)sum_log + (double)sum_q);
    } else if constexpr (BG == BG_FIXED && FAST) {
        constexpr bool HALVED = MODEL == MODEL_BGFIXED;
        constexpr bool NARROW = FAST == 2 && MODEL == MODEL_BGFIXED;
        constexpr double kScale = NARROW ? 8.0 : 2.0;
        const double s2x = kScale * (double)w.s2;
        const double scale = BOUNDED ? vgpr_constant(kScale) : kScale;
        BgFixedAcc acc;
        acc.init();
        auto four = [&](RecPtr<double> r4) {
#pragma unroll
            for (int j = 0; j < 4; ++j) {
                RecPtr<double> rr = r4 + j * ND;
                double d, n;
                star_d_n<MODEL, double, FREE, true>(rr, w, d, n);
                if constexpr (HALVED) n = fma_(scale, rr[1], s2x);
                acc.add<true, HALVED, NARROW, TAB_BIASED, !BOUNDED>(d, n, rr[XB + 2], rr[XB + 3], exptab);
            }
        };
        const int n4 = count >> 2;
        static_assert(!BOUNDED || (NARROW && PF && TAB_BIASED && !FREE), "the bounded loop is the prefetching BGFIXED one");
        if constexpr (BOUNDED) {
            int until = rescale_iters;
            for (int g = 0; g < (count >> 3); ++g, r += 8 * ND) {
                RecordPrefetch<8 * ND * 8, PF> pf;
                pf.issue(r + MCD_PREFETCH_DISTANCE * 8 * ND);
                four(r);
                four(r + 4 * ND);
                pf.retire(acc.l.p);
                if (--until == 0) { until = rescale_iters; MCD_KEEP_BRANCH(); acc.rescale_narrow(); }
            }
            acc.rescale_narrow();
            if (n4 & 1) {
                four(r);
                r += 4 * ND;
                acc.rescale_narrow();
            }
        } else if constexpr (NARROW && PF) {
            for (int g = 0; g < (count >> 3); ++g, r += 8 * ND) {
                RecordPrefetch<8 * ND * 8, PF> pf;
                pf.issue(r + MCD_PREFETCH_DISTANCE * 8 * ND);
                four(r);
                four(r + 4 * ND);
                pf.retire(acc.l.p);
                acc.rescale_narrow();
            }
            if (n4 & 1) {
                four(r);
                r += 4 * ND;
                acc.rescale_narrow();
            }
        } else if constexpr (NARROW) {
            for (int g = 0; g < n4; ++g, r += 4 * ND) {
                four(r);
                if (g & 1) { MCD_KEEP_BRANCH(); acc.rescale_narrow(); }
            }
            if (n4 & 1) acc.rescale_narrow();
        } else {
            for (int g = 0; g < n4; ++g, r += 4 * ND) {
                RecordPrefetch<4 * ND * 8, PF> pf;
                pf.issue(r + MCD_PREFETCH_DISTANCE * 4 * ND);
                four(r);
                pf.retire(acc.l.p);
                acc.rescale();
            }
        }
        for (int j = n4 * 4; j < count; ++j, r += ND) {
            double d, n;
            star_d_n<MODEL, double, FREE, true>(r, w, d, n);
            if constexpr (HALVED) n = fma_(kScale, r[1], s2x);
            acc.add<true, HALVED, NARROW, TAB_BIASED, !BOUNDED>(d, n, r[XB + 2], r[XB + 3], exptab);
            acc.rescale();
        }
        result = acc.finish();
        denormal = acc.denormal();
    } else if constexpr (BG == BG_FIXED_DENSITY && FAST) {
        constexpr bool NARROW = FAST == 2;
        BgFixedAcc acc;
        acc.init();
        auto four = [&](RecPtr<double> r4) {
#pragma unroll
            for (int j = 0; j < 4; ++j) {
                RecPtr<double> rr = r4 + j * ND;
                double d, n;
                star_d_n<MODEL, double, FREE, true, NARROW>(rr, w, d, n);
                acc.add_density<NARROW>(d, n, rr[XB + 2], w.fb, rr[XB + 1], exptab);
            }
        };
        const int n4 = count >> 2;
        if constexpr (NARROW) {
            for (int g = 0; g < n4; ++g, r += 4 * ND) {
                RecordPrefetch<4 * ND * 8, PF> pf;
                pf.issue(r + MCD_PREFETCH_DISTANCE * 4 * ND);
                four(r);
                pf.retire(acc.l.p);
                if (g & 1) { MCD_KEEP_BRANCH(); acc.rescale_density_narrow(); }
            }
            if (n4 & 1) acc.rescale_density_narrow();
        } else {
            for (int g = 0; g < n4; ++g, r += 4 * ND) {
                RecordPrefetch<4 * ND * 8, PF> pf;
                pf.issue(r + MCD_PREFETCH_DISTANCE * 4 * ND);
                four(r);
                pf.retire(acc.l.p);
                acc.rescale_density();
            }
        }
        for (int j = n4 * 4; j < count; ++j, r += ND) {
            double d, n;
            star_d_n<MODEL, double, FREE, true, NARROW>(r, w, d, n);
            acc.add_density<NARROW>(d, n, r[XB + 2], w.fb, r[XB + 1], exptab);
            acc.rescale_density();
        }
        result = acc.finish_density();
        denormal = acc.denormal();
    } else if constexpr (BG == BG_GAUSS && FAST) {
        constexpr bool HALVED = MODEL == MODEL_BGGAUSS;
        constexpr bool NARROW = FAST == 2;
        constexpr double kScale = NARROW ? 8.0 : 2.0;
        const double s2x = kScale * (double)w.s2, sb2x = kScale * (double)w.sb2;
        BgGaussAcc acc;
        acc.init();
        auto one = [&](RecPtr<double> rr) {
            double d, n;
            star_d_n<MODEL, double, FREE, true, NARROW>(rr, w, d, n);
            if constexpr (HALVED) acc.add<true, NARROW>(d, fma_(kScale, rr[1], s2x), rr[0] - w.vb, fma_(kScale, rr[1], sb2x), rr[XB], w.fb, exptab);
            else acc.add<false, NARROW>(d, n, rr[0] - w.vb, rr[1] + w.sb2, rr[XB], w.fb, exptab);
        };
        auto four = [&](RecPtr<double> r4) {
#pragma unroll
            for (int j = 0; j < 4; ++j) one(r4 + j * ND);
        };
        const int n4 = count >> 2;
        if constexpr (NARROW) {
            for (int g = 0; g < n4; ++g, r += 4 * ND) {
                RecordPrefetch<4 * ND * 8, PF> pf;
                pf.issue(r + MCD_PREFETCH_DISTANCE * 4 * ND);
                four(r);
                pf.retire(acc.ly.p);
                if (g & 1) { MCD_KEEP_BRANCH(); acc.rescale_narrow(); }
            }
            if (n4 & 1) acc.rescale_narrow();
        } else {
            for (int g = 0; g < n4; ++g, r += 4 * ND) {
                RecordPrefetch<4 * ND * 8, PF> pf;
                pf.issue(r + MCD_PREFETCH_DISTANCE * 4 * ND);
                four(r);
                pf.retire(acc.ly.p);
                acc.rescale();
            }
        }
        for (int j = n4 * 4; j < count; ++j, r += ND) {
            one(r);
            acc.rescale();
        }
        result = acc.finish<HALVED>(count);
        denormal = acc.denormal();
    } else {
        A sum = 0;
#pragma unroll 2
        for (int j = 0; j < count; ++j, r += ND) {
            T d, n;
            star_d_n<MODEL, T, FREE>(r, w, d, n);
            const T m = gauss_lnl(d, n);
            T b, p;
            if (BG == BG_FIXED) {
                b = r[XB];
                p = r[XB + 1];
            } else if (BG == BG_FIXED_DENSITY) {
                b = r[XB];
                const T rho = r[XB + 2];
                p = rho / (rho + w.fb);
            } else {
                const T nb = r[1] + w.sb2;
                const T db = r[0] - w.vb;
                b = gauss_lnl(db, nb);
                const T rho = r[XB];
                p = rho / (rho + w.fb);
            }
            sum += (A)mixture_lnl(m, b, p);
        }
        result = (double)sum;
    }
    return result;
}

template <int MODEL, bool FREE, class T>
MCD_HD void star_components(RecPtr<T> r, const WalkerConsts<T>& w, T& lc, T& lb, T& m) {
    constexpr int XB = geometry_doubles(MODEL, FREE);
    constexpr int BG = bg_kind(MODEL);
    T d, n;
    star_d_n<MODEL, T, FREE>(r, w, d, n);
    lc = gauss_lnl(d, n);
    if (BG == BG_FIXED) { lb = r[XB]; m = r[XB + 1]; }
    else if (BG == BG_FIXED_DENSITY) { lb = r[XB]; const T rho = r[XB + 2]; m = rho / (rho + w.fb); }
    else if (BG == BG_GAUSS) { lb = gauss_lnl(r[0] - w.vb, r[1] + w.sb2); const T rho = r[XB]; m = rho / (rho + w.fb); }
    else { lb = T(-INFINITY); m = T(1); }
}

}
```

Baseline: 1425 billion terms/s.

## Sort BGFIXED records by verr and use per-chunk series for the rsqrt

Records for the fixed-background f64 model are re-sorted on the host by the verr^2 field and uploaded as a second device copy, with exception indices remapped. On narrow chunks whose verr^2 spread is small relative to s2, each star's 1/sqrt(verr^2+s2) is computed from a cubic Taylor expansion around the chunk midpoint instead of a per-star Newton rsqrt. A wave-wide ballot decides whether the series path is used, so the expensive per-star reciprocal square root is removed. The cost is doubled record memory, a one-time host sort, and added accuracy risk from the truncated series.

```diff
diff --git a/include/mcd.h b/include/mcd.h
--- a/include/mcd.h
+++ b/include/mcd.h
@@ -138,6 +138,7 @@
 int64_t mcd_rerun_count(const mcd_catalog* cat);
 int mcd_last_prefetch(const mcd_catalog* cat);
 int mcd_last_narrow_bounded(const mcd_catalog* cat);
+int64_t mcd_last_series_chunks(const mcd_catalog* cat);
 int mcd_last_fast_level(const mcd_catalog* cat);
 
 int mcd_last_f32_domain(const mcd_catalog* cat, double* kappa_v, double* kappa_theta);
diff --git a/mcmc_dynamics_amd/_native.py b/mcmc_dynamics_amd/_native.py
--- a/mcmc_dynamics_amd/_native.py
+++ b/mcmc_dynamics_amd/_native.py
@@ -65,6 +65,7 @@
     "mcd_rerun_count": (ctypes.c_int64, [ctypes.c_void_p]),
     "mcd_last_prefetch": (ctypes.c_int, [ctypes.c_void_p]),
     "mcd_last_narrow_bounded": (ctypes.c_int, [ctypes.c_void_p]),
+    "mcd_last_series_chunks": (ctypes.c_int64, [ctypes.c_void_p]),
     "mcd_last_fast_level": (ctypes.c_int, [ctypes.c_void_p]),
     "mcd_last_f32_domain": (ctypes.c_int, [ctypes.c_void_p, _c_double_p, _c_double_p]),
     "mcd_set_option": (ctypes.c_int, [ctypes.c_void_p, ctypes.c_char_p, ctypes.c_int64]),
@@ -457,6 +458,10 @@
     def last_narrow_bounded(self):
         return self.lib.mcd_last_narrow_bounded(self.handle)
 
+    @property
+    def last_series_chunks(self):
+        return self.lib.mcd_last_series_chunks(self.handle)
+
     def stretch_info(self):
         a, b, c, st = ctypes.c_int64(), ctypes.c_int64(), ctypes.c_int64(), ctypes.c_int32()
         _check(self.lib, self.lib.mcd_stretch_info(self.handle, ctypes.byref(a), ctypes.byref(b), ctypes.byref(c), ctypes.byref(st)),
diff --git a/mcmc_dynamics_amd/csrc/mcd_api_catalog.hip b/mcmc_dynamics_amd/csrc/mcd_api_catalog.hip
--- a/mcmc_dynamics_amd/csrc/mcd_api_catalog.hip
+++ b/mcmc_dynamics_amd/csrc/mcd_api_catalog.hip
@@ -50,6 +50,38 @@
     const size_t bytes = (size_t)sh.n * (size_t)mcd::record_bytes(cat->model, cat->free_centre, cat->precision);
     if (mcd::bg_kind(cat->model) == mcd::BG_NONE) return cat->n_psets == 1 && bytes >= ((size_t)128 << 20);
     return bytes >= ((size_t)8 << 20);
+}
+
+bool wants_sorted(const mcd_catalog* cat, const Shard& sh) {
+    if (cat->model != mcd::MODEL_BGFIXED || cat->free_centre || cat->precision != MCD_F64 || cat->n_psets != 1 || sh.n <= 0)
+        return false;
+    if (cat->verr_sorted >= 0) return cat->verr_sorted != 0;
+    if (cat->chunk_len > 0) return false;
+    return (size_t)sh.n * (size_t)mcd::record_bytes(cat->model, cat->free_centre, cat->precision) >= ((size_t)8 << 20);
+}
+
+int ensure_sorted_records(mcd_catalog* cat, Shard& sh) {
+    if (sh.records_sorted) return MCD_OK;
+    const DeviceSlot& slot = cat->ctx->slots[sh.slot];
+    constexpr int ND = mcd::record_doubles(mcd::MODEL_BGFIXED, false);
+    const size_t n = (size_t)sh.n, bytes = n * ND * sizeof(double);
+    MCD_HIP(hipStreamSynchronize(slot.stream));
+    std::vector<double> rec(n * ND), out(n * ND);
+    MCD_HIP(hipMemcpy(rec.data(), sh.records, bytes, hipMemcpyDeviceToHost));
+    const std::vector<int64_t> perm = mcd::verr_order(rec.data(), (int64_t)n, ND);
+    sh.sorted_e2.resize(n);
+    for (size_t i = 0; i < n; ++i) {
+        std::memcpy(&out[i * ND], &rec[(size_t)perm[i] * ND], ND * sizeof(double));
+        sh.sorted_e2[i] = out[i * ND + 1];
+    }
+    sh.sorted_exceptions = mcd::permuted_exceptions(cat->stats.narrow_exceptions, perm, sh.star_begin);
+    void* d = nullptr;
+    MCD_HIP(hipMalloc(&d, bytes + 2048));
+    hipError_t e = hipMemset(d, 0, bytes + 2048);
+    if (e == hipSuccess) e = hipMemcpy(d, out.data(), bytes, hipMemcpyHostToDevice);
+    if (e != hipSuccess) { (void)hipFree(d); MCD_HIP(e); }
+    sh.records_sorted = d;
+    return MCD_OK;
 }
 
 struct Option {
@@ -74,6 +106,8 @@
     {"posterior_pass", 1, kMax, "posterior_pass must be >= 1", false, false, MCD_SET(c->posterior_pass = v)},
     {"two_lanes", kMin, kMax, nullptr, true, false, MCD_SET(c->two_lanes = v != 0)},
     {"narrow_bounded", 0, 1, "narrow_bounded: 1 (where the guard admits it, default) or 0 (never)", false, false, MCD_SET(c->narrow_bounded = (int)v)},
+    {"verr_sorted", -1, 1, "verr_sorted: -1 (by record volume, default), 0 (catalogue order) or 1 (sorted by verr)", true, true, MCD_SET(c->verr_sorted = (int)v)},
+    {"root_series", 0, 1, "root_series: 1 (series root on the narrow chunks of verr-sorted records, default) or 0 (never)", false, false, MCD_SET(c->root_series = (int)v)},
     {"prefetch", -1, 1, "prefetch: -1 (by record volume, default), 0 (off) or 1 (on)", false, false, MCD_SET(c->prefetch = (int)v)},
     {"spin_us", 0, kMax, "spin_us must be >= 0", false, false, MCD_SET(c->spin_us = v)},
     {"tail_split", kMin, kMax, nullptr, true, true, MCD_SET(c->tail_split = (int)v)},
@@ -97,7 +131,17 @@
     shape.prefetch = wants_prefetch(cat, sh);
     cat->last_prefetch = shape.prefetch && shape.fast != 0;
     shape.rerun_flag = coll ? nullptr : out_buf + n_out;
+    shape.root_series = w.sorted && cat->root_series != 0;
     return shape;
+}
+
+const void* main_records(const Shard& sh, const WorkSet& w) { return w.sorted ? sh.records_sorted : sh.records; }
+
+int64_t series_chunk_count(const mcd_catalog* cat, const WorkSet& w, int level, const double* params, int64_t n_rows) {
+    if (!w.sorted || !cat->root_series || level != 2 || w.series_need.empty()) return 0;
+    const mcd::ParamRanges pr = mcd::table_ranges(cat->model, cat->free_centre, cat->k, params, n_rows);
+    if (!pr.finite) return 0;
+    return (int64_t)(std::upper_bound(w.series_need.begin(), w.series_need.end(), pr.s2_min) - w.series_need.begin());
 }
 
 const double* fast_pset_const(const mcd_catalog* cat, const Shard& sh, int level) {
@@ -116,10 +160,14 @@
     const DeviceSlot& slot = cat->ctx->slots[sh.slot];
     MCD_HIP(hipSetDevice(slot.device));
 
+    const bool sorted = wants_sorted(cat, sh);
+    if (sorted)
+        if (int rc = ensure_sorted_records(cat, sh)) return rc;
+    const std::vector<int64_t>& exceptions = sorted ? sh.sorted_exceptions : cat->stats.narrow_exceptions;
     mcd::ChunkPlan plan;
     for (int m = cat->balance < 0 ? balance_auto_m(cat, sh.n, n_walkers) : cat->balance;; m /= 2) {
         plan = mcd::plan_chunks(cat->bin_offsets, sh.star_begin, sh.n, n_walkers, cat->target_waves, cat->tail_split,
-                                cat->stats.narrow_exceptions, cat->chunk_len, m);
+                                exceptions, cat->chunk_len, m);
         if (m == 0 || plan.balanced_m > 0) break;
     }
     const std::vector<mcd::Chunk>& chunks = plan.chunks;
@@ -132,6 +180,8 @@
     w.max_chunks_per_pset = plan.max_chunks_per_pset;
     w.uniform_len = plan.uniform_len;
     w.uniform_extra = plan.uniform_extra;
+    w.sorted = sorted;
+    if (sorted) w.series_need = mcd::series_thresholds(plan, sh.sorted_e2.data());
     {
         const int64_t n_wtiles = (n_walkers + 63) / 64;
         const bool shape_ok = plan.balanced_m > 0 && plan.balanced_m % 2 == 0 && (n_wtiles == 1 || n_wtiles == 2 || n_wtiles == 4) &&
@@ -307,6 +357,7 @@
         (void)hipStreamSynchronize(cat->ctx->slots[sh.slot].stream2);
         for (auto& kv : sh.work) free_workset(kv.second);
         if (sh.records) (void)hipFree(sh.records);
+        if (sh.records_sorted) (void)hipFree(sh.records_sorted);
         if (sh.d_pset_const) (void)hipFree(sh.d_pset_const);
         if (sh.ev_begin) (void)hipEventDestroy(sh.ev_begin);
         if (sh.ev_k0) (void)hipEventDestroy(sh.ev_k0);
@@ -420,6 +471,8 @@
 
 int mcd_last_prefetch(const mcd_catalog* cat) { return cat ? cat->last_prefetch : -1; }
 
+int64_t mcd_last_series_chunks(const mcd_catalog* cat) { return cat ? cat->last_series_chunks : -1; }
+
 int mcd_last_narrow_bounded(const mcd_catalog* cat) { return cat ? cat->last_narrow_bounded : -1; }
 
 int mcd_last_f32_domain(const mcd_catalog* cat, double* kappa_v, double* kappa_theta) {
diff --git a/mcmc_dynamics_amd/csrc/mcd_api_chain.hip b/mcmc_dynamics_amd/csrc/mcd_api_chain.hip
--- a/mcmc_dynamics_amd/csrc/mcd_api_chain.hip
+++ b/mcmc_dynamics_amd/csrc/mcd_api_chain.hip
@@ -186,6 +186,7 @@
     double* const out_buf = w.d_out;
     mcd::LaunchShape shape = main_launch_shape(cat, sh, w, level, coll, out_buf, (int64_t)Bh);
     cat->last_narrow_bounded = 0;
+    cat->last_series_chunks = 0;
     const double* pset_const = fast_pset_const(cat, sh, level);
     const int64_t n_slots = mcd::partial_slots(shape, w.n_chunks, half);
     const int64_t max_slots = B == 1 ? n_slots : w.max_chunks_per_pset;
@@ -215,7 +216,7 @@
                 if (mark && i == i0 && h == 0) MCD_HIP(hipEventRecord(mark, slot.stream));
                 prev_tag = coll ? 0.0 : (double)(++cat->launch_seq);
                 shape.launch_tag = prev_tag;
-                MCD_HIP(mcd::launch_loglike(slot.stream, shape, sh.records, w.d_chunks, w.n_chunks, w.d_wpar, w.d_partials, half));
+                MCD_HIP(mcd::launch_loglike(slot.stream, shape, main_records(sh, w), w.d_chunks, w.n_chunks, w.d_wpar, w.d_partials, half));
                 if (!fused)
                     MCD_HIP(mcd::launch_reduce(slot.stream, w.d_partials, w.d_offsets, B, n_slots, max_slots, half, pset_const,
                                                out_buf));
diff --git a/mcmc_dynamics_amd/csrc/mcd_api_eval.hip b/mcmc_dynamics_amd/csrc/mcd_api_eval.hip
--- a/mcmc_dynamics_amd/csrc/mcd_api_eval.hip
+++ b/mcmc_dynamics_amd/csrc/mcd_api_eval.hip
@@ -99,6 +99,7 @@
         w->lane1_knows_staging = false;
         w->fast = fast;
         w->narrow_rescale = narrow_rescale;
+        w->series_chunks = series_chunk_count(cat, *w, fast, params, n_rows);
         w->staged = true;
     }
     cat->cur_walkers = n_walkers;
@@ -150,6 +151,8 @@
         mcd::LaunchShape shape = main_launch_shape(cat, sh, w, w.fast, coll, out_buf, n_out);
         shape.narrow_rescale = cat->narrow_bounded ? w.narrow_rescale : 0;
         cat->last_narrow_bounded = mcd::narrow_bounded_launch(shape) ? shape.narrow_rescale : 0;
+        if (&sh == &cat->shards.front()) cat->last_series_chunks = 0;
+        cat->last_series_chunks += shape.root_series && shape.fast == 2 ? w.series_chunks : 0;
         w.launch_tag = coll ? 0.0 : (double)(++cat->launch_seq);
         shape.launch_tag = w.launch_tag;
         hipEvent_t k0 = sh.ev_k0, k1 = sh.ev_k1;
@@ -168,7 +171,7 @@
         }
         if (cat->timing && !cat->timing_all) MCD_HIP(hipEventRecord(sh.ev_begin, slot.stream));
         if (cat->timing && sampled) MCD_HIP(hipEventRecord(k0, lane_stream));
-        MCD_HIP(mcd::launch_loglike(lane_stream, shape, sh.records, w.d_chunks, w.n_chunks, w.d_wpar, lane_partials, W));
+        MCD_HIP(mcd::launch_loglike(lane_stream, shape, main_records(sh, w), w.d_chunks, w.n_chunks, w.d_wpar, lane_partials, W));
         if (cat->timing && sampled) MCD_HIP(hipEventRecord(k1, lane_stream));
         const double* pset_const = fast_pset_const(cat, sh, w.fast);
         if (coll && w.comm_pending[w.buf]) {
diff --git a/mcmc_dynamics_amd/csrc/mcd_chunks.h b/mcmc_dynamics_amd/csrc/mcd_chunks.h
--- a/mcmc_dynamics_amd/csrc/mcd_chunks.h
+++ b/mcmc_dynamics_amd/csrc/mcd_chunks.h
@@ -3,6 +3,7 @@
 #include <algorithm>
 #include <cmath>
 #include <cstdint>
+#include <limits>
 #include <vector>
 
 namespace mcd {
@@ -137,6 +138,46 @@
     return plan;
 }
 
+inline std::vector<int64_t> verr_order(const double* records, int64_t n, int nd) {
+    std::vector<int64_t> perm((size_t)n);
+    for (int64_t i = 0; i < n; ++i) perm[(size_t)i] = i;
+    std::stable_sort(perm.begin(), perm.end(), [&](int64_t a, int64_t b) {
+        const double x = records[a * nd + 1], y = records[b * nd + 1];
+        return x < y || (y != y && x == x);
+    });
+    return perm;
+}
+
+inline std::vector<int64_t> permuted_exceptions(const std::vector<int64_t>& narrow_exceptions, const std::vector<int64_t>& perm,
+                                                int64_t star_begin) {
+    std::vector<int64_t> out;
+    if (narrow_exceptions.empty()) return out;
+    const int64_t n = (int64_t)perm.size();
+    std::vector<int64_t> inverse((size_t)n);
+    for (int64_t i = 0; i < n; ++i) inverse[(size_t)perm[(size_t)i]] = i;
+    for (int64_t g : narrow_exceptions)
+        if (g >= star_begin && g < star_begin + n) out.push_back(star_begin + inverse[(size_t)(g - star_begin)]);
+    std::sort(out.begin(), out.end());
+    return out;
+}
+
+inline double series_threshold(double e_first, double e_last) {
+    const double need = 0.5 * (e_last - e_first) * 0x1p13 - (0.5 * e_first + 0.5 * e_last);
+    return need == need ? need : std::numeric_limits<double>::infinity();
+}
+
+inline std::vector<double> series_thresholds(const ChunkPlan& plan, const double* sorted_e2) {
+    std::vector<double> need;
+    need.reserve(plan.chunks.size());
+    for (size_t c = 0; c < plan.chunks.size(); ++c) {
+        const Chunk& ch = plan.chunks[c];
+        if (ch.count <= 0 || (!plan.general.empty() && plan.general[c])) continue;
+        need.push_back(series_threshold(sorted_e2[ch.begin], sorted_e2[ch.begin + ch.count - 1]));
+    }
+    std::sort(need.begin(), need.end());
+    return need;
+}
+
 inline std::vector<double> pset_background_sums(const double* lnlike_bg, const std::vector<int64_t>& bin_offsets,
                                                 int64_t star_begin, int64_t n) {
     const int64_t n_psets = (int64_t)bin_offsets.size() - 1;
diff --git a/mcmc_dynamics_amd/csrc/mcd_host.h b/mcmc_dynamics_amd/csrc/mcd_host.h
--- a/mcmc_dynamics_amd/csrc/mcd_host.h
+++ b/mcmc_dynamics_amd/csrc/mcd_host.h
@@ -106,6 +106,9 @@
     int fast = 0;
     int narrow_rescale = 0;
     bool staged = false;
+    bool sorted = false;
+    std::vector<double> series_need;
+    int64_t series_chunks = 0;
 };
 
 struct ChainArena {
@@ -119,6 +122,9 @@
     int64_t star_begin = 0;
     int64_t n = 0;
     void* records = nullptr;
+    void* records_sorted = nullptr;
+    std::vector<double> sorted_e2;
+    std::vector<int64_t> sorted_exceptions;
     double* d_pset_const = nullptr;
     std::map<int64_t, WorkSet> work;
     hipEvent_t ev_begin = nullptr, ev_k0 = nullptr, ev_k1 = nullptr, ev_end = nullptr;
@@ -156,6 +162,8 @@
 LaunchShape main_launch_shape(mcd_catalog* cat, const Shard& sh, const WorkSet& w, int level, bool coll, double* out_buf,
                               int64_t n_out);
 const double* fast_pset_const(const mcd_catalog* cat, const Shard& sh, int level);
+const void* main_records(const Shard& sh, const WorkSet& w);
+int64_t series_chunk_count(const mcd_catalog* cat, const WorkSet& w, int level, const double* params, int64_t n_rows);
 int fast_level(const mcd_catalog* cat, const double* params, int64_t n_rows);
 int sync_all(mcd_catalog* cat);
 
@@ -199,6 +207,8 @@
     int64_t chunk_len = 0;
     int prefetch = -1;
     int narrow_bounded = 1;
+    int verr_sorted = -1;
+    int root_series = 1;
     int balance = -1;
     int two_lanes = 1;
     int f32_domain = 1;
@@ -224,6 +234,7 @@
     int chain_last_status = 0;
     std::vector<hipEvent_t> chain_events;
     int last_prefetch = -1;
+    int64_t last_series_chunks = -1;
     int last_narrow_bounded = -1;
 };
 
diff --git a/mcmc_dynamics_amd/csrc/mcd_internal.h b/mcmc_dynamics_amd/csrc/mcd_internal.h
--- a/mcmc_dynamics_amd/csrc/mcd_internal.h
+++ b/mcmc_dynamics_amd/csrc/mcd_internal.h
@@ -20,6 +20,7 @@
     const uint8_t* chunk_general = nullptr;
     bool prefetch = false;
     int narrow_rescale = 0;
+    bool root_series = false;
     double* rerun_flag = nullptr;
     double launch_tag = 0.0;
 };
diff --git a/mcmc_dynamics_amd/csrc/mcd_kernels.hip b/mcmc_dynamics_amd/csrc/mcd_kernels.hip
--- a/mcmc_dynamics_amd/csrc/mcd_kernels.hip
+++ b/mcmc_dynamics_amd/csrc/mcd_kernels.hip
@@ -86,7 +86,7 @@
                                                                  int uniform_len, int uniform_extra, int64_t n_records,
                                                                  double* __restrict__ rerun_flag, double launch_tag,
                                                                  const uint8_t* __restrict__ chunk_general,
-                                                                 int64_t n_slots, int narrow_iters) {
+                                                                 int64_t n_slots, int narrow_iters, int root_series) {
     constexpr int ND = record_doubles(MODEL, FREE);
     constexpr int kThreads = WAVES * kWave;
     constexpr bool kCombine = WAVES > kWavesPerBlock;
@@ -155,7 +155,7 @@
             const bool general = bg_kind(MODEL) != BG_NONE && chunk_general != nullptr && chunk_general[chunk_id] != 0;
             if (general) result = chunk_loglike<MODEL, FREE, T, A, 1, PF, kTabBiased>(chunk_recs, ch.count, w, denormal, exptab_lds);
             else result = chunk_loglike<MODEL, FREE, T, A, 2, PF, kTabBiased, BOUNDED>(chunk_recs, ch.count, w, denormal,
-                                                                                         exptab_lds, narrow_iters);
+                                                                                         exptab_lds, narrow_iters, root_series != 0);
         } else {
             result = chunk_loglike<MODEL, FREE, T, A, FAST, PF>(chunk_recs, ch.count, w, denormal, exptab_lds);
         }
@@ -259,7 +259,7 @@
     hipLaunchKernelGGL((loglike_kernel<MODEL, FREE, T, A, FAST, PF_, WAVES_, BOUNDED_>), dim3((unsigned)grid),               \
                        dim3(WAVES_ * kWave), 0, s, (const T*)records, chunks, (const T*)wpar, partials, n_tasks, n_wtiles,   \
                        n_walkers, n_chunks, sh.uniform_len, sh.uniform_extra, sh.n_records, sh.rerun_flag, sh.launch_tag,    \
-                       sh.chunk_general, n_slots, narrow_iters)
+                       sh.chunk_general, n_slots, narrow_iters, (int)sh.root_series)
     if constexpr (kCanCombine) {
         if (combine && sh.waves == 8) {
             if (bounded) MCD_LAUNCH_MAIN(true, 8, kCanBound);
diff --git a/mcmc_dynamics_amd/csrc/mcd_math.h b/mcmc_dynamics_amd/csrc/mcd_math.h
--- a/mcmc_dynamics_amd/csrc/mcd_math.h
+++ b/mcmc_dynamics_amd/csrc/mcd_math.h
@@ -3,6 +3,7 @@
 #include <cmath>
 #include <cstdint>
 #include <cstring>
+#include <type_traits>
 
 #include "mcd_exp_table.h"
 
@@ -499,6 +500,45 @@
     return add_hi_word(t, kh) * p;
 }
 
+struct RootSeries {
+    static constexpr double kMaxT = 0x1p-13;
+    double eb, b0, b1, b2, b3;
+    MCD_HD bool setup(double eb_, double half, double s2) {
+        eb = eb_;
+        const double p = 8.0 * eb, s2x = 8.0 * s2;
+        const double m0 = p + s2x;
+        const double bb = m0 - p;
+        const double err = (p - (m0 - bb)) + (s2x - bb);
+        const double inv = rcp_nr(m0);
+        const double y = rsqrt_nr(m0);
+        const double h = m0 * y;
+        const double eh = fma_(m0, y, -h);
+        const double res = fma_(-h, y, 1.0) - eh * y;
+        const double G0 = 2.0 * y;
+        const double q = 8.0 * inv;
+        b0 = fma_(G0, 0.5 * (res - err * inv), G0);
+        b1 = -0.5 * (G0 * q);
+        b2 = -0.75 * (b1 * q);
+        b3 = (-5.0 / 6.0) * (b2 * q);
+        return half >= 0.0 && 8.0 * half <= kMaxT * m0;
+    }
+    MCD_HD bool setup_chunk(double e_first, double e_last, double s2) {
+        return setup(0.5 * e_first + 0.5 * e_last, 0.5 * (e_last - e_first), s2);
+    }
+    MCD_HD double g(double e) const {
+        const double delta = e - eb;
+        return fma_(fma_(fma_(b3, delta, b2), delta, b1), delta, b0);
+    }
+};
+
+MCD_HD bool wave_all(bool ok) {
+#if defined(__HIP_DEVICE_COMPILE__)
+    return __builtin_amdgcn_ballot_w64(!ok) == 0;
+#else
+    return ok;
+#endif
+}
+
 MCD_HD bool is_zero_bits(double x) {
     uint64_t b;
     __builtin_memcpy(&b, &x, sizeof b);
@@ -548,6 +588,10 @@
     template <bool UNIFORM_OMP = true, bool HALVED = false, bool NARROW = false, bool TAB_BIASED = false, bool CLAMP = true>
     MCD_HD void add(double d, double n, double omp, double nbp, const double* __restrict__ exptab) {
         const double g = (NARROW && HALVED) ? rsqrt2_newton(n) : rsqrt_nr(n);
+        add_g<UNIFORM_OMP, HALVED, NARROW, TAB_BIASED, CLAMP>(d, g, omp, nbp, exptab);
+    }
+    template <bool UNIFORM_OMP = true, bool HALVED = false, bool NARROW = false, bool TAB_BIASED = false, bool CLAMP = true>
+    MCD_HD void add_g(double d, double g, double omp, double nbp, const double* __restrict__ exptab) {
         const double dg = d * g;
         const double u0 = HALVED ? fnma_sgpr_addend(dg, dg, nbp) : fma_sgpr_addend(-0.5 * dg, dg, nbp);
         const double u = NARROW ? u0 : fmax_raw(u0, -1100.0);
@@ -800,7 +844,7 @@
 
 template <int MODEL, bool FREE, class T, class A, int FAST, bool PF = false, bool TAB_BIASED = false, bool BOUNDED = false>
 MCD_HD double chunk_loglike(RecPtr<T> r, int count, const WalkerConsts<T>& w, bool& denormal,
-                            const double* __restrict__ exptab, int rescale_iters = 1) {
+                            const double* __restrict__ exptab, int rescale_iters = 1, bool series = false) {
     constexpr int ND = record_doubles(MODEL, FREE);
     denormal = false;
     constexpr int XB = geometry_doubles(MODEL, FREE);
@@ -971,31 +1015,37 @@
         const double scale = BOUNDED ? vgpr_constant(kScale) : kScale;
         BgFixedAcc acc;
         acc.init();
-        auto four = [&](RecPtr<double> r4) {
+        RootSeries sr;
+        auto one = [&](RecPtr<double> rr, auto SERIES, double sc) {
+            double d, n;
+            star_d_n<MODEL, double, FREE, true>(rr, w, d, n);
+            if constexpr (decltype(SERIES)::value) {
+                acc.add_g<true, HALVED, NARROW, TAB_BIASED, !BOUNDED>(d, sr.g(rr[1]), rr[XB + 2], rr[XB + 3], exptab);
+            } else {
+                if constexpr (HALVED) n = fma_(sc, rr[1], s2x);
+                acc.add<true, HALVED, NARROW, TAB_BIASED, !BOUNDED>(d, n, rr[XB + 2], rr[XB + 3], exptab);
+            }
+        };
+        auto four = [&](RecPtr<double> r4, auto SERIES) {
 #pragma unroll
-            for (int j = 0; j < 4; ++j) {
-                RecPtr<double> rr = r4 + j * ND;
-                double d, n;
-                star_d_n<MODEL, double, FREE, true>(rr, w, d, n);
-                if constexpr (HALVED) n = fma_(scale, rr[1], s2x);
-                acc.add<true, HALVED, NARROW, TAB_BIASED, !BOUNDED>(d, n, rr[XB + 2], rr[XB + 3], exptab);
-            }
+            for (int j = 0; j < 4; ++j) one(r4 + j * ND, SERIES, scale);
         };
         const int n4 = count >> 2;
         static_assert(!BOUNDED || (NARROW && PF && TAB_BIASED && !FREE), "the bounded loop is the prefetching BGFIXED one");
+        auto run = [&](auto SERIES) {
         if constexpr (BOUNDED) {
             int until = rescale_iters;
             for (int g = 0; g < (count >> 3); ++g, r += 8 * ND) {
                 RecordPrefetch<8 * ND * 8, PF> pf;
                 pf.issue(r + MCD_PREFETCH_DISTANCE * 8 * ND);
-                four(r);
-                four(r + 4 * ND);
+                four(r, SERIES);
+                four(r + 4 * ND, SERIES);
                 pf.retire(acc.l.p);
                 if (--until == 0) { until = rescale_iters; MCD_KEEP_BRANCH(); acc.rescale_narrow(); }
             }
             acc.rescale_narrow();
             if (n4 & 1) {
-                four(r);
+                four(r, SERIES);
                 r += 4 * ND;
                 acc.rescale_narrow();
             }
@@ -1003,19 +1053,19 @@
             for (int g = 0; g < (count >> 3); ++g, r += 8 * ND) {
                 RecordPrefetch<8 * ND * 8, PF> pf;
                 pf.issue(r + MCD_PREFETCH_DISTANCE * 8 * ND);
-                four(r);
-                four(r + 4 * ND);
+                four(r, SERIES);
+                four(r + 4 * ND, SERIES);
                 pf.retire(acc.l.p);
                 acc.rescale_narrow();
             }
             if (n4 & 1) {
-                four(r);
+                four(r, SERIES);
                 r += 4 * ND;
                 acc.rescale_narrow();
             }
         } else if constexpr (NARROW) {
             for (int g = 0; g < n4; ++g, r += 4 * ND) {
-                four(r);
+                four(r, SERIES);
                 if (g & 1) { MCD_KEEP_BRANCH(); acc.rescale_narrow(); }
             }
             if (n4 & 1) acc.rescale_narrow();
@@ -1023,17 +1073,29 @@
             for (int g = 0; g < n4; ++g, r += 4 * ND) {
                 RecordPrefetch<4 * ND * 8, PF> pf;
                 pf.issue(r + MCD_PREFETCH_DISTANCE * 4 * ND);
-                four(r);
+                four(r, SERIES);
                 pf.retire(acc.l.p);
                 acc.rescale();
             }
         }
         for (int j = n4 * 4; j < count; ++j, r += ND) {
-            double d, n;
-            star_d_n<MODEL, double, FREE, true>(r, w, d, n);
-            if constexpr (HALVED) n = fma_(kScale, r[1], s2x);
-            acc.add<true, HALVED, NARROW, TAB_BIASED, !BOUNDED>(d, n, r[XB + 2], r[XB + 3], exptab);
+            one(r, SERIES, kScale);
             acc.rescale();
+        }
+        };
+        constexpr bool kCanSeries = NARROW && MODEL == MODEL_BGFIXED && !FREE;
+        bool use_series = false;
+        if constexpr (kCanSeries) {
+            if (series && count > 0) {
+                const bool ok = sr.setup_chunk(r[1], r[(int64_t)(count - 1) * ND + 1], (double)w.s2);
+                use_series = wave_all(ok);
+            }
+        }
+        if constexpr (kCanSeries) {
+            if (use_series) { MCD_KEEP_BRANCH(); run(std::true_type()); }
+            else run(std::false_type());
+        } else {
+            run(std::false_type());
         }
         result = acc.finish();
         denormal = acc.denormal();
```

After: 1574 billion terms/s, median of 6. 1.1x the previous value.
